# bonevbs/HierarchicalSolvers.jl

Hardware: AMD Instinct MI355X
Metric: factorize+solve time, synthetic 3D problem, exact (swlevel=0) nested-dissection elimination (lower is better)
Workload: dtype f64; 1 GPU; poisson3d_128; n=2097152, nnz=14581760, tree_nodes=1023, tree_depth=10, nrhs=1, compression=none (swlevel=0), partition=subtree-per-rank x1

## Files before the change

### hierarchicalsolvers.jl_amd/_lib.py

```python
from __future__ import annotations

import ctypes as C
import os
import subprocess

_HERE = os.path.dirname(os.path.abspath(__file__))
LIB_PATH = os.path.join(_HERE, "libhs_solver.so")
CSRC = os.path.join(_HERE, "csrc")

i64 = C.c_int64
p_i64 = C.POINTER(C.c_int64)
p_f64 = C.POINTER(C.c_double)


class hs_options(C.Structure):
    _fields_ = [
        ("swlevel", i64), ("swsize", i64), ("atol", C.c_double), ("rtol", C.c_double), ("c_tol", C.c_double),
        ("leafsize", i64), ("kest", i64), ("stepsize", i64), ("verbose", C.c_uint8),
        ("keep_schur", C.c_uint8), ("profile", C.c_uint8), ("split", C.c_uint8), ("hss_d", C.c_uint8), ("hss_dexp", C.c_uint8), ("mf", C.c_uint8), ("dist_top", C.c_uint8), ("seed", i64), ("symmetric", C.c_uint8),
    ]


class hs_tree(C.Structure):
    _fields_ = [
        ("nnodes", i64), ("left", p_i64), ("right", p_i64),
        ("int_ptr", p_i64), ("int_idx", p_i64), ("bnd_ptr", p_i64), ("bnd_idx", p_i64),
        ("iloc_ptr", p_i64), ("iloc_idx", p_i64), ("bloc_ptr", p_i64), ("bloc_idx", p_i64),
    ]


class hs_stats(C.Structure):
    _fields_ = [
        ("n", i64), ("nnodes", i64), ("nlevels", i64), ("max_ni", i64), ("max_nb", i64),
        ("flops_factor", C.c_double), ("bytes_factors", C.c_double), ("bytes_solve", C.c_double),
        ("t_symbolic", C.c_double), ("t_upload", C.c_double), ("t_assemble", C.c_double), ("t_panel", C.c_double),
        ("t_trsm", C.c_double), ("t_gemm", C.c_double), ("t_total", C.c_double), ("t_solve", C.c_double),
        ("gemm_flops", C.c_double), ("gemm_launches", i64),
        ("t_mfma_kernel", C.c_double), ("mfma_kernel_launches", i64), ("gemm_bytes", C.c_double),
    ]


class hs_sparse_dev(C.Structure):
    _fields_ = [("n", i64), ("colptr", C.c_void_p), ("rowval", C.c_void_p), ("nzval", C.c_void_p),
                ("rowptr", C.c_void_p), ("colind", C.c_void_p), ("nzval_r", C.c_void_p)]


class hs_block_arg(C.Structure):
    _fields_ = [("dense", C.c_void_p), ("ld", i64), ("colptr", p_i64), ("rowval", p_i64), ("nzval", C.c_void_p)]


class hs_hss_blockop(C.Structure):
    _fields_ = [("n1", i64), ("n2", i64), ("H1", C.c_void_p), ("H2", C.c_void_p), ("gid", p_i64), ("A", C.POINTER(hs_sparse_dev)), ("lpos", C.c_void_p)]


class hs_hss_options(C.Structure):
    _fields_ = [("leafsize", i64), ("first_split", i64), ("atol", C.c_double), ("rtol", C.c_double), ("kest", i64), ("pad", i64), ("seed", i64),
                ("level_scale", C.c_double)]


HS_TRANSFER_FN = C.CFUNCTYPE(C.c_int, C.c_void_p, i64, p_i64, C.POINTER(C.c_void_p), p_i64, i64, p_i64, C.POINTER(C.c_void_p), p_i64)

HS_OK = 0
HS_ERR_ARGUMENT, HS_ERR_DIMENSION, HS_ERR_TREE, HS_ERR_SINGULAR = -1, -2, -3, -4
HS_ERR_HSS_LEAF, HS_ERR_DEVICE, HS_ERR_NOMEM, HS_ERR_UNSUPPORTED = -5, -6, -7, -8
HS_BLK_LU, HS_BLK_LBI, HS_BLK_UIB, HS_BLK_S, HS_BLK_DLU = 0, 1, 2, 3, 4

EXPORTS = [
    "hs_options_default", "hs_factor_d", "hs_factor_z", "hs_ldiv_d", "hs_ldiv_z", "hs_ldiv_dev_d", "hs_ldiv_dev_z",
    "hs_ldiv_t_d", "hs_ldiv_t_z", "hs_ldiv_dev_t_d", "hs_ldiv_dev_t_z",
    "hs_ldiv_block_d", "hs_ldiv_block_z", "hs_ldiv_block_dev_d", "hs_ldiv_block_dev_z", "hs_ldiv_block_info", "hsk_multi_prob_d", "hsk_multi_prob_z",
    "hs_ldiv_block_t_d", "hs_ldiv_block_t_z", "hs_ldiv_block_dev_t_d", "hs_ldiv_block_dev_t_z", "hsk_multi_prob_t_d", "hsk_multi_prob_t_z",
    "hs_ldiv_ulv_d", "hs_ldiv_ulv_z", "hs_ldiv_ulv_dev_d", "hs_ldiv_ulv_dev_z",
    "hs_mul_d", "hs_mul_z", "hs_mul_dev_d", "hs_mul_dev_z", "hs_mul_info", "hs_factor_error_d", "hs_factor_error_z",
    "hsk_multi_tri_d", "hsk_multi_tri_z", "hsk_multi_tri_t_d", "hsk_multi_tri_t_z",
    "hs_ldiv_sparse_d", "hs_ldiv_sparse_z", "hs_ldiv_sparse_dev_d", "hs_ldiv_sparse_dev_z", "hs_ldiv_sparse_plan", "hs_ldiv_sparse_info",
    "hs_opnorm", "hs_normestinv", "hs_condest", "hs_ldiv_refine_d", "hs_ldiv_refine_z", "hs_ldiv_refine_dev_d", "hs_ldiv_refine_dev_z",
    "hs_ldiv_refine_block_d", "hs_ldiv_refine_block_z", "hs_ldiv_refine_block_dev_d", "hs_ldiv_refine_block_dev_z", "hs_ldiv_refine_block_info",
    "hs_logabsdet", "hs_selinv", "hs_selinv_info", "hs_selinv_lr", "hs_selinv_lr_info", "hs_sym_info",
    "hs_interface_size", "hs_interface_indices", "hs_interface_matrix_d", "hs_interface_matrix_z", "hs_interface_info", "hsk_lu_product_d", "hsk_lu_product_z",
    "hs_interface_condense_d", "hs_interface_condense_z", "hs_interface_condense_dev_d", "hs_interface_condense_dev_z",
    "hs_interface_solve_d", "hs_interface_solve_z", "hs_interface_solve_dev_d", "hs_interface_solve_dev_z",
    "hs_interface_expand_d", "hs_interface_expand_z", "hs_interface_expand_dev_d", "hs_interface_expand_dev_z",
    "hs_sens_d", "hs_sens_z", "hs_sens_dev_d", "hs_sens_dev_z", "hs_misfit_d", "hs_misfit_z", "hs_misfit_dev_d", "hs_misfit_dev_z", "hs_sens_info", "hsk_sddmm_d", "hsk_sddmm_z",
    "hs_tangent_d", "hs_tangent_z", "hs_tangent_dev_d", "hs_tangent_dev_z", "hs_gn_hessvec_d", "hs_gn_hessvec_z", "hs_gn_hessvec_dev_d", "hs_gn_hessvec_dev_z",
    "hs_gn_diag_d", "hs_gn_diag_z", "hs_gn_diag_dev_d", "hs_gn_diag_dev_z", "hs_gn_info", "hsk_gn_rhs_d", "hsk_gn_rhs_z", "hsk_gn_rowsq_d", "hsk_gn_rowsq_z",
    "hs_mod_create_d", "hs_mod_create_z", "hs_mod_create_dev_d", "hs_mod_create_dev_z", "hs_mod_create_sparse_d", "hs_mod_create_sparse_z", "hs_mod_ldiv_d", "hs_mod_ldiv_z",
    "hs_mod_ldiv_dev_d", "hs_mod_ldiv_dev_z", "hs_mod_info", "hs_mod_free", "hs_gmres_block_mod_d", "hs_gmres_block_mod_z",
    "hs_eigs_d", "hs_eigs_z", "hs_eigs_info", "hs_eigs_gen_d", "hs_eigs_gen_z", "hs_eigs_gen_info", "hsk_eigs_coldot_d", "hsk_eigs_coldot_z", "hsk_eigs_rotate_d", "hsk_eigs_rotate_z", "hsk_eigs_chol_inv_d", "hsk_eigs_chol_inv_z", "hsk_small_eig_z", "hsk_eigs_phase_timing", "hsk_eigs_phases", "hsk_eigs_gen_mprod_seconds",
    "hs_f32_create", "hs_f32_ldiv_d", "hs_f32_ldiv_z", "hs_f32_ldiv_dev_d", "hs_f32_ldiv_dev_z", "hs_f32_info", "hs_f32_free", "hs_gmres_block_f32_d", "hs_gmres_block_f32_z",
    "hsk_multi_prob_f32_d", "hsk_multi_prob_f32_z", "hsk_multi_prob_t_f32_d", "hsk_multi_prob_t_f32_z", "hsk_round_factors_f32",
    "hsk_mod_inner_d", "hsk_mod_inner_z", "hsk_mod_apply_d", "hsk_mod_apply_z", "hsk_mod_gather_d", "hsk_mod_gather_z", "hsk_mod_cap_d", "hsk_mod_cap_z",
    "hs_maxrank", "hs_is_complex", "hs_size", "hs_free", "hs_last_error", "hs_last_error_info", "hs_get_stats",
    "hs_node_info", "hs_node_ranks", "hs_node_export", "hs_node_export_piv", "hs_device_info",
    "hs_analyze", "hs_plan", "hs_numeric_begin", "hs_numeric_levels", "hs_numeric_end", "hs_solve_fwd_levels", "hs_solve_bwd_levels",
    "hs_nlevels", "hs_cut_level", "hs_node_owner", "hs_num_exchanges", "hs_exchange_info", "hs_set_schur_buffer",
    "hs_pack_bnd", "hs_unpack_bnd", "hs_extract_owned", "hs_gmres_d", "hs_gmres_z", "hs_gmres_block_d", "hs_gmres_block_z", "hs_gmres_block_info", "hsk_spmm_d", "hsk_spmm_z",
    "hs_gmres_t_d", "hs_gmres_t_z", "hs_gmres_block_t_d", "hs_gmres_block_t_z", "hsk_spmm_op_d", "hsk_spmm_op_z",
    "hs_exchange_kind", "hs_schur_pack_size", "hs_schur_pack", "hs_schur_unpack", "hs_flow_info", "hs_hss_pack_size", "hs_hss_pack", "hs_hss_unpack", "hs_hss_qr_order",
    "hs_comm_unique_id", "hs_comm_create_rccl", "hs_comm_create_host", "hs_comm_free", "hs_comm_kind", "hs_comm_selftest", "hs_comm_bandwidth", "hs_set_comm",
    "hs_symbolic_from_elimtree", "hs_symbolic_from_graph", "hs_symbolic_size", "hs_symbolic_perm", "hs_symbolic_tree", "hs_symbolic_free",
    "hs_hss_options_default", "hs_hss_compress_d", "hs_hss_compress_z", "hs_hss_compress_ex_d", "hs_hss_compress_ex_z", "hs_hss_compress_lru_d", "hs_hss_compress_lru_z", "hs_hss_compress_lru_multi_d", "hs_hss_compress_lru_multi_z", "hs_hss_set_stream", "hs_hss_rank", "hs_hss_size", "hs_hss_samples", "hs_hss_num_nodes",
    "hs_hss_node_info", "hs_hss_node_data", "hs_hss_getindex", "hs_hss_basis", "hs_hss_expand", "hs_hss_mul", "hs_hss_mul_t", "hs_hss_child", "hs_hss_factor", "hs_hss_ldiv", "hs_hss_ldiv_t", "hsk_ulv_t_group_d", "hsk_ulv_t_group_z", "hs_hss_time", "hs_hss_trim", "hs_hss_free", "hs_node_schur_hss",
    "hs_hss_offdiag", "hs_hss_bytes", "hs_hss_prune_leaves", "hs_hss_compatible", "hs_hss_depth", "hs_hss_compress_blockop_d", "hs_hss_compress_blockop_z", "hs_hss_blockop_apply",
    "hsk_gemm_d", "hsk_gemm_z", "hsk_lowrank_d", "hsk_lowrank_z", "hsk_front_factor_d", "hsk_front_factor_z", "hsk_front_batch_d", "hsk_front_batch_z", "hsk_sweep_level_d", "hsk_sweep_level_z", "hsk_flow_tall_rule", "hsk_sweep_path", "hsk_mfma_f64_peak", "hsk_mfma_f64_peak_random", "hsk_flow_pingpong_us", "hsk_bisect_perm",
    "hs_probs_stats_mode", "hs_probs_stats", "hs_trim", "hs_stream_order",
    "hsk_leaf_envelope", "hsk_envelope_enable", "hsk_branch_envelope", "hsk_branch_envelope_enable", "hsk_front_batch_env_d", "hsk_op_flops_mode", "hsk_op_flops",
    "hsk_env_order_enable", "hsk_env_tile_order",
    "hsk_gemm_op_d", "hsk_gemm_lds_enable", "hsk_gemm_lds_launches",
    "hsk_gemm_lds_edge_launches", "hsk_gemm_reg_launches", "hsk_gemm_lds_route", "hsk_gemm_schur_d",
    "hsk_trsm_inv_d", "hsk_trsm_strip_enable", "hsk_trsm_strip_launches", "hsk_trsm_half_launches", "hsk_lookahead_runs", "hsk_front_batch_sym_d", "hsk_front_batch_sym_z",
    "hsk_qr_params", "hsk_qr_chol_d", "hsk_qr_chol_z", "hsk_qr_select", "hsk_qr_refine_d", "hsk_qr_refine_z",
]

_lib = None


def build(force=False, verbose=False):
    if force:
        subprocess.run(["make", "-C", CSRC, "clean"], check=True, capture_output=not verbose)
    r = subprocess.run(["make", "-C", CSRC, "-j4"], capture_output=True, text=True)
    if r.returncode != 0:
        raise RuntimeError("building libhs_solver.so failed:\n" + r.stdout[-4000:] + r.stderr[-4000:])
    return LIB_PATH


def lib():
    global _lib
    if _lib is not None:
        return _lib
    if not os.path.exists(LIB_PATH):
        raise RuntimeError(
            f"{LIB_PATH} not found: the HIP extension is not built (run __graft_entry__.build() or `make -C {CSRC}`); "
            "there is no CPU fallback"
        )
    try:
        import torch
    except Exception:
        pass
    L = C.CDLL(LIB_PATH)
    vp = C.c_void_p
    L.hs_options_default.argtypes = [C.POINTER(hs_options)]
    L.hs_options_default.restype = None
    for f in (L.hs_factor_d, L.hs_factor_z):
        f.argtypes = [i64, p_i64, p_i64, p_f64, C.POINTER(hs_tree), C.POINTER(hs_options), C.POINTER(vp)]
        f.restype = C.c_int
    for f in (L.hs_ldiv_d, L.hs_ldiv_z):
        f.argtypes = [vp, p_f64, i64, p_f64, i64, i64, i64]
        f.restype = C.c_int
    for f in (L.hs_ldiv_dev_d, L.hs_ldiv_dev_z):
        f.argtypes = [vp, vp, i64, vp, i64, i64, i64, vp]
        f.restype = C.c_int
    for host, dev in (("hs_ldiv_t", "hs_ldiv_dev_t"), ("hs_ldiv_block", "hs_ldiv_block_dev"), ("hs_ldiv_block_t", "hs_ldiv_block_dev_t"), ("hs_ldiv_ulv", "hs_ldiv_ulv_dev"),
                      ("hs_mul", "hs_mul_dev")):
        for sfx in ("_d", "_z"):
            f = getattr(L, host + sfx)
            f.argtypes = [vp, C.c_int, p_f64, i64, p_f64, i64, i64, i64]
            f.restype = C.c_int
            f = getattr(L, dev + sfx)
            f.argtypes = [vp, C.c_int, vp, i64, vp, i64, i64, i64, vp]
            f.restype = C.c_int
    L.hs_ldiv_block_info.argtypes = [vp, p_f64]
    L.hs_ldiv_block_info.restype = C.c_int
    L.hs_mul_info.argtypes = [vp, p_f64]
    L.hs_mul_info.restype = C.c_int
    for f in (L.hs_factor_error_d, L.hs_factor_error_z):
        f.argtypes = [vp, C.c_int, vp, i64, i64, i64, C.c_int, p_f64]
        f.restype = C.c_int
    for f in (L.hsk_multi_tri_d, L.hsk_multi_tri_z):
        f.argtypes = [i64, i64, i64, p_f64, i64, p_f64, i64, p_f64, i64, C.c_int, C.c_int, C.POINTER(C.c_int32)]
        f.restype = C.c_int
    for f in (L.hsk_multi_tri_t_d, L.hsk_multi_tri_t_z):
        f.argtypes = [i64, i64, i64, p_f64, i64, p_f64, i64, p_f64, i64, C.c_int, C.c_int, C.c_int, C.POINTER(C.c_int32)]
        f.restype = C.c_int
    for f in (L.hs_ldiv_sparse_d, L.hs_ldiv_sparse_z):
        f.argtypes = [vp, C.c_int, i64, i64, p_i64, p_i64, p_f64, p_i64, i64, p_f64, i64]
        f.restype = C.c_int
    for f in (L.hs_ldiv_sparse_dev_d, L.hs_ldiv_sparse_dev_z):
        f.argtypes = [vp, C.c_int, i64, i64, p_i64, p_i64, vp, p_i64, i64, vp, i64, vp]
        f.restype = C.c_int
    L.hs_ldiv_sparse_plan.argtypes = [vp, C.c_int, i64, i64, p_i64, p_i64, p_i64, i64, p_i64, p_i64, C.POINTER(C.c_uint8)]
    L.hs_ldiv_sparse_plan.restype = C.c_int
    L.hs_ldiv_sparse_info.argtypes = [vp, p_f64]
    L.hs_ldiv_sparse_info.restype = C.c_int
    for f in (L.hsk_multi_prob_d, L.hsk_multi_prob_z):
        f.argtypes = [i64, i64, i64, p_f64, i64, p_f64, i64, p_f64, i64, C.c_int, C.c_int, C.POINTER(C.c_int32)]
        f.restype = C.c_int
    for f in (L.hsk_multi_prob_t_d, L.hsk_multi_prob_t_z):
        f.argtypes = [i64, i64, i64, p_f64, i64, p_f64, i64, p_f64, i64, C.c_int, C.c_int, C.c_int, C.POINTER(C.c_int32)]
        f.restype = C.c_int
    L.hs_opnorm.argtypes = [vp, C.c_int, p_f64]
# ... 352 lines not shown
        f.restype = C.c_int
    for f in (L.hs_hss_compress_lru_d, L.hs_hss_compress_lru_z):
        f.argtypes = [i64, vp, i64, vp, i64, vp, i64, vp, i64, i64, i64, C.c_int, p_i64, C.POINTER(hs_hss_options), vp, C.POINTER(vp)]
        f.restype = C.c_int
    for f in (L.hs_hss_compress_lru_multi_d, L.hs_hss_compress_lru_multi_z):
        f.argtypes = [i64, p_i64, C.POINTER(vp), p_i64, C.POINTER(vp), p_i64, C.POINTER(vp), p_i64, C.POINTER(vp), p_i64, p_i64, p_i64, C.POINTER(p_i64),
                      C.POINTER(C.POINTER(hs_hss_options)), vp, C.POINTER(vp)]
        f.restype = C.c_int
    for f in (L.hs_hss_rank, L.hs_hss_size, L.hs_hss_samples, L.hs_hss_num_nodes, L.hs_hss_bytes):
        f.argtypes = [vp]
        f.restype = i64
    L.hs_node_schur_hss.argtypes = [vp, i64, C.POINTER(hs_hss_options), C.POINTER(vp)]
    L.hs_node_schur_hss.restype = C.c_int
    L.hs_hss_set_stream.argtypes = [vp, vp]
    L.hs_hss_set_stream.restype = C.c_int
    L.hs_hss_node_info.argtypes = [vp, i64, p_i64]
    L.hs_hss_node_info.restype = C.c_int
    L.hs_hss_node_data.argtypes = [vp, i64, p_i64, vp, vp, vp, vp]
    L.hs_hss_node_data.restype = C.c_int
    L.hs_hss_getindex.argtypes = [vp, p_i64, i64, p_i64, i64, vp, i64, C.c_int]
    L.hs_hss_getindex.restype = C.c_int
    L.hs_hss_trim.argtypes = []
    L.hs_hss_trim.restype = i64
    L.hs_hss_basis.argtypes = [vp, i64, vp, i64, C.c_int]
    L.hs_hss_basis.restype = C.c_int
    L.hs_hss_expand.argtypes = [vp, vp, i64, C.c_int]
    L.hs_hss_expand.restype = C.c_int
    L.hs_hss_mul.argtypes = [vp, vp, i64, vp, i64, i64, C.c_int]
    L.hs_hss_mul.restype = C.c_int
    L.hs_hss_mul_t.argtypes = [vp, vp, i64, vp, i64, i64, C.c_int]
    L.hs_hss_mul_t.restype = C.c_int
    L.hs_hss_child.argtypes = [vp, C.c_int, C.POINTER(vp)]
    L.hs_hss_child.restype = C.c_int
    L.hs_hss_prune_leaves.argtypes = [vp, C.POINTER(vp)]
    L.hs_hss_prune_leaves.restype = C.c_int
    L.hs_hss_compatible.argtypes = [vp, vp]
    L.hs_hss_compatible.restype = C.c_int
    L.hs_hss_depth.argtypes = [vp]
    L.hs_hss_depth.restype = i64
    L.hs_hss_offdiag.argtypes = [vp, C.c_int, vp, i64, vp, i64, C.c_int]
    L.hs_hss_offdiag.restype = C.c_int
    for f in (L.hs_hss_compress_blockop_d, L.hs_hss_compress_blockop_z):
        f.argtypes = [C.POINTER(hs_hss_blockop), vp, i64, vp, i64, vp, i64, i64, i64, p_i64, C.POINTER(hs_hss_options), vp, C.POINTER(vp)]
        f.restype = C.c_int
    L.hs_hss_blockop_apply.argtypes = [C.POINTER(hs_hss_blockop), C.c_int, vp, i64, vp, i64, i64, C.c_int, vp]
    L.hs_hss_blockop_apply.restype = C.c_int
    L.hs_hss_factor.argtypes = [vp]
    L.hs_hss_factor.restype = C.c_int
    L.hs_hss_ldiv.argtypes = [vp, vp, i64, i64, C.c_int]
    L.hs_hss_ldiv.restype = C.c_int
    L.hs_hss_ldiv_t.argtypes = [vp, C.c_int, vp, i64, i64, C.c_int]
    L.hs_hss_ldiv_t.restype = C.c_int
    for f in (L.hsk_ulv_t_group_d, L.hsk_ulv_t_group_z):
        f.argtypes = [i64, p_i64, p_f64, i64, p_f64, i64, p_f64, i64, C.c_int]
        f.restype = C.c_int
    L.hs_hss_time.argtypes = [vp, C.c_int]
    L.hs_hss_time.restype = C.c_double
    L.hs_hss_free.argtypes = [vp]
    L.hs_hss_free.restype = None
    L.hsk_bisect_perm.argtypes = [i64, p_i64, p_i64, i64, p_i64, p_i64]
    L.hsk_bisect_perm.restype = C.c_int
    L.hs_stream_order.argtypes = [vp, vp, C.c_int]
    L.hs_stream_order.restype = C.c_int
    L.hs_trim.argtypes = []
    L.hs_trim.restype = i64
    L.hs_probs_stats_mode.argtypes = [C.c_int]
    L.hs_probs_stats_mode.restype = C.c_int
    L.hs_probs_stats.argtypes = [p_f64]
    L.hs_probs_stats.restype = C.c_int
    L.hsk_leaf_envelope.argtypes = [i64, p_i64, p_i64, C.POINTER(C.c_int32), i64, i64, C.POINTER(C.c_int32), C.POINTER(C.c_int32)]
    L.hsk_leaf_envelope.restype = C.c_int
    L.hsk_envelope_enable.argtypes = [C.c_int]
    L.hsk_envelope_enable.restype = C.c_int
    L.hsk_branch_envelope.argtypes = [i64, p_i64, p_i64, C.POINTER(C.c_int32), i64, i64, i64, i64, C.POINTER(C.c_int32), C.POINTER(C.c_int32)]
    L.hsk_branch_envelope.restype = C.c_int
    L.hsk_front_batch_env_d.argtypes = [i64, p_i64, p_i64, C.c_int, p_f64, C.POINTER(C.c_int32), p_f64, p_f64, p_f64, p_i64, p_i64, p_i64]
    L.hsk_front_batch_env_d.restype = C.c_int
    L.hsk_branch_envelope_enable.argtypes = [C.c_int]
    L.hsk_branch_envelope_enable.restype = C.c_int
    L.hsk_env_order_enable.argtypes = [C.c_int]
    L.hsk_env_order_enable.restype = C.c_int
    L.hsk_env_tile_order.argtypes = [C.c_int, C.c_int, C.c_int, C.POINTER(C.c_int32), C.POINTER(C.c_int32)]
    L.hsk_env_tile_order.restype = C.c_int
    L.hsk_op_flops_mode.argtypes = [C.c_int]
    L.hsk_op_flops_mode.restype = C.c_int
    L.hsk_op_flops.argtypes = [p_f64]
    L.hsk_op_flops.restype = C.c_int
    L.hsk_flow_pingpong_us.argtypes = [C.c_int, C.c_int]
    L.hsk_flow_pingpong_us.restype = C.c_double
    L.hsk_mfma_f64_peak.argtypes = [C.c_int, C.c_int]
    L.hsk_mfma_f64_peak.restype = C.c_double
    L.hsk_mfma_f64_peak_random.argtypes = [C.c_int, C.c_int]
    L.hsk_mfma_f64_peak_random.restype = C.c_double
    _lib = L
    return L


class DimensionMismatch(ValueError):
    """Julia ``DimensionMismatch`` (blockmatrix.jl:13-16,116-117; nesteddissection.jl:107)."""


class SingularException(ArithmeticError):
    """``LinearAlgebra.SingularException`` -- what ``\\`` raises in the reference on an exactly singular block."""


class DeviceError(RuntimeError):
    """No usable gfx950 device / HIP runtime failure.  There is no CPU fallback."""


class UnsupportedError(NotImplementedError):
    pass


class NoConvergence(ArithmeticError):

    def __init__(self, msg, partial=None):
        super().__init__(msg)
        self.partial = partial


def check(status):
    if status == HS_OK:
        return
    msg = lib().hs_last_error().decode("utf-8", "replace")
    info = lib().hs_last_error_info()
    exc = {
        HS_ERR_ARGUMENT: ValueError,
        HS_ERR_DIMENSION: DimensionMismatch,
        HS_ERR_TREE: RuntimeError,
        HS_ERR_SINGULAR: SingularException,
        HS_ERR_HSS_LEAF: RuntimeError,
        HS_ERR_DEVICE: DeviceError,
        HS_ERR_NOMEM: MemoryError,
        HS_ERR_UNSUPPORTED: UnsupportedError,
    }.get(status, RuntimeError)
    e = exc(msg)
    e.info = info
    e.status = status
    raise e
```

### hierarchicalsolvers.jl_amd/csrc/hs_api.hip

```cpp
#include <chrono>
#include <mutex>
#include <algorithm>
#include <cmath>
#include <cstdarg>
#include <cstdio>
#include <cstring>
#include <cstdlib>
#include <string>
#include <utility>
#include <vector>

#include "../../include/hs_solver.h"
#include "../../include/hs_hss.h"
#include "hs_common.h"
#include "hs_host.h"
#include "hs_sweep.h"
#include "hs_condest.h"
#include "hs_selinv.h"
#include "hs_interface.h"
#include "hs_solve_multi.h"

static thread_local std::string g_err;
static thread_local long long g_err_info = 0;

// ... 105 lines not shown
      x12, x21;
  bool mfb = false;
  void *hss2 = nullptr, *hss_keep = nullptr;
  void *bW12 = nullptr, *bZ12 = nullptr, *bC21 = nullptr, *bZ21 = nullptr;
  int bk12 = 0, bk21 = 0, bldw = 0, bldz12 = 0, bldc21 = 0, bldz21 = 0;
  bool hss_interior() const { return hssd || (mf && !mfd); }
};

struct LevelH {
  std::vector<int> nodes;
  std::vector<int> mine;
  int maxni = 0, maxnb = 0, maxm = 0, maxnbc = 0;
  size_t lf_begin = 0, lf_end = 0;
  size_t cfs_end = 0;
  size_t sb_begin = 0, sb_end = 0;
  size_t desc_off = 0;
  size_t sc_off = 0, sc_cnt = 0;
  std::vector<int> h_ni, h_nb;
  std::vector<const int*> h_env;
  std::vector<const int*> h_env_leaf;
  int ndense = 0;
  int nplain = 0;
  int nmf = 0;
  int dmaxni = 0, dmaxnb = 0, dmaxm = 0;
  bool aligned16 = true;
  bool sym_ok = true;
};

struct Exchange {
  int node, level, src, dst, nb;
  long long nelems;
  int hss = 0;
};

#include "hs_envelope.h"
#include "hs_sched.h"
#include "hs_split.h"
#include "hs_comm.h"

struct hs_handle {
  size_t fac_bytes = 0, inv_bytes = 0, sb_bytes = 0;
  void* d_cfs = nullptr;
  size_t cfs_bytes = 0, cfs_elems = 0;
  bool is_complex = false;
  int64_t n = 0, nnz = 0;
  int nnodes = 0;
  int nreal = 0;
  int nuser = 0;
  std::vector<int> last_of_user, first_of_user, u_ni, u_nb, u_level;
  int rank = 0, nranks = 1, cut_level = 1;
  hs_options opts;
  std::vector<NodeH> nodes;
  std::vector<LevelH> levels;
  std::vector<int> fidx_host;
  std::vector<Exchange> exchanges;
  void* d_fac = nullptr;
  void* d_inv = nullptr;
  void* d_sb = nullptr;
  int* d_int = nullptr;
  int* d_tmpi = nullptr;
  int* d_info = nullptr;
  int* d_growth = nullptr;
  unsigned long long* d_symflag = nullptr;
  int64_t sym_fronts = 0, sym_plain = 0;
  bool optimistic = true;
  int* d_own = nullptr;
  int* d_pos = nullptr;
  int* d_owned = nullptr;
  int64_t n_owned = 0;
  int64_t* d_rowptr = nullptr;
  int32_t* d_colind = nullptr;
  int64_t* d_tperm = nullptr;
  void* d_nzr = nullptr;
  int* d_lpos = nullptr;
  bool mf_on = false;
  double static_factor_bytes = 0.0;
  int64_t* d_colptr = nullptr;
  int32_t* d_rowval = nullptr;
  void* d_nz = nullptr;
  void* d_nodes = nullptr;
  void* d_sc = nullptr;
  void* d_solve = nullptr;
  int* d_env = nullptr;
  std::vector<int> env_host;
  std::vector<const int*> env_dev[2];
  int env_dev_state = 1;
  void* d_w1 = nullptr;
  void* d_w2 = nullptr;
  int* d_flow = nullptr;
  void* d_e1 = nullptr;
  void* d_e2 = nullptr;
  size_t flow_bytes = 0;
  int* h_flow_err = nullptr;
  int flow_seq = 0;
  void* d_part = nullptr;
  void* d_b = nullptr;
  size_t fac_elems = 0, inv_elems = 0, sb_elems = 0, int_elems = 0;
  bool sb_kept = false;
  bool numeric_open = false, factored = false;
  hipStream_t stream = nullptr;
  hipStream_t stream2 = nullptr;
  hipStream_t stream_la = nullptr;
  hipStream_t stream2m = nullptr;
  hipEvent_t ev0 = nullptr, ev1 = nullptr;
  hs_comm* comm = nullptr;
  hipStream_t stream_comm = nullptr;
  int* d_gflags = nullptr;
  void* d_stage_u = nullptr;
  void *d_stage_s = nullptr, *d_stage_r = nullptr;
  void *d_xs = nullptr, *d_xr = nullptr, *d_xall = nullptr;
  int* d_owned_all = nullptr;
  std::vector<int64_t> owned_off;
  hipEvent_t ev_ca = nullptr, ev_cb = nullptr;
  Profiler prof;
  void* d_cdesc = nullptr;
  size_t cdesc_cap = 0;
  void* d_lr_t = nullptr;
  void* d_lr_part = nullptr;
  size_t lr_t_elems = 0, lr_part_elems = 0;
  int64_t maxrank = 0;
  std::vector<std::pair<int, hipEvent_t>> level_events;
  double flops = 0.0;
  hs_stats stats;
  void* cx = nullptr;
  void (*cx_free)(void*) = nullptr;
  void* sx = nullptr;
  void (*sx_free)(void*) = nullptr;
  void* mx = nullptr;
  void (*mx_free)(void*) = nullptr;
  void* ix = nullptr;
  void (*ix_free)(void*) = nullptr;
  std::vector<int> sp_owner;
  double sp_info[8] = {0, 0, 0, 0, 0, 0, 0, 0};
  double sens_info[8] = {0, 0, 0, 0, 0, 0, 0, 0};
  double gn_info[8] = {0, 0, 0, 0, 0, 0, 0, 0};
};

static inline int rup(int x, int a) { return (x + a - 1) / a * a; }
static inline size_t rups(size_t x, size_t a) { return (x + a - 1) / a * a; }

namespace {
struct ArenaCache {
  std::mutex mu;
  struct Blk { void* p; size_t bytes; };
  std::vector<Blk> v;
};
ArenaCache& arena_cache() {
  static ArenaCache* c = new ArenaCache();
  return *c;
}
constexpr size_t HS_ARENA_MIN = (size_t)256 << 20;
constexpr size_t HS_ARENA_SLOTS = 4;
bool arena_cache_on() {
  static const bool on = !(getenv("HS_ARENA_CACHE") && getenv("HS_ARENA_CACHE")[0] == '0');
  return on;
}
}
extern "C" int64_t hs_arena_trim(void) {
  int64_t freed = 0;
  ArenaCache& c = arena_cache();
  std::lock_guard<std::mutex> lk(c.mu);
  for (auto& b : c.v) {
    (void)hipFree(b.p);
    freed += (int64_t)b.bytes;
  }
  c.v.clear();
  return freed;
}
extern "C" int64_t hs_trim(void) { return hs_arena_trim() + hs_hss_trim(); }
static void* arena_take(size_t bytes) {
  if (!arena_cache_on() || bytes < HS_ARENA_MIN) return nullptr;
  ArenaCache& c = arena_cache();
  std::lock_guard<std::mutex> lk(c.mu);
  size_t best = c.v.size();
  for (size_t i = 0; i < c.v.size(); ++i)
    if (c.v[i].bytes >= bytes && c.v[i].bytes <= bytes + bytes / 8 && (best == c.v.size() || c.v[i].bytes < c.v[best].bytes)) best = i;
  if (best == c.v.size()) return nullptr;
  void* p = c.v[best].p;
  c.v.erase(c.v.begin() + (long)best);
  return p;
}
static void arena_give(void* p, size_t bytes) {
  if (!p) return;
  if (!arena_cache_on() || bytes < HS_ARENA_MIN) {
    (void)hipFree(p);
    return;
  }
  ArenaCache& c = arena_cache();
  std::lock_guard<std::mutex> lk(c.mu);
  c.v.push_back({p, bytes});
  while (c.v.size() > HS_ARENA_SLOTS) {
    (void)hipFree(c.v.front().p);
    c.v.erase(c.v.begin());
  }
}

static void free_lowrank_any(hs_handle* h);
static void free_hss_any(hs_handle* h);
static void free_mfd_buffers(hs_handle* h);
static void free_handle(hs_handle* h) {
  if (!h) return;
  if (h->stream) (void)hipStreamSynchronize(h->stream);
  if (h->cx && h->cx_free) h->cx_free(h->cx);
  if (h->sx && h->sx_free) h->sx_free(h->sx);
  if (h->mx && h->mx_free) h->mx_free(h->mx);
  if (h->ix && h->ix_free) h->ix_free(h->ix);
  for (auto& x : h->nodes)
    if (x.S_hss) {
      hs_hss_free((hs_hss*)x.S_hss);
      x.S_hss = nullptr;
    }
  free_mfd_buffers(h);
  free_hss_any(h);
  free_lowrank_any(h);
  arena_give(h->d_fac, h->fac_bytes);
  arena_give(h->d_inv, h->inv_bytes);
  arena_give(h->d_sb, h->sb_bytes);
  arena_give(h->d_cfs, h->cfs_bytes);
  void* ptrs[] = {h->d_int, h->d_tmpi, h->d_colptr, h->d_rowval, h->d_nz,
                  h->d_nodes, h->d_sc,  h->d_solve, h->d_w1,  h->d_w2,   h->d_part,   h->d_b,   h->d_owned,
                  h->d_rowptr, h->d_colind, h->d_tperm, h->d_nzr, h->d_lpos, h->d_env, h->d_symflag};
  for (void* p : ptrs)
    if (p) (void)hipFree(p);
  if (h->ev0) (void)hipEventDestroy(h->ev0);
  if (h->ev1) (void)hipEventDestroy(h->ev1);
  if (h->d_gflags) (void)hipFree(h->d_gflags);
  if (h->d_flow) (void)hipFree(h->d_flow);
  if (h->d_e1) (void)hipFree(h->d_e1);
  if (h->d_e2) (void)hipFree(h->d_e2);
  if (h->h_flow_err) (void)hipHostFree(h->h_flow_err);
  for (void* q : {h->d_xs, h->d_xr, h->d_xall, (void*)h->d_owned_all})
    if (q) (void)hipFree(q);
  if (h->ev_ca) (void)hipEventDestroy(h->ev_ca);
  if (h->ev_cb) (void)hipEventDestroy(h->ev_cb);
  if (h->d_stage_u) (void)hipFree(h->d_stage_u);
  if (h->d_stage_s) (void)hipFree(h->d_stage_s);
  if (h->d_stage_r) (void)hipFree(h->d_stage_r);
  if (h->stream_comm) (void)hipStreamDestroy(h->stream_comm);
  if (h->stream2) (void)hipStreamDestroy(h->stream2);
  if (h->stream_la) (void)hipStreamDestroy(h->stream_la);
  if (h->stream2m) (void)hipStreamDestroy(h->stream2m);
  if (h->stream) (void)hipStreamDestroy(h->stream);
  delete h;
}

extern "C" void hs_free(hs_handle* h) { free_handle(h); }

static void build_plan(hs_handle* h, int64_t n, const hs_tree* tr, const SplitTree* st = nullptr) {
  if (!tr || tr->nnodes <= 0) HS_FAIL(HS_ERR_ARGUMENT, 0, "ArgumentError: empty tree");
  const int nn = (int)tr->nnodes;
  h->nreal = nn;
  std::vector<NodeH>& N = h->nodes;
  N.assign(nn, NodeH());
  auto len = [](const int64_t* ptr, int i) { return (int)(ptr[i + 1] - ptr[i]); };
  for (int i = 0; i < nn; ++i) {
    NodeH& x = N[i];
    x.left = (int)tr->left[i];
    x.right = (int)tr->right[i];
    x.kind = st ? st->kind[i] : 0;
    x.user = st ? st->user[i] : i;
    if ((x.left < 0) != (x.right < 0) && x.kind != 2)
      HS_FAIL(HS_ERR_TREE, i, "Expected nested dissection to be a binary tree. Found a node with only one child.");
    x.leaf = x.left < 0;
    if (!x.leaf) {
      if (x.left >= i || x.right >= i || x.left == x.right)
        HS_FAIL(HS_ERR_ARGUMENT, i, "ArgumentError: tree is not in post-order (children must precede node %d)", i);
      if (N[x.left].parent >= 0 || (x.right >= 0 && N[x.right].parent >= 0)) HS_FAIL(HS_ERR_ARGUMENT, i, "ArgumentError: node has two parents");
      N[x.left].parent = i;
      if (x.right >= 0) N[x.right].parent = i;
    }
    x.ni = len(tr->int_ptr, i);
    x.nb = len(tr->bnd_ptr, i);
    x.m = x.ni + x.nb;
  }
  for (int i = 0; i < nn - 1; ++i)
    if (N[i].parent < 0) HS_FAIL(HS_ERR_ARGUMENT, i, "ArgumentError: found either less than or more than one root.");
  N[nn - 1].level = 1;
  int maxlevel = 1;
  for (int i = nn - 2; i >= 0; --i) {
    N[i].level = N[N[i].parent].level + 1;
    maxlevel = std::max(maxlevel, N[i].level);
  }
  h->fidx_host.clear();
  std::vector<int>& F = h->fidx_host;
  for (int i = 0; i < nn; ++i) {
    NodeH& x = N[i];
    x.off_fidx = F.size();
    for (int64_t e = tr->int_ptr[i]; e < tr->int_ptr[i + 1]; ++e) {
      int64_t g = tr->int_idx[e];
      if (g < 1 || g > n) HS_FAIL(HS_ERR_DIMENSION, i, "BoundsError: int index %lld of node %d outside 1:%lld", (long long)g, i, (long long)n);
      F.push_back((int)(g - 1));
    }
    for (int64_t e = tr->bnd_ptr[i]; e < tr->bnd_ptr[i + 1]; ++e) {
      int64_t g = tr->bnd_idx[e];
      if (g < 1 || g > n) HS_FAIL(HS_ERR_DIMENSION, i, "BoundsError: bnd index %lld of node %d outside 1:%lld", (long long)g, i, (long long)n);
      F.push_back((int)(g - 1));
    }
  }
  for (int i = 0; i < nn; ++i) {
    NodeH& x = N[i];
    if (x.leaf) {
      x.ni1 = x.ni;
      x.nb1 = x.nb;
      x.oni = x.ni; x.oni1 = x.ni1; x.onb1 = x.nb1;
// ... 525 lines not shown
      }
      HS_HIP(hipMemcpy(h->d_colptr, cp.data(), (n + 1) * sizeof(int64_t), hipMemcpyHostToDevice));
      HS_HIP(hipMemcpy(h->d_rowval, rv.data(), nnz * sizeof(int32_t), hipMemcpyHostToDevice));
    }
    {
      std::vector<int> hint(ints, 0);
      std::copy(h->fidx_host.begin(), h->fidx_host.end(), hint.begin());
      for (int i = 0; i < h->nnodes; ++i) {
        NodeH& x = N[i];
        if (x.parent < 0 || !(x.mine || x.ghost)) continue;
        int* cm = hint.data() + x.off_cmap;
        for (int e = 0; e < x.nb; ++e) cm[e] = -1;
        const NodeH& p = N[x.parent];
        if (p.level == 0) {
          for (int e = 0; e < x.nb; ++e) cm[e] = e;
          continue;
        }
        bool is_left = (p.left == i);
        int offi = is_left ? 0 : p.oni1, offb = is_left ? 0 : p.onb1;
        const int* np = (split.active && p.kind == 1 && !split.newpos[x.parent].empty()) ? split.newpos[x.parent].data() : nullptr;
        int q = 0;
        for (int64_t e = tree->iloc_ptr[i]; e < tree->iloc_ptr[i + 1]; ++e, ++q) cm[tree->iloc_idx[e] - 1] = np ? np[offi + q] : offi + q;
        q = 0;
        for (int64_t e = tree->bloc_ptr[i]; e < tree->bloc_ptr[i + 1]; ++e, ++q) cm[tree->bloc_idx[e] - 1] = p.oni + offb + q;
      }
      for (int i = 0; i < h->nnodes; ++i) {
        NodeH& x = N[i];
        if (x.off_spos < 0) continue;
        const std::vector<int>& np = split.newpos[i];
        int* sp = hint.data() + x.off_spos;
        for (int e = 0; e < x.oni; ++e) sp[np[e]] = e;
      }
      HS_HIP(hipMemcpy(dint, hint.data(), ints * sizeof(int), hipMemcpyHostToDevice));
      if (h->mf_on) mf_sperm(h, hint);
    }
    if (h->mf_on) {
      mf_couplings(h, n, colptr, rowval);
      mf_build_csr(h, n, colptr, rowval);
    }
    lapa("pattern, index lists, cmaps (host + upload)");
    if (nranks > 1) {
      std::vector<int> owned;
      for (int i = 0; i < h->nnodes; ++i)
        if (N[i].owner == h->rank) owned.insert(owned.end(), h->fidx_host.begin() + N[i].off_fidx, h->fidx_host.begin() + N[i].off_fidx + N[i].ni);
      h->n_owned = (int64_t)owned.size();
      dmalloc((void**)&h->d_owned, owned.size() * sizeof(int), "owned index list");
      if (!owned.empty()) HS_HIP(hipMemcpy(h->d_owned, owned.data(), owned.size() * sizeof(int), hipMemcpyHostToDevice));
    }

    if (colptr && rowval) {
      std::vector<int> where((size_t)n, -1);
      for (LevelH& L : h->levels) {
        L.h_env.clear();
        L.h_env_leaf.clear();
        for (int k = 0; k < L.ndense; ++k) {
          NodeH& x = N[L.mine[k]];
          if (x.kind != 0 || x.dist || x.compressed || x.hssd || x.mf || x.ni <= 0) continue;
          const int nblk = hs_env_nblocks(x.ni, x.nb);
          x.off_env = (long long)h->env_host.size();
          h->env_host.resize(h->env_host.size() + 2 * (size_t)nblk);
          int* fl = h->env_host.data() + x.off_env;
          const int* fidx = h->fidx_host.data() + x.off_fidx;
          if (x.leaf)
            hs_leaf_envelope(colptr, rowval, fidx, x.ni, x.nb, where.data(), fl, fl + nblk);
          else
            hs_branch_envelope(colptr, rowval, fidx, x.ni, x.nb, x.ni1, x.nb1, where.data(), fl, fl + nblk);
        }
      }
      if (!h->env_host.empty()) {
        dmalloc((void**)&h->d_env, h->env_host.size() * sizeof(int), "front envelopes");
        HS_HIP(hipMemcpy(h->d_env, h->env_host.data(), h->env_host.size() * sizeof(int), hipMemcpyHostToDevice));
        for (LevelH& L : h->levels) {
          bool any = false, any_leaf = false;
          for (int k = 0; k < L.ndense; ++k) {
            any = any || N[L.mine[k]].off_env >= 0;
            any_leaf = any_leaf || (N[L.mine[k]].off_env >= 0 && N[L.mine[k]].leaf);
          }
          for (int k = 0; k < L.ndense; ++k) {
            const NodeH& x = N[L.mine[k]];
            if (any) L.h_env.push_back(x.off_env >= 0 ? h->env_host.data() + x.off_env : nullptr);
            if (any_leaf) L.h_env_leaf.push_back(x.off_env >= 0 && x.leaf ? h->env_host.data() + x.off_env : nullptr);
          }
        }
      }
    }

    {
      std::vector<NodeDesc<T>> hn;
      std::vector<ScatterDesc<T>> hsc;
      std::vector<SolveNode<T>> sn;
      for (int lv = (int)h->levels.size() - 1; lv >= 0; --lv) {
        LevelH& L = h->levels[lv];
        L.sc_off = hsc.size();
        for (int id : L.mine) {
          NodeH& x = N[id];
          NodeDesc<T> d;
          memset(&d, 0, sizeof d);
          d.LF = (x.cfront ? (T*)h->d_cfs : dfac) + x.off_LF;
          d.UR = (x.cfront ? (T*)h->d_cfs : dfac) + x.off_UR;
          d.SB = dsb + x.off_SB;
          int nblk = (x.ni + HS_PB - 1) / HS_PB;
          d.invL = dinv + x.off_inv;
          d.invU = dinv + x.off_inv + (size_t)nblk * HS_PB * HS_PB;
          d.inv256L = dinv + x.off_inv256;
          d.inv256U = d.inv256L + (size_t)((x.ni + 255) / 256) * 256 * 256;
          d.ipiv = dint + x.off_ipiv;
          d.rperm = dint + x.off_rperm;
          d.cand0 = h->d_tmpi + x.off_cand;
          d.cand1 = d.cand0 + x.ncand;
          d.pivlist = d.cand1 + x.ncand;
          d.info = h->d_info + id;
          d.growth = h->d_growth + id;
          d.fidx = dint + x.off_fidx;
          d.ni = x.ni; d.nb = x.nb; d.m = x.m;
          d.ldl = x.ldl; d.ldu = x.ldu; d.lds = x.lds;
          d.ni1 = x.ni1; d.nb1 = x.nb1;
          d.s_ni = x.oni; d.s_ni1 = x.oni1; d.s_nb1 = x.onb1;
          d.spos = x.off_spos >= 0 ? dint + x.off_spos : nullptr;
          d.isleaf = x.leaf ? 1 : 0;
          d.node = id;
          d.env = x.off_env >= 0 ? h->d_env + x.off_env : nullptr;
          d.finalize();
          hn.push_back(d);
          h->env_dev[1].push_back(d.env);
          h->env_dev[0].push_back(x.leaf ? d.env : nullptr);
          if (x.batch_pos < L.ndense && ((((uintptr_t)d.LF | (uintptr_t)d.UR | (uintptr_t)d.SB) & 15) || ((d.ldl | d.ldu | d.lds) & 1)))
            L.aligned16 = false;
          SolveNode<T> q;
          memset(&q, 0, sizeof q);
          q.LF = d.LF; q.UR = d.UR; q.invL = d.invL; q.invU = d.invU;
          q.inv256L = dinv + x.off_inv256;
          q.inv256U = q.inv256L + (size_t)((x.ni + 255) / 256) * 256 * 256;
          q.rperm = d.rperm; q.fidx = d.fidx;
          q.ni = x.ni; q.nb = x.nb; q.m = x.m; q.ldl = x.ldl; q.ldu = x.ldu;
          q.compressed = x.compressed ? 1 : 0;
          q.mrows = x.compressed ? x.ni : x.m;
          if (x.hssd || x.mf) q.ni = q.nb = q.m = q.mrows = 0;
          q.woff = x.woff;
          q.poff = poff;
          poff += (long long)((x.nb + 511) / 512) * x.ni;
          sn.push_back(q);
          h->flops += front_flops(x.ni, x.nb);
          for (int side = 0; side < 2; ++side) {
            int c = side == 0 ? x.left : x.right;
            if (x.leaf || c < 0) continue;
            const NodeH& ch = N[c];
            if (ch.nb == 0 || x.mf) continue;
            ScatterDesc<T> sc;
            sc.S = dsb + ch.off_SB;
            sc.cmap = dint + ch.off_cmap;
            sc.nbc = ch.nb;
            sc.lds = ch.lds;
            sc.parent = x.batch_pos;
            hsc.push_back(sc);
            L.maxnbc = std::max(L.maxnbc, ch.nb);
          }
        }
        L.sc_cnt = hsc.size() - L.sc_off;
      }
      dmalloc(&h->d_nodes, hn.size() * sizeof(NodeDesc<T>), "front descriptors");
      dmalloc(&h->d_sc, hsc.size() * sizeof(ScatterDesc<T>), "scatter descriptors");
      dmalloc(&h->d_solve, sn.size() * sizeof(SolveNode<T>), "solve descriptors");
      if (!hn.empty()) HS_HIP(hipMemcpy(h->d_nodes, hn.data(), hn.size() * sizeof(NodeDesc<T>), hipMemcpyHostToDevice));
      if (h->env_dev[0] == h->env_dev[1]) h->env_dev[0].clear(), h->env_dev[1].clear();
      h->env_dev_state = 1;
      if (!hsc.empty()) HS_HIP(hipMemcpy(h->d_sc, hsc.data(), hsc.size() * sizeof(ScatterDesc<T>), hipMemcpyHostToDevice));
// ... 90 lines not shown
  T* dsb = (T*)h->d_sb;
  const NodeDesc<T>* dn_all = (const NodeDesc<T>*)h->d_nodes;
  const ScatterDesc<T>* dsc_all = (const ScatterDesc<T>*)h->d_sc;
  const bool branch_env = hs_branch_envelope_enabled();
  if (!h->env_dev[0].empty() && h->env_dev_state != (branch_env ? 1 : 0)) {
    HS_HIP(hipStreamSynchronize(s));
    const std::vector<const int*>& v = h->env_dev[branch_env ? 1 : 0];
    HS_HIP(hipMemcpy2D((char*)h->d_nodes + offsetof(NodeDesc<T>, env), sizeof(NodeDesc<T>), v.data(), sizeof(const int*), sizeof(const int*), v.size(),
                       hipMemcpyHostToDevice));
    h->env_dev_state = branch_env ? 1 : 0;
  }
  for (int lv = lv_from; lv >= lv_to; --lv) {
    LevelH& L = h->levels[lv];
    if (L.mine.empty()) continue;
    const NodeDesc<T>* dn = dn_all + L.desc_off;
    const int nb_ = (int)L.mine.size() - L.nmf;
    static const bool progress = getenv("HS_PROGRESS") != nullptr;
    if (progress) fprintf(stderr, "[hs] enqueue level %d (%d fronts)\n", lv, nb_);
    static const bool opt_env = !(getenv("HS_OPTIMISTIC") && getenv("HS_OPTIMISTIC")[0] == '0');
    bool try_opt = opt_env && h->optimistic && (L.ndense > 0 || L.nplain > 0);
    const NodeH* dx = (L.mine.size() == 1 && h->nodes[L.mine[0]].dist) ? &h->nodes[L.mine[0]] : nullptr;
    DistFront<T> DF;
    if (dx) {
      if (!h->comm) HS_FAIL(HS_ERR_ARGUMENT, 0, "ArgumentError: hs_options.dist_top needs a communicator (hs_set_comm) before hs_numeric_levels");
      hipStream_t sc = h->stream_comm;
      static const int dist_nb = Sched<T>::env_int("HS_DIST_NB", 512);
      if (dist_nb < 256 || (dist_nb & (dist_nb - 1))) HS_FAIL(HS_ERR_ARGUMENT, dist_nb, "ArgumentError: HS_DIST_NB = %d must be a power of two >= 256", dist_nb);
      const size_t nblk32 = (dx->ni + HS_PB - 1) / HS_PB;
      T* dinv = (T*)h->d_inv;
      static const int dist_period = std::max(1, Sched<T>::env_int("HS_DIST_PERIOD", 2));
      DF = DistFront<T>{h->comm, dx->glo, dx->gcnt, h->rank, dist_nb, dist_period, sc, dx->ni, dx->nb, dx->m, dx->ldl, dx->ldu, dx->lds,
                        dfac + dx->off_LF, dfac + dx->off_UR, dsb + dx->off_SB, dinv + dx->off_inv, dinv + dx->off_inv + nblk32 * HS_PB * HS_PB,
                        dinv + dx->off_inv256, dinv + dx->off_inv256 + (size_t)((dx->ni + 255) / 256) * 65536, h->d_int + dx->off_ipiv,
                        (T*)h->d_stage_s, (T*)h->d_stage_r, (T*)h->d_stage_u};
      const NodeH& cl = h->nodes[dx->left];
      const NodeH& cr = h->nodes[dx->right];
      const NodeH& cm = cl.mine ? cl : cr;
      const NodeH& co = cl.mine ? cr : cl;
      const int partner = cl.mine ? h->rank + cm.gcnt : h->rank - cm.gcnt;
      hipEvent_t ej;
      HS_HIP(hipEventCreateWithFlags(&ej, hipEventDisableTiming));
      HS_HIP(hipEventRecord(ej, s));
      HS_HIP(hipStreamWaitEvent(sc, ej, 0));
      std::vector<HsPiece> sends, recvs;
      if (cm.nb > 0) sends.push_back({partner, cm.ext_sb ? (T*)cm.ext_sb : dsb + cm.off_SB, (size_t)cm.lds * cm.nb * sizeof(T)});
      if (co.nb > 0) recvs.push_back({partner, co.ext_sb ? (T*)co.ext_sb : dsb + co.off_SB, (size_t)co.lds * co.nb * sizeof(T)});
      h->comm->transfer(sends, recvs, sc);
      HS_HIP(hipEventRecord(ej, sc));
      HS_HIP(hipStreamWaitEvent(s, ej, 0));
      HS_HIP(hipStreamSynchronize(sc));
      (void)hipEventDestroy(ej);
      try_opt = dist_group_or(h->comm, h->d_gflags, dx->glo, dx->gcnt, h->rank, try_opt ? 0 : 1, sc) == 0 && L.ndense > 0;
    }
    int sym_counted = 0;
    for (int attempt = 0; attempt < 2; ++attempt) {
    h->prof.tag = lv;
    hipEvent_t ea = h->prof.begin(s);
    if (L.lf_end > L.lf_begin) HS_HIP(hipMemsetAsync(dfac + L.lf_begin, 0, (L.lf_end - L.lf_begin) * sizeof(T), s));
    if (L.cfs_end > 0) HS_HIP(hipMemsetAsync(h->d_cfs, 0, L.cfs_end * sizeof(T), s));
    if (h->nranks == 1) {
      if (L.sb_end > L.sb_begin) HS_HIP(hipMemsetAsync(dsb + L.sb_begin, 0, (L.sb_end - L.sb_begin) * sizeof(T), s));
    } else {
      for (int id : L.mine) {
        const NodeH& x = h->nodes[id];
        if (x.nb == 0) continue;
        T* sb = x.ext_sb ? (T*)x.ext_sb : dsb + x.off_SB;
        HS_HIP(hipMemsetAsync(sb, 0, (size_t)x.lds * x.nb * sizeof(T), s));
      }
    }
    launch_init_fronts<T>(dn, nb_, L.maxni, s);
    launch_mark<T>(dn, nb_, L.maxm, h->d_own, h->d_pos, s);
    launch_gather<T>(dn, nb_, L.maxm, h->d_colptr, h->d_rowval, (const T*)h->d_nz, h->d_own, h->d_pos, s);
    launch_scatter<T>(dn, dsc_all + L.sc_off, (int)L.sc_cnt, L.maxnbc, s);
    h->prof.end(ea, HS_CAT_ASSEMBLE, s);
    if (L.ndense > 0) {
      Sched<T> sch{dn, L.ndense, L.dmaxni, L.dmaxnb, L.dmaxm, s, &h->prof, L.h_ni.data(), L.h_nb.data(), h->stream2, 0, h->stream_la, h->stream2m};
      sch.sn = (const SolveNode<T>*)h->d_solve + L.desc_off;
      sch.optimistic = try_opt && attempt == 0;
      sch.aligned16 = L.aligned16 && h->nranks == 1;
      const std::vector<const int*>& henv = branch_env ? L.h_env : L.h_env_leaf;
      if (sch.optimistic && !dx && !henv.empty() && hs_envelope_enabled()) {
        sch.env = true;
        sch.h_env = henv.data();
      }
      sch.sym = h->opts.symmetric && sch.optimistic && !dx && L.sym_ok;
      if (attempt == 1) h->sym_fronts -= sym_counted, h->sym_plain -= L.ndense - sym_counted;
      sym_counted = sch.sym ? L.ndense : 0;
      h->sym_fronts += sym_counted;
      h->sym_plain += L.ndense - sym_counted;
      if (dx)
        factor_front_dist<T>(sch, DF);
      else
        sch.factor_fronts();
    }
    if (L.nplain > 0)
      factor_compressed_level<T>(h, L.mine.data() + L.ndense, L.nplain, dn + L.ndense, (const SolveNode<T>*)h->d_solve + L.desc_off + L.ndense, 1, try_opt && attempt == 0);
      if (!(try_opt && attempt == 0)) break;
      std::vector<int> gr(h->nnodes);
      HS_HIP(hipMemcpyAsync(gr.data(), h->d_growth, sizeof(int) * h->nnodes, hipMemcpyDeviceToHost, s));
      HS_HIP(hipStreamSynchronize(s));
      static const bool force_redo = getenv("HS_OPTIMISTIC_FORCE_REDO") != nullptr;
      bool redo = force_redo;
      for (int k = 0; k < L.ndense + L.nplain; ++k) redo = redo || gr[L.mine[k]] != 0;
      if (dx) redo = dist_group_or(h->comm, h->d_gflags, dx->glo, dx->gcnt, h->rank, redo ? 1 : 0, h->stream_comm) != 0;
      if (!redo) break;
      h->optimistic = false;
      if (h->opts.verbose) fprintf(stderr, "[hs] level %d: a pivot outside the diagonal block was needed; redoing the level with tournament pivoting\n", lv);
    }
    h->sym_plain += (int64_t)L.mine.size() - L.ndense;
    if (L.nplain > 0) factor_compressed_level<T>(h, L.mine.data() + L.ndense, L.nplain, dn + L.ndense, (const SolveNode<T>*)h->d_solve + L.desc_off + L.ndense, 2);
    if (nb_ > L.ndense + L.nplain) factor_hss_fronts<T>(h, L.mine.data() + L.ndense + L.nplain, nb_ - L.ndense - L.nplain, dn + L.ndense + L.nplain);
    {
      std::vector<int> todo;
      for (int k = 0; k < L.ndense; ++k)
        if (h->nodes[L.mine[k]].s_hss) todo.push_back(L.mine[k]);
      if (!todo.empty()) {
        std::vector<MfSchurArgs<T>> args;
        for (int id : todo) {
          const NodeH& x = h->nodes[id];
          args.push_back(MfSchurArgs<T>{id, x.ext_sb ? (const T*)x.ext_sb : dsb + x.off_SB, x.lds, nullptr, 0, nullptr, 0, nullptr, 0, 0, 0});
        }
        mf_compress_schur_dense_batch<T>(h, args, s);
      }
    }
    if (L.nmf > 0) factor_mf_fronts<T>(h, L.mine.data() + nb_, L.nmf);
    static const bool lvl_env = getenv("HS_VERBOSE_LEVELS") != nullptr;
    if (h->opts.profile || lvl_env) {
      hipEvent_t e = nullptr;
      (void)hipEventCreate(&e);
      (void)hipEventRecord(e, s);
      h->level_events.push_back({lv, e});
    }
  }
}

static void numeric_end(hs_handle* h) {
  if (!h->numeric_open) HS_FAIL(HS_ERR_ARGUMENT, 0, "ArgumentError: hs_numeric_end before hs_numeric_begin");
  hipStream_t s = h->stream;
  HS_HIP(hipEventRecord(h->ev1, s));
  HS_HIP(hipStreamSynchronize(s));
  h->numeric_open = false;
  float ms = 0.f;
  HS_HIP(hipEventElapsedTime(&ms, h->ev0, h->ev1));
  h->stats.t_total = ms * 1e-3;
  Profiler& prof = h->prof;
  prof.collect();
  if (!h->level_events.empty()) {
    const char* ev = getenv("HS_VERBOSE_LEVELS");
    hipEvent_t prev = h->ev0;
    for (auto& le : h->level_events) {
      float lms = 0.f;
      (void)hipEventElapsedTime(&lms, prev, le.second);
      if (ev && ev[0] == '1') {
        const LevelH& L = h->levels[le.first];
        double fl = 0.0;
        for (int id : L.mine) fl += front_flops(h->nodes[id].ni, h->nodes[id].nb);
        if (h->is_complex) fl *= 4.0;
        fprintf(stderr, "[hs] level %2d: %4zu fronts, max (ni,nb)=(%d,%d)  %9.3f ms  %8.2f TFLOP/s (minimal count)\n", le.first, L.mine.size(),
                L.maxni, L.maxnb, lms, lms > 0 ? fl / (lms * 1e-3) / 1e12 : 0.0);
        if (prof.on && le.first >= 0 && le.first < 64) {
          const double* m = prof.ms_tag[le.first];
          fprintf(stderr, "[hs]          per-launch events: gemm %.1f  panel %.1f  laswp %.1f  trsm %.1f  assemble %.1f ms\n", m[HS_CAT_GEMM], m[HS_CAT_PANEL],
                  m[HS_CAT_LASWP], m[HS_CAT_TRSM], m[HS_CAT_ASSEMBLE]);
        }
      }
      if (prev != h->ev0) (void)hipEventDestroy(prev);
// ... 1162 lines not shown
```

### hierarchicalsolvers.jl_amd/csrc/hs_common.h

```cpp
#pragma once
#include <hip/hip_runtime.h>
#include <stdint.h>

#define HS_PB 32
#define HS_CHUNK 256
#define HS_BIG (1 << 30)
#define HS_GROWTH_MAX 4.0

struct cplx {
  double re, im;
};

__host__ __device__ inline cplx operator+(cplx a, cplx b) { return {a.re + b.re, a.im + b.im}; }
__host__ __device__ inline cplx operator-(cplx a, cplx b) { return {a.re - b.re, a.im - b.im}; }
__host__ __device__ inline cplx operator-(cplx a) { return {-a.re, -a.im}; }
__host__ __device__ inline cplx operator*(cplx a, cplx b) { return {a.re * b.re - a.im * b.im, a.re * b.im + a.im * b.re}; }
__host__ __device__ inline cplx operator/(cplx a, cplx b) {
  if (fabs(b.re) >= fabs(b.im)) {
    double r = b.im / b.re, d = b.re + b.im * r;
    return {(a.re + a.im * r) / d, (a.im - a.re * r) / d};
  } else {
    double r = b.re / b.im, d = b.re * r + b.im;
    return {(a.re * r + a.im) / d, (a.im * r - a.re) / d};
  }
// ... 17 lines not shown
template <>
__device__ __forceinline__ void gst<cplx>(cplx* p, cplx v) {
  hs_d2u w = {v.re, v.im};
  *(hs_d2u HS_AS_GLOBAL*)p = w;
}
__device__ __forceinline__ hs_d2u gld2(const double* p) { return *(const hs_d2u HS_AS_GLOBAL*)p; }
__device__ __forceinline__ hs_d2u gld2(const cplx* p) { return *(const hs_d2u HS_AS_GLOBAL*)p; }
__device__ __forceinline__ void gst2(cplx* p, hs_d2u v) { *(hs_d2u HS_AS_GLOBAL*)p = v; }

template <class T>
struct Scal;
template <>
struct Scal<double> {
  static __host__ __device__ inline double zero() { return 0.0; }
  static __host__ __device__ inline double one() { return 1.0; }
  static __host__ __device__ inline double abs1(double a) { return fabs(a); }
  static __host__ __device__ inline double fma(double a, double b, double c) { return ::fma(a, b, c); }
  static __host__ __device__ inline double fnma(double a, double b, double c) { return ::fma(-a, b, c); }
};
template <>
struct Scal<cplx> {
  static __host__ __device__ inline cplx zero() { return {0.0, 0.0}; }
  static __host__ __device__ inline cplx one() { return {1.0, 0.0}; }
  static __host__ __device__ inline double abs1(cplx a) { return fabs(a.re) + fabs(a.im); }
  static __host__ __device__ inline cplx fma(cplx a, cplx b, cplx c) {
    return {::fma(a.re, b.re, ::fma(-a.im, b.im, c.re)), ::fma(a.re, b.im, ::fma(a.im, b.re, c.im))};
  }
  static __host__ __device__ inline cplx fnma(cplx a, cplx b, cplx c) {
    return {::fma(-a.re, b.re, ::fma(a.im, b.im, c.re)), ::fma(-a.re, b.im, ::fma(-a.im, b.re, c.im))};
  }
};

template <class T>
struct NodeDesc {
  T* LF;
  T* UR;
  T* SB;
  T* invL;
  T* invU;
  T* inv256L;
  T* inv256U;
  int* ipiv;
  int* rperm;
  int* cand0;
  int* cand1;
  int* pivlist;
  int* info;
  int* growth;
  const int* fidx;
  int ni, nb, m;
  int ldl, ldu, lds;
  int ni1, nb1;
  const int* spos;
  int s_ni, s_ni1, s_nb1;
  int pivrows;
  int isleaf;
  int node;
  const int* env;
  T* mp[3];
  int mld[3], mrows[3], mcols[3];
  __host__ void finalize() {
    if (pivrows <= 0) pivrows = ni;
    if (s_ni <= 0) { s_ni = ni; s_ni1 = ni1; s_nb1 = nb1; }
    mp[0] = LF; mp[1] = UR; mp[2] = SB;
    mld[0] = ldl; mld[1] = ldu; mld[2] = lds;
    mrows[0] = m; mrows[1] = ni; mrows[2] = nb;
    mcols[0] = ni; mcols[1] = nb; mcols[2] = nb;
  }
};

enum { HS_MAT_LF = 0, HS_MAT_UR = 1, HS_MAT_SB = 2 };

struct GemmOp {
  int cmat, bmat;
  int r0, r1;
  int c0, c1;
  int k0, k1;
  int ainv;
  int cap;
  int prio;
  int env;
  int count;
  int order;
};

#define HS_ENV_NONE HS_BIG
__host__ __device__ inline int hs_env_block(int p, int ni) { return p < ni ? p >> 5 : ((ni + 31) >> 5) + ((p - ni) >> 5); }
__host__ __device__ inline int hs_env_min(const int* first, int ni, int lo, int hi) {
  int v = HS_ENV_NONE;
  for (int b = hs_env_block(lo, ni), b1 = hs_env_block(hi - 1, ni); b <= b1; ++b) v = first[b] < v ? first[b] : v;
  return v;
}
struct EnvClip {
  const int* fL;
  const int* fU;
  int row0, col0, kbase, ni;
};
__host__ __device__ inline int hs_env_kstart(const EnvClip& e, int m_lo, int m_hi, int n_lo, int n_hi) {
  int k = e.kbase;
  if (e.fL) { const int v = hs_env_min(e.fL, e.ni, e.row0 + m_lo, e.row0 + m_hi); k = v > k ? v : k; }
  if (e.fU) { const int v = hs_env_min(e.fU, e.ni, e.col0 + n_lo, e.col0 + n_hi); k = v > k ? v : k; }
  return k;
}

template <class T>
struct GemmProb {
  const T* A;
  const T* B;
  T* C;
  int M, N, K;
  int lda, ldb, ldc;
  int* flag = nullptr;
  int flag_rows = 0;
};

template <class T>
__device__ inline void mat_of(const NodeDesc<T>* pn, int which, T*& p, int& ld, int& rows, int& cols) {
  p = pn->mp[which];
  ld = pn->mld[which];
  rows = pn->mrows[which];
  cols = pn->mcols[which];
}

enum { HS_GEMM_ROUTE_REG = 0, HS_GEMM_ROUTE_LDS = 1, HS_GEMM_ROUTE_EDGE = 2 };
template <class T>
void launch_gemm_op(const NodeDesc<T>* dnodes, int nbatch, int maxM, int maxN, const GemmOp& op, hipStream_t s, int route = HS_GEMM_ROUTE_REG,
                    bool shifted = false, long long live_tiles = -1);
inline int hs_gemm_lds_route(int cmat, int r0, int k0, int k1, int ni) {
  const int K = (k1 < ni ? k1 : ni) - k0, arow = r0 + (cmat == HS_MAT_SB ? ni : 0);
  if (K <= 0 || (k0 & 1)) return HS_GEMM_ROUTE_REG;
  return ((K & 15) == 0 && !(arow & 1)) ? HS_GEMM_ROUTE_LDS : HS_GEMM_ROUTE_EDGE;
}
inline int hs_gemm_lds_route_join(int a, int b) {
  if (a == HS_GEMM_ROUTE_REG || b == HS_GEMM_ROUTE_REG) return HS_GEMM_ROUTE_REG;
  return (a == HS_GEMM_ROUTE_EDGE || b == HS_GEMM_ROUTE_EDGE) ? HS_GEMM_ROUTE_EDGE : HS_GEMM_ROUTE_LDS;
}
bool hs_trsm_strip_enabled();
void hs_trsm_half_note();
void hs_lookahead_note();
void launch_trsm_strip(const NodeDesc<double>* dnodes, int nbatch, int maxN, const GemmOp& op, hipStream_t s);
bool hs_envelope_enabled();
bool hs_branch_envelope_enabled();
template <class T>
void launch_gemm_probs(const GemmProb<T>* dprobs, int nprob, int maxM, int maxN, int accumulate_minus, hipStream_t s);

template <class T>
void launch_tournament_round(const NodeDesc<T>* dnodes, int nbatch, int pb, int round, int maxchunks, hipStream_t s);
template <class T>
void launch_tournament_stage(const NodeDesc<T>* dnodes, int nbatch, int pb, int stage, int maxblocks, hipStream_t s);
int hs_tour_block_rows(bool is_complex);
void hs_create_lookahead_streams(hipStream_t* la, hipStream_t* side_masked, hipStream_t* side);
template <class T>
void launch_panel_pivot(const NodeDesc<T>* dnodes, int nbatch, int pb, int fuse, hipStream_t s);
template <class T>
void launch_panel_l21(const NodeDesc<T>* dnodes, int nbatch, int pb, int maxrows, int fuse, hipStream_t s, int rlim = HS_BIG);
template <class T>
bool launch_trsm_small(const NodeDesc<T>* dnodes, int nbatch, int mat, int r0, int rows, int c0, int c1, int maxcols, hipStream_t s);
template <class T>
bool launch_group256(const NodeDesc<T>* dnodes, int nbatch, int grp, hipStream_t s);
template <class T>
void launch_laswp(const NodeDesc<T>* dnodes, int nbatch, int mat, int c0, int c1, int k0, int k1, int maxcols, hipStream_t s);
#define HS_SYM_STRIP 256
template <class T>
void launch_sym_transpose(const NodeDesc<T>* dnodes, int nbatch, int mat, int r0, int r1, int c0, int c1, int lower, int maxrows, int maxcols, hipStream_t s);
template <class T>
void launch_sym_check(int64_t n, const int64_t* colptr, const int32_t* rowval, const T* nz, unsigned long long* first, hipStream_t s);

template <class T>
void launch_init_fronts(const NodeDesc<T>* dnodes, int nbatch, int maxni, hipStream_t s);
template <class T>
void launch_mark(const NodeDesc<T>* dnodes, int nbatch, int maxm, int* own, int* pos, hipStream_t s);
template <class T>
void launch_gather(const NodeDesc<T>* dnodes, int nbatch, int maxm, const int64_t* colptr, const int32_t* rowval,
                   const T* nzval, const int* own, const int* pos, hipStream_t s);
template <class T>
struct ScatterDesc {
  const T* S;
  const int* cmap;
  int nbc, lds;
  int parent;
};
template <class T>
void launch_scatter(const NodeDesc<T>* dnodes, const ScatterDesc<T>* dsc, int nsc, int maxnbc, hipStream_t s);

template <class T>
struct SolveNode {
  const T* LF;
  const T* UR;
  const T* invL;
  const T* invU;
  T* inv256L;
  T* inv256U;
  const int* rperm;
  const int* fidx;
  int ni, nb, m, ldl, ldu;
  int mrows;
  int compressed;
  long long woff;
  long long poff;
};
template <class T>
void launch_sweep_gather(const SolveNode<T>* dn, int nbatch, int maxni, const T* b, T* w, bool perm, hipStream_t s);
template <class T>
void launch_sweep_scatter(const SolveNode<T>* dn, int nbatch, int maxni, T* b, const T* x, bool perm, hipStream_t s);
template <class T>
void launch_fwd_step(const SolveNode<T>* dn, int nbatch, int blk, int maxm, T* w, T* y, T* b, hipStream_t s);
template <class T>
void launch_int_update(const SolveNode<T>* dn, int nbatch, int maxni, int maxnb, const T* b, T* part, const T* y, T* w, hipStream_t s);
template <class T>
void launch_bwd_step(const SolveNode<T>* dn, int nbatch, int blk, T* w, T* x, hipStream_t s);
// ... 56 lines not shown
```

### hierarchicalsolvers.jl_amd/csrc/hs_dist.h

```cpp
#pragma once

template <class T>
struct DistFront {
  hs_comm* comm;
  int glo, gcnt, rank;
  int NB;
  int period;
  hipStream_t sc;
  int ni, nb, m, ldl, ldu, lds;
  T *LF, *UR, *SB, *invL, *invU, *inv256L, *inv256U;
  int* ipiv;
  T *stage_s, *stage_r;
  T* stage_u;
  int owner(int j) const { return glo + (j / period) % gcnt; }
};

static inline size_t dist_stage_elems(int m, int ni, int NB, size_t esz) {
  return (size_t)m * NB + (size_t)2 * (NB / HS_PB) * HS_PB * HS_PB + (size_t)2 * (NB / 256) * 65536 + ((size_t)2 * ni * sizeof(int) + esz - 1) / esz + 64;
}

template <class T>
static size_t dist_panel_message(const DistFront<T>& D, int j, T* stage, int pack, hipStream_t s) {
  const int c0 = j * D.NB, w = std::min(D.NB, D.ni - c0), rows = D.m - c0;
  const int b32 = c0 / HS_PB, n32 = (w + HS_PB - 1) / HS_PB, b256 = c0 / 256, n256 = (w + 255) / 256;
// ... 10 lines not shown
  blk(D.invL + (size_t)b32 * HS_PB * HS_PB, (size_t)n32 * HS_PB * HS_PB);
  blk(D.invU + (size_t)b32 * HS_PB * HS_PB, (size_t)n32 * HS_PB * HS_PB);
  blk(D.inv256L + (size_t)b256 * 65536, (size_t)n256 * 65536);
  blk(D.inv256U + (size_t)b256 * 65536, (size_t)n256 * 65536);
  const size_t ibytes = (size_t)2 * D.ni * sizeof(int);
  if (pack == 1) HS_HIP(hipMemcpyAsync(q, D.ipiv, ibytes, hipMemcpyDeviceToDevice, s));
  if (pack == 0) HS_HIP(hipMemcpyAsync(D.ipiv, q, ibytes, hipMemcpyDeviceToDevice, s));
  return (size_t)((char*)q - (char*)stage) + ibytes;
}

template <class T>
static void dist_fanout(const DistFront<T>& D, int j, T* from, size_t bytes, hipStream_t s) {
  const int owner = D.owner(j);
  std::vector<HsPiece> sends, recvs;
  if (owner == D.rank) {
    for (int r = D.glo; r < D.glo + D.gcnt; ++r)
      if (r != D.rank) sends.push_back({r, from, bytes});
  } else {
    recvs.push_back({owner, D.stage_r, bytes});
  }
  D.comm->transfer(sends, recvs, s);
}

template <class T>
static void dist_bcast_panel(const DistFront<T>& D, int j, hipStream_t s) {
  const size_t bytes = dist_panel_message(D, j, (T*)nullptr, -1, s);
  dist_fanout(D, j, D.stage_s, bytes, s);
  if (D.owner(j) != D.rank) dist_panel_message(D, j, D.stage_r, 0, s);
}

template <class T>
static void dist_bcast_upper(const DistFront<T>& D, int j, hipStream_t s) {
  const int c0 = j * D.NB, w = std::min(D.NB, D.ni - c0);
  if (c0 == 0) return;
  const bool mine = D.owner(j) == D.rank;
  const size_t bytes = (size_t)c0 * w * sizeof(T);
  T* Up = D.LF + (size_t)c0 * D.ldl;
  if (mine) HS_HIP(hipMemcpy2DAsync(D.stage_u, (size_t)c0 * sizeof(T), Up, (size_t)D.ldl * sizeof(T), (size_t)c0 * sizeof(T), w, hipMemcpyDeviceToDevice, s));
  dist_fanout(D, j, D.stage_u, bytes, s);
  if (!mine) HS_HIP(hipMemcpy2DAsync(Up, (size_t)D.ldl * sizeof(T), D.stage_r, (size_t)c0 * sizeof(T), (size_t)c0 * sizeof(T), w, hipMemcpyDeviceToDevice, s));
}

static inline void dist_bnd_slice(int nb, int gcnt, int q, int& b0, int& b1) {
  int per = ((nb + gcnt - 1) / gcnt + 127) / 128 * 128;
  b0 = std::min(q * per, nb);
  b1 = std::min(b0 + per, nb);
}

template <class T>
static void dist_allgather_bnd(const DistFront<T>& D, hipStream_t s) {
  if (D.nb == 0) return;
  int mb0, mb1;
  dist_bnd_slice(D.nb, D.gcnt, D.rank - D.glo, mb0, mb1);
  for (int which = 0; which < 2; ++which) {
    T* base = which == 0 ? D.UR : D.SB;
    const size_t ld = which == 0 ? D.ldu : D.lds;
    std::vector<HsPiece> sends, recvs;
    for (int q = 0; q < D.gcnt; ++q) {
      const int r = D.glo + q;
      if (r == D.rank) continue;
      int b0, b1;
      dist_bnd_slice(D.nb, D.gcnt, q, b0, b1);
      if (mb1 > mb0) sends.push_back({r, base + (size_t)mb0 * ld, ld * (mb1 - mb0) * sizeof(T)});
      if (b1 > b0) recvs.push_back({r, base + (size_t)b0 * ld, ld * (b1 - b0) * sizeof(T)});
    }
    D.comm->transfer(sends, recvs, s);
  }
}

template <class T>
static void factor_front_dist(Sched<T>& base, const DistFront<T>& D) {
  const int NB = D.NB, ni = D.ni, g = D.gcnt, me = D.rank - D.glo;
  const int nblk = (ni + NB - 1) / NB;
  if (nblk <= 0) return;
  auto mine = [&](int j) { return D.owner(j) == D.rank; };
  int last_packed = -1;
  Sched<T> mn = base, side = base;
  mn.s2 = nullptr;
  mn.s_la = nullptr;
  side.s = base.s2 ? base.s2 : base.s;
  side.s2 = nullptr;
  side.s_la = nullptr;
  side.hiprio = base.s2 ? 1 : 0;
  hipStream_t s = mn.s, s2 = side.s, sc = D.sc;
  int b0, b1;
  dist_bnd_slice(D.nb, g, me, b0, b1);
  std::vector<hipEvent_t> ev_have(nblk), ev_fact(nblk);
  for (auto& e : ev_have) HS_HIP(hipEventCreateWithFlags(&e, hipEventDisableTiming));
  for (auto& e : ev_fact) HS_HIP(hipEventCreateWithFlags(&e, hipEventDisableTiming));
  hipEvent_t ev_main, ev_iter[3];
  HS_HIP(hipEventCreateWithFlags(&ev_main, hipEventDisableTiming));
  for (auto& e : ev_iter) HS_HIP(hipEventCreateWithFlags(&e, hipEventDisableTiming));
  HS_HIP(hipEventRecord(ev_main, s));
  HS_HIP(hipStreamWaitEvent(sc, ev_main, 0));
  if (s2 != s) HS_HIP(hipStreamWaitEvent(s2, ev_main, 0));
  if (mine(0)) {
    side.lu_rec(0, NB);
    dist_panel_message(D, 0, D.stage_s, 1, s2);
    last_packed = 0;
    HS_HIP(hipEventRecord(ev_fact[0], s2));
    HS_HIP(hipStreamWaitEvent(sc, ev_fact[0], 0));
  }
  dist_bcast_panel(D, 0, sc);
  HS_HIP(hipEventRecord(ev_have[0], sc));
  for (int j = 0; j < nblk; ++j) {
    const int c0 = j * NB, c1 = c0 + NB, c2 = c1 + NB;
    const bool has_next = j + 1 < nblk;
    if (j >= 3) HS_HIP(hipEventSynchronize(ev_iter[j % 3]));
    HS_HIP(hipStreamWaitEvent(s, mine(j) ? ev_fact[j] : ev_have[j], 0));
    const bool next_mine = has_next && mine(j + 1);
    if (next_mine) {
      mn.laswp(HS_MAT_LF, c1, c2, c0, c1);
      mn.trsm_rec(HS_MAT_LF, c0, c1, c1, c2);
      mn.gemm(HS_MAT_LF, HS_MAT_LF, c1, HS_BIG, c1, c2, c0, c1);
      HS_HIP(hipEventRecord(ev_main, s));
      HS_HIP(hipStreamWaitEvent(s2, ev_main, 0));
      side.lu_rec(c1, c2);
      if (last_packed >= 0) HS_HIP(hipStreamWaitEvent(s2, ev_have[last_packed], 0));
      dist_panel_message(D, j + 1, D.stage_s, 1, s2);
      last_packed = j + 1;
      HS_HIP(hipEventRecord(ev_fact[j + 1], s2));
      HS_HIP(hipStreamWaitEvent(sc, ev_fact[j + 1], 0));
    }
    if (has_next) {
      dist_bcast_panel(D, j + 1, sc);
      HS_HIP(hipEventRecord(ev_have[j + 1], sc));
      dist_bcast_upper(D, j + 1, sc);
    }
    for (int k = j + (next_mine ? 2 : 1); k < nblk;) {
      if (!mine(k)) {
        ++k;
        continue;
      }
      int ke = k;
      while (ke < nblk && mine(ke)) ++ke;
      const int k0 = k * NB, k1 = ke * NB;
      mn.laswp(HS_MAT_LF, k0, k1, c0, c1);
      mn.trsm_rec(HS_MAT_LF, c0, c1, k0, k1);
      mn.gemm(HS_MAT_LF, HS_MAT_LF, c1, HS_BIG, k0, k1, c0, c1);
      k = ke;
    }
    if (b1 > b0) {
      mn.laswp(HS_MAT_UR, b0, b1, c0, c1);
      mn.trsm_rec(HS_MAT_UR, c0, c1, b0, b1);
      mn.gemm(HS_MAT_UR, HS_MAT_UR, c1, HS_BIG, b0, b1, c0, c1);
    }
    HS_HIP(hipEventRecord(ev_iter[j % 3], s));
  }
  HS_HIP(hipEventRecord(ev_main, sc));
  HS_HIP(hipStreamWaitEvent(s, ev_main, 0));
  for (int c0 = 0; c0 + NB < ni; c0 += NB) mn.laswp(HS_MAT_LF, c0, c0 + NB, c0 + NB, HS_BIG);
  if (b1 > b0) mn.gemm(HS_MAT_SB, HS_MAT_UR, 0, HS_BIG, b0, b1, 0, HS_BIG);
  if (D.nb > 0) {
    HS_HIP(hipEventRecord(ev_main, s));
    HS_HIP(hipStreamWaitEvent(sc, ev_main, 0));
    dist_allgather_bnd(D, sc);
    HS_HIP(hipEventRecord(ev_main, sc));
    HS_HIP(hipStreamWaitEvent(s, ev_main, 0));
  }
  HS_HIP(hipStreamSynchronize(s));
  for (auto& e : ev_have) (void)hipEventDestroy(e);
  for (auto& e : ev_fact) (void)hipEventDestroy(e);
  for (auto& e : ev_iter) (void)hipEventDestroy(e);
  (void)hipEventDestroy(ev_main);
}

// ... 18 lines not shown
```

### hierarchicalsolvers.jl_amd/csrc/hs_sched.h

```cpp
#pragma once
#include <algorithm>
#include <climits>
#include <cstdio>
#include <cstdlib>
#include <utility>
#include <vector>
#include "../../include/hs_solver.h"
#include "hs_common.h"

enum { HS_CAT_GEMM = 0, HS_CAT_PANEL = 1, HS_CAT_LASWP = 2, HS_CAT_TRSM = 3, HS_CAT_ASSEMBLE = 4, HS_NCAT = 5 };
struct Profiler {
  bool on = false;
  struct Rec {
    hipEvent_t e0, e1;
    int cat;
    double fl;
    int M, N, K, nbatch, tag;
    int form, side;
    double bytes;
  };
  int tag = 0;
  double ms_tag[64][HS_NCAT] = {};
  std::vector<Rec> recs;
  double flops[HS_NCAT] = {0, 0, 0, 0, 0};
  double gemm_bytes = 0.0;
  double ms[HS_NCAT] = {0, 0, 0, 0, 0};
  long long launches[HS_NCAT] = {0, 0, 0, 0, 0};
  hipEvent_t begin(hipStream_t s) {
    hipEvent_t e = nullptr;
    if (on) {
      (void)hipEventCreate(&e);
      (void)hipEventRecord(e, s);
    }
    return e;
  }
  void end(hipEvent_t e0, int cat, hipStream_t s, double fl = 0.0, int M = 0, int N = 0, int K = 0, int nbatch = 0, int form = 0, int side = 0,
           double bytes = 0.0) {
    launches[cat]++;
    flops[cat] += fl;
    if (!on) return;
    hipEvent_t e1;
    (void)hipEventCreate(&e1);
    (void)hipEventRecord(e1, s);
    recs.push_back({e0, e1, cat, fl, M, N, K, nbatch, tag, form, side, bytes});
  }
  void collect() {
    const char* logf = getenv("HS_GEMM_LOG");
    FILE* lf = (logf && on) ? fopen(logf, "a") : nullptr;
    const char* logl = getenv("HS_LAUNCH_LOG");
    FILE* ll = (logl && on) ? fopen(logl, "a") : nullptr;
    for (auto& r : recs) {
      float t = 0.f;
      if (hipEventElapsedTime(&t, r.e0, r.e1) == hipSuccess) {
        ms[r.cat] += t;
        if (r.tag >= 0 && r.tag < 64) ms_tag[r.tag][r.cat] += t;
      }
      if (lf && r.cat == HS_CAT_GEMM) fprintf(lf, "%d %d %d %d %.6g %.6f\n", r.M, r.N, r.K, r.nbatch, r.fl, t);
      if (ll) fprintf(ll, "%d %d %d %d %d %.6g %.6f\n", r.tag, r.cat, r.form, r.side, r.nbatch, r.bytes, t);
      (void)hipEventDestroy(r.e0);
      (void)hipEventDestroy(r.e1);
    }
    if (lf) fclose(lf);
    if (ll) fclose(ll);
    recs.clear();
  }
};

template <class T>
struct Sched {
  const NodeDesc<T>* dn;
  int nbatch, maxni, maxnb, maxm;
  hipStream_t s;
  Profiler* pf;
  const int* h_ni;
  const int* h_nb;
  hipStream_t s2 = nullptr;
  int maxpiv = 0;
  hipStream_t s_la = nullptr;
  hipStream_t s2m = nullptr;
  int hiprio = 0;
  const SolveNode<T>* sn = nullptr;
  bool wide = false;
  int rlim = HS_BIG;
  bool optimistic = false;
  bool env = false;
  const int* const* h_env = nullptr;
  bool sym = false;
  bool aligned16 = false;

  void dbg(const char* what, int a = 0, int b = 0, int c = 0, int d = 0) {
    static int on = -1;
    if (on < 0) {
      const char* e = getenv("HS_DEBUG_SYNC");
      on = (e && (e[0] == '1' || e[0] == '2')) ? 1 : 0;
    }
    if (!on) return;
    hipError_t e = hipStreamSynchronize(s);
    if (e == hipSuccess) e = hipGetLastError();
    if (e != hipSuccess) fprintf(stderr, "[hs debug] %s(%d,%d,%d,%d) nbatch=%d maxni=%d maxnb=%d maxm=%d -> %s\n", what, a, b, c, d, nbatch, maxni, maxnb, maxm, hipGetErrorString(e));
  }

  static int env_int(const char* name, int dflt) {
    const char* e = getenv(name);
    return e ? atoi(e) : dflt;
  }
  int rows_of(int mat) const { return mat == HS_MAT_LF ? maxm : (mat == HS_MAT_UR ? maxni : maxnb); }
  int cols_of(int mat) const { return mat == HS_MAT_LF ? maxni : maxnb; }

  std::vector<std::pair<int, int>> kcol;
  std::vector<long long> kpre;
  void gemm(int cmat, int bmat, int r0, int r1, int c0, int c1, int k0, int k1, int cap = 0) {
    GemmOp op{cmat, bmat, r0, r1, c0, c1, k0, k1, 0, cap, hiprio, env ? 1 : 0};
    int M = std::min(r1, rows_of(cmat)) - r0, N = std::min(c1, cols_of(cmat)) - c0, K = std::min(k1, maxni) - k0;
    if (M <= 0 || N <= 0 || K <= 0) return;
    double fl = 0.0;
    bool clipped = false;
    long long live = 0;
    int route = (sizeof(T) == 8 && aligned16 && h_ni) ? HS_GEMM_ROUTE_LDS : HS_GEMM_ROUTE_REG;
    bool shifted = false;
    if (h_ni) {
      for (int i = 0; i < nbatch; ++i) {
        int ni = h_ni[i], nb = h_nb[i], m = ni + nb;
        int rows = cmat == HS_MAT_LF ? m : (cmat == HS_MAT_UR ? ni : nb), cols = cmat == HS_MAT_LF ? ni : nb;
        double Mi = std::min(r1, rows) - r0, Ni = std::min(c1, cols) - c0, Ki = std::min(k1, ni) - k0;
        if (Mi > 0 && Ni > 0 && Ki > 0) {
          route = hs_gemm_lds_route_join(route, hs_gemm_lds_route(cmat, r0, k0, k1, ni));
          shifted = shifted || ((r0 + (cmat == HS_MAT_SB ? ni : 0)) & 1);
          if (env && h_env && h_env[i]) {
            const int BMh = 128, BNh = sizeof(T) == 16 ? 64 : 128;
            const int M_ = (int)Mi, N_ = (int)Ni, kend = k0 + (int)Ki;
            const int* fL = h_env[i];
            const int* fU = fL + hs_env_block(m - 1, ni) + 1;
            const int row0 = r0 + (cmat == HS_MAT_SB ? ni : 0), col0 = c0 + (cmat == HS_MAT_LF ? 0 : ni);
            const int tn_ = (N_ + BNh - 1) / BNh;
            kcol.clear();
            long long ncols = 0;
            int kc_min = HS_ENV_NONE;
            for (int tn = 0; tn < tn_; ++tn) {
              const int kc = hs_env_min(fU, ni, col0 + tn * BNh, col0 + std::min(N_, (tn + 1) * BNh));
              if (kc >= kend) continue;
              kcol.push_back({kc, std::min(BNh, N_ - tn * BNh)});
              kc_min = std::min(kc_min, kc);
            }
            std::sort(kcol.begin(), kcol.end());
            kpre.assign(2 * (kcol.size() + 1), 0);
            for (size_t j = 0; j < kcol.size(); ++j) {
              kpre[2 * (j + 1)] = kpre[2 * j] + kcol[j].second;
              kpre[2 * (j + 1) + 1] = kpre[2 * j + 1] + (long long)kcol[j].second * kcol[j].first;
            }
            ncols = kpre[2 * kcol.size()];
            const long long ncolsk = kpre[2 * kcol.size() + 1];
            long long macs = 0, nrows = 0, rd = 0;
            int kr_min = HS_ENV_NONE;
            for (int m0 = 0; m0 < M_ && ncols > 0; m0 += BMh) {
              const int mt = std::min(BMh, M_ - m0);
              const int kr = std::max(k0, hs_env_min(fL, ni, row0 + m0, row0 + m0 + mt));
              if (kr >= kend) continue;
              const size_t j = std::upper_bound(kcol.begin(), kcol.end(), std::make_pair(kr, INT_MAX)) - kcol.begin();
              macs += mt * (kpre[2 * j] * (kend - kr) + (ncols - kpre[2 * j]) * kend - (ncolsk - kpre[2 * j + 1]));
              nrows += mt;
              rd += (long long)mt * (kend - std::max(kr, kc_min));
              kr_min = std::min(kr_min, kr);
            }
            fl += 2.0 * (double)macs;
            clipped = clipped || macs != (long long)M_ * N_ * (kend - k0);
            live += (long long)((nrows + BMh - 1) / BMh) * (long long)kcol.size();
            if (nrows > 0)
              for (const auto& c : kcol) rd += (long long)c.second * (kend - std::max(c.first, kr_min));
            pf->gemm_bytes += (2.0 * (double)nrows * (double)ncols + (double)rd) * sizeof(T);
            continue;
          }
          fl += 2.0 * Mi * Ni * Ki;
          pf->gemm_bytes += (Mi * Ki + Ki * Ni + 2.0 * Mi * Ni) * sizeof(T);
          live += (long long)(((int)Mi + 127) / 128) * (((int)Ni + (sizeof(T) == 16 ? 63 : 127)) / (sizeof(T) == 16 ? 64 : 128));
        }
      }
      if (sizeof(T) == 16) fl *= 4.0;
    }
    if (env && h_ni && !clipped) op.env = 0;
    hipEvent_t e0 = pf->begin(s);
    launch_gemm_op<T>(dn, nbatch, M, N, op, s, route, shifted, op.env ? live : -1);
    pf->end(e0, HS_CAT_GEMM, s, fl, M, N, K, nbatch, 0, hiprio);
    dbg("gemm", cmat, r0, c0, k0);
  }
  void panel(int pb, int fuse = 0) {
    int c0 = pb * HS_PB;
    if (c0 >= maxni) return;
    static const int big = env_int("HS_TOUR_BIG", 0);
    hipEvent_t e0 = pf->begin(s);
    if (optimistic) {
      fuse |= 4;
    } else if (big) {
      const int BR = hs_tour_block_rows(sizeof(T) == 16);
      int cnt = (maxpiv > 0 ? maxpiv : maxni) - c0, nblk = (cnt + BR - 1) / BR;
      for (int stage = 0;; ++stage) {
        launch_tournament_stage<T>(dn, nbatch, pb, stage, nblk, s);
        dbg("tournament", pb, stage, nblk);
        if (nblk == 1) break;
        cnt = nblk * HS_PB;
        nblk = (cnt + BR - 1) / BR;
      }
    } else {
      int cnt = (maxpiv > 0 ? maxpiv : maxni) - c0, nch = (cnt + HS_CHUNK - 1) / HS_CHUNK;
      for (int round = 0;; ++round) {
        launch_tournament_round<T>(dn, nbatch, pb, round, nch, s);
        dbg("tournament", pb, round, nch);
        if (nch == 1) break;
        cnt = nch * HS_PB;
        nch = (cnt + HS_CHUNK - 1) / HS_CHUNK;
      }
    }
    launch_panel_pivot<T>(dn, nbatch, pb, fuse, s);
    dbg("panel_pivot", pb);
    launch_panel_l21<T>(dn, nbatch, pb, std::min(maxm, rlim) - c0, fuse, s, rlim);
    dbg("panel_l21", pb);
    pf->end(e0, HS_CAT_PANEL, s, 0.0, 0, 0, 0, nbatch, 0, hiprio);
  }
  void laswp(int mat, int c0, int c1, int k0, int k1) {
    int nc = std::min(c1, cols_of(mat)) - c0;
    if (nc <= 0 || k0 >= maxni) return;
    hipEvent_t e0 = pf->begin(s);
    launch_laswp<T>(dn, nbatch, mat, c0, c1, k0, k1, nc, s);
    pf->end(e0, HS_CAT_LASWP, s, 0.0, 0, 0, 0, nbatch, 0, hiprio);
    dbg("laswp", mat, c0, k0, k1);
  }
  bool sym_on() const { return sym && optimistic && rlim == HS_BIG; }
  static int sym_strip(int extent, long long tiles_m, int bn) {
    const int lo = HS_SYM_STRIP * std::max(1, (extent + 16 * HS_SYM_STRIP - 1) / (16 * HS_SYM_STRIP));
    const int hi = std::max(lo, extent / 4 / HS_SYM_STRIP * HS_SYM_STRIP);
    const long long units = (1024LL * bn + HS_SYM_STRIP * std::max(1LL, tiles_m) - 1) / (HS_SYM_STRIP * std::max(1LL, tiles_m));
    return (int)std::min<long long>(hi, std::max<long long>(lo, HS_SYM_STRIP * units));
  }
  bool gemm_lower(int cmat, int bmat, int c0, int c1, int k0, int k1, int cap = 0) {
    c1 = std::min(c1, cols_of(cmat));
    if (c1 <= c0) return false;
    long long tiles_m = 0;
    for (int i = 0; i < nbatch; ++i) {
      const int rows = !h_ni ? rows_of(cmat) : (cmat == HS_MAT_LF ? h_ni[i] + h_nb[i] : h_nb[i]);
      tiles_m += std::max(0, rows - c0 + 127) / 128;
    }
    const int W = sym_strip(c1 - c0, tiles_m, sizeof(T) == 16 ? 64 : 128);
    for (int j0 = c0; j0 < c1; j0 += W) gemm(cmat, bmat, j0, HS_BIG, j0, std::min(c1, j0 + W), k0, k1, cap);
    return c1 - c0 > W;
  }
  void transpose(int mat, int r0, int r1, int c0, int c1, bool lower) {
    const int lim = mat == HS_MAT_LF ? maxni : maxnb;
    const int nr = std::min(r1, lim) - r0, nc = std::min(c1, lim) - c0;
    if (nr <= 0 || nc <= 0) return;
    hipEvent_t e0 = pf->begin(s);
    launch_sym_transpose<T>(dn, nbatch, mat, r0, r1, c0, c1, lower ? 1 : 0, nr, nc, s);
    pf->end(e0, HS_CAT_LASWP, s, 0.0, 0, 0, 0, nbatch, 0, hiprio);
    dbg("sym_transpose", mat, r0, c0, lower);
  }
  double trsm_bytes(int mat, bool below, int blk0, int blkw, int f0, int f1, int rd_hi, int wr_lo, int wr_hi) const {
    if (!pf->on || !h_ni) return 0.0;
    double b = 0.0;
    for (int i = 0; i < nbatch; ++i) {
      const int ni = h_ni[i], nb = h_nb[i];
      const int w = std::min(blkw, ni - blk0);
      const int ext = std::min(f1, below ? ni + nb : (mat == HS_MAT_LF ? ni : nb)) - f0;
      if (w <= 0 || ext <= 0) continue;
      b += (double)ext * (std::min(rd_hi, w) + std::max(0, std::min(wr_hi, w) - wr_lo)) * sizeof(T);
    }
    return b;
// ... 87 lines not shown
    if (c1 - c0 == 256 && diag_first()) {
      hipEvent_t eg = pf->begin(s);
      if (launch_group256<T>(dn, nbatch, c0 / 256, s)) {
        pf->end(eg, HS_CAT_PANEL, s, 0.0, 0, 0, 0, nbatch, 0, hiprio);
        dbg("group256", c0);
      } else {
        if (eg) (void)hipEventDestroy(eg);
        rlim = c0 + 256;
        lu_rec_inner(c0, c1);
        rlim = HS_BIG;
      }
      launch_inv256<T>(sn, nbatch, maxni, s, c0 / 256);
      const int r0 = c0 + 256;
      if (r0 < maxm) {
        if (sizeof(T) == 8) {
          for (int code : {7, 8}) {
            GemmOp op{HS_MAT_LF, HS_MAT_LF, r0, HS_BIG, c0, c1, c0, c1, code, 0, hiprio, env ? 1 : 0};
            hipEvent_t e0 = pf->begin(s);
            launch_gemm_op<T>(dn, nbatch, maxm - r0, 128, op, s);
            pf->end(e0, HS_CAT_TRSM, s, 0.0, 0, 0, 0, nbatch, code, hiprio,
                    code == 7 ? trsm_bytes(HS_MAT_LF, true, c0, 256, r0, HS_BIG, 256, 128, 256) : trsm_bytes(HS_MAT_LF, true, c0, 256, r0, HS_BIG, 128, 0, 128));
            dbg("l_below", c0, r0, code);
          }
        } else {
          const int wl = std::min(256, maxni - c0);
          for (int q = (wl - 1) / 64; q >= 0; --q) {
            GemmOp op{HS_MAT_LF, HS_MAT_LF, r0, HS_BIG, c0, c1, c0, c1, 16 + q, 0, hiprio, env ? 1 : 0};
            hipEvent_t e0 = pf->begin(s);
            launch_gemm_op<T>(dn, nbatch, maxm - r0, 64, op, s);
            pf->end(e0, HS_CAT_TRSM, s);
            dbg("l_below", c0, r0, 16 + q);
          }
        }
      }
      return;
    }
    lu_rec_inner(c0, c1);
    if (sn && c1 - c0 == 256) launch_inv256<T>(sn, nbatch, maxni, s, c0 / 256);
  }
  void lu_rec_inner(int c0, int c1) {
    if (c1 - c0 == HS_PB) {
      panel(c0 / HS_PB);
      return;
    }
    static const int pair = env_int("HS_PANEL_PAIR", 1);
    if (pair && c1 - c0 == 2 * HS_PB) {
      panel(c0 / HS_PB, 1);
      if (c0 + HS_PB < maxni) panel(c0 / HS_PB + 1, 2);
      return;
    }
    int mid = (c0 + c1) / 2;
    lu_rec(c0, mid);
    if (mid < maxni) {
      laswp(HS_MAT_LF, mid, c1, c0, mid);
      trsm_rec(HS_MAT_LF, c0, mid, mid, c1);
      if (sym_on() && c1 - mid >= 256) {
        if (gemm_lower(HS_MAT_LF, HS_MAT_LF, mid, c1, c0, mid)) transpose(HS_MAT_LF, mid, c1, mid, c1, true);
      } else {
        gemm(HS_MAT_LF, HS_MAT_LF, mid, rlim, mid, c1, c0, mid);
      }
      lu_rec(mid, c1);
      laswp(HS_MAT_LF, c0, mid, mid, c1);
    }
  }
  void factor_fronts_lookahead(int NB) {
    Sched<T> mn = *this;
    Sched<T> side = *this;
    hipStream_t s_la = (nbatch == 1 && s2m) ? this->s_la : nullptr;
    hipStream_t s2 = s_la ? s2m : this->s2;
    hipEvent_t ev_main, ev_side;
    (void)hipEventCreateWithFlags(&ev_main, hipEventDisableTiming);
    (void)hipEventCreateWithFlags(&ev_side, hipEventDisableTiming);
    if (s_la) {
      mn.s = s_la;
      (void)hipEventRecord(ev_main, s);
      (void)hipStreamWaitEvent(s_la, ev_main, 0);
    }
    mn.s2 = nullptr;
    mn.s_la = nullptr;
    side.s = s2;
    side.s2 = nullptr;
    side.s_la = nullptr;
    side.hiprio = 1;
    if (s_la) {
      (void)hipStreamWaitEvent(s2, ev_main, 0);
      side.lu_rec(0, NB);
      (void)hipEventRecord(ev_side, s2);
      (void)hipStreamWaitEvent(mn.s, ev_side, 0);
    } else {
      mn.lu_rec(0, NB);
    }
    static const int cap_total = env_int("HS_LA_GEMM_CAP", 448);
    static const int cap_opt = env_int("HS_LA_CAP_OPT", 0);
    const int gcap = (cap_total > 0 && nbatch == 1 && (!optimistic || cap_opt)) ? cap_total : 0;
    hipEvent_t ev_iter[3];
    for (auto& e : ev_iter) (void)hipEventCreateWithFlags(&e, hipEventDisableTiming);
    int iter = 0;
    for (int c0 = 0; c0 < maxni; c0 += NB, ++iter) {
      const int c1 = c0 + NB, c2 = c1 + NB;
      const bool has_next = c1 < maxni;
      if (iter >= 3) (void)hipEventSynchronize(ev_iter[iter % 3]);
      if (has_next) {
        mn.laswp(HS_MAT_LF, c1, c2, c0, c1);
        mn.trsm_rec(HS_MAT_LF, c0, c1, c1, c2);
        mn.gemm(HS_MAT_LF, HS_MAT_LF, c1, HS_BIG, c1, c2, c0, c1);
        if (mn.sym_on()) {
          mn.transpose(HS_MAT_LF, c1, c2, c1, c2, true);
          mn.transpose(HS_MAT_LF, c2, HS_BIG, c1, c2, false);
        }
        (void)hipEventRecord(ev_main, mn.s);
        (void)hipStreamWaitEvent(s2, ev_main, 0);
        side.lu_rec(c1, c2);
        (void)hipEventRecord(ev_side, s2);
        mn.laswp(HS_MAT_LF, c2, HS_BIG, c0, c1);
        mn.trsm_rec(HS_MAT_LF, c0, c1, c2, HS_BIG);
        if (mn.sym_on())
          mn.gemm_lower(HS_MAT_LF, HS_MAT_LF, c2, HS_BIG, c0, c1, has_next ? gcap : 0);
        else
          mn.gemm(HS_MAT_LF, HS_MAT_LF, c1, HS_BIG, c2, HS_BIG, c0, c1, has_next ? gcap : 0);
      }
      if (maxnb > 0) {
        mn.laswp(HS_MAT_UR, 0, HS_BIG, c0, c1);
        mn.trsm_rec(HS_MAT_UR, c0, c1, 0, HS_BIG);
        mn.gemm(HS_MAT_UR, HS_MAT_UR, c1, HS_BIG, 0, HS_BIG, c0, c1, has_next ? gcap : 0);
      }
      if (has_next) (void)hipStreamWaitEvent(mn.s, ev_side, 0);
      (void)hipEventRecord(ev_iter[iter % 3], mn.s);
    }
    for (auto& e : ev_iter) (void)hipEventDestroy(e);
    for (int c0 = 0; c0 + NB < maxni; c0 += NB) mn.laswp(HS_MAT_LF, c0, c0 + NB, c0 + NB, HS_BIG);
    if (s_la) {
      (void)hipEventRecord(ev_main, s_la);
      (void)hipStreamWaitEvent(s, ev_main, 0);
    }
    if (maxnb > 0) schur_update();
    (void)hipEventDestroy(ev_main);
    (void)hipEventDestroy(ev_side);
  }
  void factor_fronts() {
    if (maxni <= 0) return;
    static const int la_min = env_int("HS_LA_MIN", sizeof(T) == 16 ? 1200 : 1536), la_nb = env_int("HS_LA_NB", sizeof(T) == 16 ? 512 : 1024);
    const bool la_inv_ok = !sn || la_nb >= 256;
    if (s2 && la_nb >= HS_PB && (la_nb & (la_nb - 1)) == 0 && maxni >= la_min && maxni > la_nb && la_inv_ok) {
      hs_lookahead_note();
      factor_fronts_lookahead(la_nb);
      return;
    }
    int P2 = HS_PB;
    while (P2 < maxni) P2 *= 2;
    lu_rec(0, P2);
    if (sn && P2 < 256) launch_inv256<T>(sn, nbatch, maxni, s, 0);
    if (maxnb > 0) {
      laswp(HS_MAT_UR, 0, HS_BIG, 0, P2);
      trsm_rec(HS_MAT_UR, 0, P2, 0, HS_BIG);
      schur_update();
    }
  }
  void schur_update() {
    if (sym_on()) {
      gemm_lower(HS_MAT_SB, HS_MAT_UR, 0, HS_BIG, 0, HS_BIG);
      transpose(HS_MAT_SB, 0, HS_BIG, 0, HS_BIG, true);
    } else {
      gemm(HS_MAT_SB, HS_MAT_UR, 0, HS_BIG, 0, HS_BIG, 0, HS_BIG);
    }
  }
};
// ... 2 lines not shown
```

### hierarchicalsolvers.jl_amd/csrc/hs_testhooks.hip

```cpp
#include <algorithm>
#include <atomic>
#include <cstring>
#include <chrono>
#include <vector>

#include "../../include/hs_kernels.h"
#include "hs_host.h"
#include "hs_sched.h"
#include "hs_envelope.h"
#include "hs_lowrank.h"
#include "hs_solve_multi.h"
#include "hs_sweep.h"

namespace {
void need_device() {
  int cnt = 0;
  if (hipGetDeviceCount(&cnt) != hipSuccess || cnt <= 0) HS_FAIL(HS_ERR_DEVICE, 0, "no HIP device available");
}
size_t rup32(size_t e) { return (e + 31) / 32 * 32; }
template <class T>
T* put_block(HsDevBuf& buf, const T* src, int64_t ld, int64_t rows, int64_t cols) {
  const int64_t r = std::max<int64_t>(rows, 1);
  T* d = buf.get<T>((size_t)(r * std::max<int64_t>(cols, 1)));
  if (src && rows > 0 && cols > 0) HS_HIP(hipMemcpy2D(d, r * sizeof(T), src, ld * sizeof(T), rows * sizeof(T), cols, hipMemcpyHostToDevice));
// ... 111 lines not shown
  time_repeats(repeat, ms_out, [&] { sch.gemm(HS_MAT_UR, HS_MAT_UR, r0, HS_BIG, 0, HS_BIG, k0, k1); });
  prof.collect();
}
extern "C" int hsk_gemm_op_d(int64_t count, const int64_t* M, const int64_t* N, int64_t K, int64_t koff, int64_t roff, const double* A,
                             const double* B, double* C, int64_t* routed, int repeat, double* ms_out) {
  HS_GUARD(gemm_op_hook(count, M, N, K, koff, roff, A, B, C, routed, repeat, ms_out));
}

static void gemm_schur_hook(int64_t count, const int64_t* ni_, const int64_t* nb_, const double* A, const double* B, double* C, int env,
                            int64_t* routed_lds, int64_t* routed_edge, int repeat, double* ms_out) {
  typedef double T;
  const bool data = A && B && C;
  if (count <= 0 || count > 65535 || !ni_ || !nb_ || (!data && (A || B || C)) || (env && !data))
    HS_FAIL(HS_ERR_ARGUMENT, count, "hsk_gemm_schur_d: count in [1, 65535], ni and nb non-null, A, B, C all given or all null (env needs them) required");
  for (int64_t f = 0; f < count; ++f)
    if (ni_[f] <= 0 || nb_[f] <= 0 || ni_[f] + nb_[f] > (1 << 20))
      HS_FAIL(HS_ERR_ARGUMENT, f, "hsk_gemm_schur_d: front %lld has ni = %lld, nb = %lld", (long long)f, (long long)ni_[f], (long long)nb_[f]);
  need_device();
  auto even = [](int v) { return (v + 1) / 2 * 2; };
  std::vector<NodeDesc<T>> hn(count);
  std::vector<int> h_ni(count), h_nb(count);
  std::vector<size_t> olf(count), our(count), osb(count), oenv(count);
  size_t nT = 0, nE = 0;
  int maxni = 0, maxnb = 0, maxm = 0;
  for (int64_t f = 0; f < count; ++f) {
    const int ni = (int)ni_[f], nb = (int)nb_[f];
    h_ni[f] = ni; h_nb[f] = nb;
    maxni = std::max(maxni, ni); maxnb = std::max(maxnb, nb); maxm = std::max(maxm, ni + nb);
    olf[f] = nT; nT += rup32((size_t)even(ni + nb) * ni);
    our[f] = nT; nT += rup32((size_t)even(ni) * nb);
    osb[f] = nT; nT += rup32((size_t)even(nb) * nb);
    oenv[f] = nE; nE += 2 * (size_t)hs_env_nblocks(ni, nb);
  }
  HsDevBuf buf("hsk_gemm_schur_d");
  T* dbuf = buf.get<T>(nT);
  NodeDesc<T>* dn = buf.get<NodeDesc<T>>((size_t)count);
  HS_HIP(hipMemsetD32(dbuf, 0x3F800000, 2 * nT));
  std::vector<int> henv(env ? nE : 0);
  std::vector<const int*> h_envp(count, nullptr);
  int* denv = env ? buf.get<int>(nE) : nullptr;
  bool aligned = true;
  const T *Af = A, *Bf = B;
  T* Cf = C;
  for (int64_t f = 0; f < count; ++f) {
    NodeDesc<T>& d = hn[f];
    memset(&d, 0, sizeof d);
    d.ni = h_ni[f]; d.nb = h_nb[f]; d.m = d.ni + d.nb;
    d.ldl = even(d.m); d.ldu = even(d.ni); d.lds = even(d.nb);
    d.LF = dbuf + olf[f]; d.UR = dbuf + our[f]; d.SB = dbuf + osb[f];
    d.ni1 = d.ni; d.nb1 = d.nb; d.node = (int)f;
    const int ni = d.ni, nb = d.nb;
    if (env) {
      const int nI = (ni + 31) / 32, nblk = hs_env_nblocks(ni, nb);
      int* fL = henv.data() + oenv[f];
      int* fU = fL + nblk;
      for (int b = 0; b < nblk; ++b) fL[b] = fU[b] = b < nI ? 32 * b : HS_ENV_NONE;
      for (int k = 0; k < ni; ++k)
        for (int r = 0; r < nb; ++r)
          if (Af[(size_t)r + (size_t)k * nb] != 0.0) { int& v = fL[nI + r / 32]; v = std::min(v, k & ~31); }
      for (int c = 0; c < nb; ++c)
        for (int k = 0; k < ni; ++k)
          if (Bf[(size_t)k + (size_t)c * ni] != 0.0) { int& v = fU[nI + c / 32]; v = std::min(v, k & ~31); break; }
      d.env = denv + oenv[f];
      h_envp[f] = fL;
    }
    d.finalize();
    aligned = aligned && !((((uintptr_t)d.LF | (uintptr_t)d.UR | (uintptr_t)d.SB) & 15) || ((d.ldl | d.ldu | d.lds) & 1));
    if (data) {
      HS_HIP(hipMemcpy2D(d.LF + ni, sizeof(T) * d.ldl, Af, sizeof(T) * nb, sizeof(T) * nb, ni, hipMemcpyHostToDevice));
      HS_HIP(hipMemcpy2D(d.UR, sizeof(T) * d.ldu, Bf, sizeof(T) * ni, sizeof(T) * ni, nb, hipMemcpyHostToDevice));
      HS_HIP(hipMemcpy2D(d.SB, sizeof(T) * d.lds, Cf, sizeof(T) * nb, sizeof(T) * nb, nb, hipMemcpyHostToDevice));
      Af += (size_t)nb * ni; Bf += (size_t)ni * nb; Cf += (size_t)nb * nb;
    }
  }
  if (env) HS_HIP(hipMemcpy(denv, henv.data(), sizeof(int) * nE, hipMemcpyHostToDevice));
  HS_HIP(hipMemcpy(dn, hn.data(), sizeof(NodeDesc<T>) * count, hipMemcpyHostToDevice));
  Profiler prof;
  Sched<T> sch{dn, (int)count, maxni, maxnb, maxm, (hipStream_t) nullptr, &prof, h_ni.data(), h_nb.data()};
  sch.aligned16 = aligned;
  if (env) {
    sch.optimistic = true;
    sch.env = true;
    sch.h_env = h_envp.data();
  }
  const long long lds0 = hsk_gemm_lds_launches(0), edge0 = hsk_gemm_lds_edge_launches(0);
  sch.gemm(HS_MAT_SB, HS_MAT_UR, 0, HS_BIG, 0, HS_BIG, 0, HS_BIG);
  HS_HIP(hipDeviceSynchronize());
  if (routed_lds) *routed_lds = (int64_t)(hsk_gemm_lds_launches(0) - lds0);
  if (routed_edge) *routed_edge = (int64_t)(hsk_gemm_lds_edge_launches(0) - edge0);
  if (data) {
    Cf = C;
    for (int64_t f = 0; f < count; ++f) {
      const NodeDesc<T>& d = hn[f];
      bring_block(Cf, d.nb, d.SB, d.lds, d.nb, d.nb);
      Cf += (size_t)d.nb * d.nb;
    }
  }
  time_repeats(repeat, ms_out, [&] { sch.gemm(HS_MAT_SB, HS_MAT_UR, 0, HS_BIG, 0, HS_BIG, 0, HS_BIG); });
  prof.collect();
}
extern "C" int hsk_gemm_schur_d(int64_t count, const int64_t* ni, const int64_t* nb, const double* A, const double* B, double* C, int env,
                                int64_t* routed_lds, int64_t* routed_edge, int repeat, double* ms_out) {
  HS_GUARD(gemm_schur_hook(count, ni, nb, A, B, C, env, routed_lds, routed_edge, repeat, ms_out));
}

static void trsm_inv_hook(int64_t count, const int64_t* ni_, const int64_t* nb_, int64_t r0, int64_t c0, int64_t c1, int64_t ldpad, int64_t shift,
                          const double* inv, double* X, int env, int64_t* strips) {
  typedef double T;
  if (count <= 0 || count > 65535 || !ni_ || !nb_ || !inv || !X || r0 < 0 || (r0 & 255) || c0 < 0 || c1 <= c0 || ldpad < 0 || shift < 0 || shift > 1)
    HS_FAIL(HS_ERR_ARGUMENT, count, "hsk_trsm_inv_d: count in [1, 65535], r0 a multiple of 256, 0 <= c0 < c1, ldpad >= 0, shift 0 or 1 and non-null arrays required");
  for (int64_t f = 0; f < count; ++f)
    if (ni_[f] <= 0 || nb_[f] <= 0 || ni_[f] + nb_[f] > (1 << 20))
      HS_FAIL(HS_ERR_ARGUMENT, f, "hsk_trsm_inv_d: front %lld has ni = %lld, nb = %lld", (long long)f, (long long)ni_[f], (long long)nb_[f]);
  need_device();
  std::vector<NodeDesc<T>> hn(count);
  std::vector<SolveNode<T>> hs(count);
  std::vector<int> h_ni(count), h_nb(count);
  std::vector<size_t> our(count), oenv(count);
  size_t nT = 0, nE = 0;
  int maxni = 0, maxnb = 0, maxm = 0;
  const size_t nblk = (size_t)(r0 / 256) + 1;
  for (int64_t f = 0; f < count; ++f) {
    const int ni = (int)ni_[f], nb = (int)nb_[f];
    h_ni[f] = ni; h_nb[f] = nb;
    maxni = std::max(maxni, ni); maxnb = std::max(maxnb, nb); maxm = std::max(maxm, ni + nb);
    our[f] = nT + (size_t)shift; nT += rup32((size_t)(ni + ldpad) * nb + 2);
    oenv[f] = nE; nE += 2 * (size_t)hs_env_nblocks(ni, nb);
  }
  HsDevBuf buf("hsk_trsm_inv_d");
  T* dbuf = buf.get<T>(nT);
  T* dinv = buf.get<T>((size_t)count * nblk * 65536);
  NodeDesc<T>* dn = buf.get<NodeDesc<T>>((size_t)count);
  SolveNode<T>* dsn = buf.get<SolveNode<T>>((size_t)count);
  HS_HIP(hipMemsetD32(dbuf, 0x3F800000, 2 * nT));
  HS_HIP(hipMemsetD32(dinv, 0x3F800000, 2 * (size_t)count * nblk * 65536));
  std::vector<int> henv(env ? nE : 0);
  std::vector<const int*> h_envp(count, nullptr);
  int* denv = env ? buf.get<int>(nE) : nullptr;
  const T* Xf = X;
  for (int64_t f = 0; f < count; ++f) {
    NodeDesc<T>& d = hn[f];
    memset(&d, 0, sizeof d);
    memset(&hs[f], 0, sizeof hs[f]);
    const int ni = h_ni[f], nb = h_nb[f];
    d.ni = ni; d.nb = nb; d.m = ni + nb;
    d.ldl = d.m; d.ldu = ni + (int)ldpad; d.lds = nb;
    d.UR = dbuf + our[f];
    d.inv256L = dinv + (size_t)f * nblk * 65536;
    d.ni1 = ni; d.nb1 = nb; d.node = (int)f;
    if (env) {
      const int nI = (ni + 31) / 32, nb_all = hs_env_nblocks(ni, nb);
      int* fL = henv.data() + oenv[f];
      int* fU = fL + nb_all;
      for (int b = 0; b < nb_all; ++b) fL[b] = fU[b] = b < nI ? 32 * b : HS_ENV_NONE;
      for (int c = 0; c < nb; ++c)
        for (int k = 0; k < ni; ++k)
          if (Xf[(size_t)k + (size_t)c * ni] != 0.0) { int& v = fU[nI + c / 32]; v = std::min(v, k & ~31); break; }
      d.env = denv + oenv[f];
      h_envp[f] = fL;
    }
    d.finalize();
    d.mrows[HS_MAT_LF] = d.mcols[HS_MAT_LF] = d.mrows[HS_MAT_SB] = d.mcols[HS_MAT_SB] = 0;
    HS_HIP(hipMemcpy2D(d.UR, sizeof(T) * d.ldu, Xf, sizeof(T) * ni, sizeof(T) * ni, nb, hipMemcpyHostToDevice));
    HS_HIP(hipMemcpy(d.inv256L + (nblk - 1) * 65536, inv + (size_t)f * 65536, sizeof(T) * 65536, hipMemcpyHostToDevice));
    Xf += (size_t)ni * nb;
  }
// ... 107 lines not shown
    d.ipiv = dint + x.ip;
    d.rperm = d.ipiv + x.ni;
    d.info = d.rperm + x.ni;
    d.growth = d.info + 1;
    d.cand0 = dint + x.cand;
    d.cand1 = d.cand0 + x.ncand;
    d.pivlist = d.cand1 + x.ncand;
    d.ni = x.ni; d.nb = x.nb; d.m = x.m;
    d.ldl = x.ldl; d.ldu = x.ldu; d.lds = x.lds;
    d.ni1 = x.ni; d.nb1 = x.nb; d.isleaf = 1; d.node = (int)k;
    d.pivrows = x.ni;
    d.finalize();
    SolveNode<T>& q = hs[k];
    memset(&q, 0, sizeof q);
    q.LF = d.LF; q.UR = d.UR; q.invL = d.invL; q.invU = d.invU;
    q.inv256L = d.inv256L; q.inv256U = d.inv256U;
    q.rperm = d.rperm;
    q.ni = x.ni; q.nb = x.nb; q.m = x.m; q.ldl = x.ldl; q.ldu = x.ldu;
    q.mrows = x.m;
    const int m = x.m;
    if (x.ni > 0) HS_HIP(hipMemcpy2D(d.LF, sizeof(T) * x.ldl, Fk, sizeof(T) * m, sizeof(T) * m, x.ni, hipMemcpyHostToDevice));
    if (x.ni > 0 && x.nb > 0) HS_HIP(hipMemcpy2D(d.UR, sizeof(T) * x.ldu, Fk + (size_t)m * x.ni, sizeof(T) * m, sizeof(T) * x.ni, x.nb, hipMemcpyHostToDevice));
    if (x.nb > 0) HS_HIP(hipMemcpy2D(d.SB, sizeof(T) * x.lds, Fk + (size_t)m * x.ni + x.ni, sizeof(T) * m, sizeof(T) * x.nb, x.nb, hipMemcpyHostToDevice));
    Fk += (size_t)m * m;
  }
  HS_HIP(hipMemcpy(dn, hn.data(), sizeof(NodeDesc<T>) * count, hipMemcpyHostToDevice));
}

template <class T>
void FrontBatch<T>::set_env(const int32_t* env) {
  size_t nE = 0;
  for (int64_t k = 0; k < count; ++k) nE += 2 * (size_t)hs_env_nblocks(o[k].ni, o[k].nb);
  env_host.assign(env, env + nE);
  int* denv = buf.get<int>(nE);
  HS_HIP(hipMemcpy(denv, env_host.data(), sizeof(int) * nE, hipMemcpyHostToDevice));
  h_env.resize(count);
  size_t off = 0;
  for (int64_t k = 0; k < count; ++k) {
    hn[k].env = denv + off;
    h_env[k] = env_host.data() + off;
    off += 2 * (size_t)hs_env_nblocks(o[k].ni, o[k].nb);
  }
  HS_HIP(hipMemcpy(dn, hn.data(), sizeof(NodeDesc<T>) * count, hipMemcpyHostToDevice));
}

template <class T>
int FrontBatch<T>::aligned16_status() const {
  for (int64_t k = 0; k < count; ++k) {
    const NodeDesc<T>& d = hn[k];
    if ((((uintptr_t)d.LF | (uintptr_t)d.UR | (uintptr_t)d.SB) & 15) || ((d.ldl | d.ldu | d.lds) & 1)) {
      hs_set_error(HS_ERR_UNSUPPORTED, k, "front batch: LF / UR / SB of front %lld are not 16-byte aligned with even leading dimensions", (long long)k);
      return HS_ERR_UNSUPPORTED;
    }
  }
  return HS_OK;
}

template <class T>
void FrontBatch<T>::factor(int mode, double* ms_out, bool sym) {
  const bool aligned = (mode & 4) != 0;
  mode &= 3;
  if (aligned) HS_CHECK(aligned16_status());
  Profiler prof;
  struct Streams {
    hipStream_t main = nullptr, side = nullptr, la = nullptr, sidem = nullptr;
    ~Streams() {
      for (hipStream_t s : {main, side, la, sidem})
        if (s) (void)hipStreamDestroy(s);
    }
  } st;
  HsEvents<2> ev;
  HS_HIP(hipStreamCreate(&st.main));
  hs_create_lookahead_streams(&st.la, &st.sidem, &st.side);
  HS_HIP(hipEventRecord(ev[0], st.main));
  launch_init_fronts<T>(dn, (int)count, maxni, st.main);
  Sched<T> sch{dn, (int)count, maxni, maxnb, maxm, st.main, &prof, h_ni.data(), h_nb.data(), st.side, 0, st.la, st.sidem};
  if (mode >= 2) sch.sn = dsn;
  sch.optimistic = (mode == 1 || mode == 2);
  sch.aligned16 = aligned;
  sch.sym = sym && sch.optimistic;
  if (sch.optimistic && !h_env.empty()) {
    sch.env = true;
    sch.h_env = h_env.data();
  }
  const auto h0 = std::chrono::steady_clock::now();
  sch.factor_fronts();
  HS_HIP(hipEventRecord(ev[1], st.main));
  if (getenv("HS_HOOK_VERBOSE"))
    fprintf(stderr, "[hook] host enqueue time %.2f ms\n", std::chrono::duration<double, std::milli>(std::chrono::steady_clock::now() - h0).count());
  HS_HIP(hipEventSynchronize(ev[1]));
  float ms = 0.f;
  HS_HIP(hipEventElapsedTime(&ms, ev[0], ev[1]));
  if (ms_out) *ms_out = ms;
  HS_HIP(hipDeviceSynchronize());
}

template <class T>
void FrontBatch<T>::copy_out(T* outLF, T* outUR, T* outSB, int64_t* out_rperm, int64_t* info, int64_t* growth, T* outInvL, T* outInvU, T* outInv256L,
                             T* outInv256U) {
  std::vector<int> ip;
  size_t pLF = 0, pUR = 0, pSB = 0, pR = 0, pInv = 0, pInv256 = 0;
  for (int64_t k = 0; k < count; ++k) {
    const Off& x = o[k];
    const NodeDesc<T>& d = hn[k];
    const int ni = x.ni, nb = x.nb, m = x.m;
    if (ni > 0 && outLF) bring_block(outLF + pLF, m, d.LF, x.ldl, m, ni);
    if (ni > 0 && nb > 0 && outUR) bring_block(outUR + pUR, ni, d.UR, x.ldu, ni, nb);
    if (nb > 0 && outSB) bring_block(outSB + pSB, nb, d.SB, x.lds, nb, nb);
    ip.resize((size_t)ni + 2);
    HS_HIP(hipMemcpy(ip.data(), d.rperm, sizeof(int) * ((size_t)ni + 2), hipMemcpyDeviceToHost));
    if (out_rperm)
      for (int i = 0; i < ni; ++i) out_rperm[pR + i] = ip[i];
    if (info) info[k] = ip[ni];
    if (growth) growth[k] = ip[ni + 1];
    const size_t n32 = (size_t)x.nblk * HS_PB * HS_PB, n256 = (size_t)x.nb256 * 65536;
    if (outInvL && n32) HS_HIP(hipMemcpy(outInvL + pInv, d.invL, sizeof(T) * n32, hipMemcpyDeviceToHost));
    if (outInvU && n32) HS_HIP(hipMemcpy(outInvU + pInv, d.invU, sizeof(T) * n32, hipMemcpyDeviceToHost));
    if (outInv256L && n256) HS_HIP(hipMemcpy(outInv256L + pInv256, d.inv256L, sizeof(T) * n256, hipMemcpyDeviceToHost));
    if (outInv256U && n256) HS_HIP(hipMemcpy(outInv256U + pInv256, d.inv256U, sizeof(T) * n256, hipMemcpyDeviceToHost));
    pLF += (size_t)m * ni; pUR += (size_t)ni * nb; pSB += (size_t)nb * nb; pR += ni; pInv += n32; pInv256 += n256;
  }
}

template <class T>
static void front_batch_hook(int64_t count, const int64_t* ni_, const int64_t* nb_, int mode, const T* F, T* outLF, T* outUR, T* outSB,
                             int64_t* out_rperm, int64_t* info, int64_t* growth, T* outInvL, T* outInvU, T* outInv256L, T* outInv256U,
                             double* ms_out, const int32_t* env = nullptr, bool sym = false) {
  FrontBatch<T>::check(sym ? "hsk_front_batch_sym" : "hsk_front_batch", count, ni_, nb_, F, mode, 0, 7);
  if (sym && mode != 1 && mode != 2 && mode != (2 | 4))
    HS_FAIL(HS_ERR_ARGUMENT, mode, "hsk_front_batch_sym: the symmetric schedule runs under optimistic pivoting only (modes 1, 2 and 2 | 4)");
  if (env && (mode & 3) != 1 && (mode & 3) != 2) HS_FAIL(HS_ERR_ARGUMENT, mode, "hsk_front_batch_env: block envelopes hold under optimistic pivoting only (modes 1, 2)");
  if ((outInvL || outInvU || outInv256L || outInv256U) && (mode & 3) < 2)
    HS_FAIL(HS_ERR_ARGUMENT, mode, "hsk_front_batch: the stored inverses are returned by modes 2 and 3 only");
  FrontBatch<T> fb;
  fb.setup(count, ni_, nb_, F);
  if (env) fb.set_env(env);
  fb.upload_solve();
  fb.factor(mode, ms_out, sym);
  fb.copy_out(outLF, outUR, outSB, out_rperm, info, growth, outInvL, outInvU, outInv256L, outInv256U);
}

template <class T>
static void sweep_level_hook(int64_t count, const int64_t* ni_, const int64_t* nb_, int mode, const T* F, const int64_t* flags, int64_t n,
                             const int64_t* fidx, const T* b, int path, int trans, int tall, T* outLF, T* outUR, int64_t* out_rperm, int64_t* info,
                             int64_t* growth, T* outInvL, T* outInvU, T* outInv256L, T* outInv256U, T* out_y, T* out_bfwd, T* out_x, T* out_bbwd,
                             int* tall_used) {
  const char* name = "hsk_sweep_level";
  FrontBatch<T>::check(name, count, ni_, nb_, F, mode, 2);
  if (!fidx || !b || n <= 0 || n > 0x7fffffff || path < 0 || path > 2 || trans < 0 || trans > 2 || tall < -1 || tall > 1)
    HS_FAIL(HS_ERR_ARGUMENT, 0, "%s: fidx and b non-null, n in [1, 2^31), path in 0..2, trans in 0..2 and tall in -1..1 required", name);
  if (path == 2 && trans != 0) HS_FAIL(HS_ERR_ARGUMENT, trans, "%s: the 32-column sweeps (path 2) exist for trans = 0 only", name);
  if (trans == 2 && sizeof(T) == 8) HS_FAIL(HS_ERR_ARGUMENT, trans, "%s: trans = 2 (adjoint) is for ComplexF64; Float64 has trans = 1", name);
  size_t nidx = 0;
  for (int64_t k = 0; k < count; ++k) nidx += (size_t)(ni_[k] + nb_[k]);
  std::vector<int> hidx(nidx + 1, 0);
  {
    std::vector<char> seen((size_t)n, 0);
    for (size_t p = 0; p < nidx; ++p) {
      if (fidx[p] < 0 || fidx[p] >= n || seen[(size_t)fidx[p]])
        HS_FAIL(HS_ERR_ARGUMENT, (int64_t)p, "%s: fidx[%lld] = %lld is outside 0:%lld or occurs twice (the fronts of a level are disjoint)", name,
                (long long)p, (long long)fidx[p], (long long)n - 1);
      seen[(size_t)fidx[p]] = 1;
      hidx[p] = (int)fidx[p];
    }
  }
  FrontBatch<T> fb;
// ... 825 lines not shown
```

### hierarchicalsolvers.jl_amd/csrc/kernels_gemm.hip

```cpp
#include <atomic>
#include <mutex>
#include <vector>
#include <algorithm>
#include <initializer_list>
#include <cstdio>
#include <cstdlib>
#include <cstring>
#include "hs_common.h"

typedef double double4_t __attribute__((ext_vector_type(4)));
typedef hs_d2u double2_u;

template <class T>
struct TileCfg;
template <>
struct TileCfg<double> {
  static constexpr int BM = 128, BN = 128;
  static constexpr int BK = 16;
  static constexpr int LDA = 144;
  static constexpr int LDB = 18;
  static constexpr int A_IMG = BK * LDA;
  static constexpr int STAGE = A_IMG + BN * LDB;
  static constexpr int STAGE_LDS = A_IMG + BN * BK;
  static constexpr int smem_doubles = 2 * STAGE;
  static constexpr int smem_doubles_lds = 2 * STAGE_LDS;
};
template <>
struct TileCfg<cplx> {
  static constexpr int BM = 128, BN = 64;
  static constexpr int BK = 16;
  static constexpr int LDA = 144;
  static constexpr int LDB = 18;
  static constexpr int smem_doubles = 2 * BK * LDA + 2 * BN * LDB;
};

__host__ __device__ inline int xcd_remap(int bid, int nwg) {
  int q = nwg >> 3, r = nwg & 7, x = bid & 7, o = bid >> 3;
  int base = (x < r) ? x * (q + 1) : r * (q + 1) + (x - r) * q;
  return base + o;
}
__host__ __device__ inline int xcd_remap_shift(int bid, int nwg, int shift) {
  if (shift == 0) return xcd_remap(bid, nwg);
  const int x = (bid + shift) & 7;
  int base = 0;
#pragma unroll
  for (int xx = 0; xx < 8; ++xx) {
    const int first = (xx - shift) & 7;
    const int cnt = first < nwg ? (nwg - first + 7) >> 3 : 0;
    base += (xx < x) ? cnt : 0;
  }
  return base + ((bid - ((x - shift) & 7)) >> 3);
}

__host__ __device__ inline void tile_coords(int t, int tiles_m, int tiles_n, int& tm, int& tn) {
  const int GROUP_M = 8;
  int per_group = GROUP_M * tiles_n;
  int g = t / per_group;
  int first_m = g * GROUP_M;
  int gm = min(tiles_m - first_m, GROUP_M);
  int in_g = t - g * per_group;
  tm = first_m + in_g % gm;
  tn = in_g / gm;
}

__host__ __device__ inline int env_order_stride(int T) {
  if (T <= 8) return 1;
  const int s0 = (T * 40503 + 32768) >> 16;
  for (int d = 0;; ++d)
    for (int s = s0 - d; s <= s0 + d; s += (d ? 2 * d : 1)) {
      int a = s, b = T;
      while (b) { const int r = a % b; a = b; b = r; }
      if (a == 1) return s;
    }
}
__host__ __device__ inline void env_order_apply(int& tm, int& tn, int tiles_m, int tiles_n, int sm, int sn) {
  if (sm > 1) tm = tm * sm % tiles_m;
  if (sn > 1) tn = tn * sn % tiles_n;
}

template <class T, bool ENV>
__device__ inline bool resolve_op(const NodeDesc<T>* pn, const GemmOp& op, GemmProb<T>& p, EnvClip* ep) {
  EnvClip e_unused;
  EnvClip& e = ENV ? *ep : e_unused;
  T *cp, *bp;
  int ldc, ldb, crows, ccols, brows, bcols;
  mat_of(pn, op.cmat, cp, ldc, crows, ccols);
  mat_of(pn, op.bmat, bp, ldb, brows, bcols);
  const int ni = pn->ni, ldl = pn->ldl;
  T* const LF = pn->LF;
  const int* env = nullptr;
  const int* envU = nullptr;
  if constexpr (ENV) {
    env = op.env ? pn->env : nullptr;
    envU = env ? env + hs_env_block(pn->m - 1, ni) + 1 : nullptr;
    e.fL = e.fU = nullptr;
    e.ni = ni;
    e.row0 = op.r0 + (op.cmat == HS_MAT_SB ? ni : 0);
    e.col0 = op.c0 + (op.cmat == HS_MAT_LF ? 0 : ni);
    e.kbase = op.k0;
  }
  if (op.ainv >= 16) {
    const int q = op.ainv - 16;
    const int wl = min(256, ni - op.k0);
    const int M = min(op.r1, crows) - op.r0;
    const int N = min(64, wl - 64 * q);
    if (wl <= 0 || M <= 0 || N <= 0 || q > 3) return false;
    const T* V = pn->inv256U + (size_t)(op.k0 / 256) * 65536;
    T* X = LF + (size_t)op.r0 + (size_t)op.k0 * ldl;
    p.A = X; p.B = V + (size_t)(64 * q) * 256; p.C = X + (size_t)(64 * q) * ldl;
    p.M = M; p.N = N; p.K = min(wl, 64 * (q + 1));
    p.lda = ldl; p.ldb = 256; p.ldc = ldl;
    p.flag = pn->growth;
    p.flag_rows = pn->pivrows - op.r0;
    if constexpr (ENV) e.fL = env;
    return true;
  }
  if (op.ainv >= 7) {
    const int wl = min(256, ni - op.k0);
    const int M = min(op.r1, crows) - op.r0;
    if (wl <= 0 || M <= 0) return false;
    const T* V = pn->inv256U + (size_t)(op.k0 / 256) * 65536;
    T* X = LF + (size_t)op.r0 + (size_t)op.k0 * ldl;
    if (op.ainv == 7) {
      if (wl <= 128) return false;
      p.A = X; p.B = V + (size_t)128 * 256; p.C = X + (size_t)128 * ldl;
      p.M = M; p.N = wl - 128; p.K = wl;
    } else {
      p.A = X; p.B = V; p.C = X;
      p.M = M; p.N = min(128, wl); p.K = min(128, wl);
    }
    p.lda = ldl; p.ldb = 256; p.ldc = ldl;
    p.flag = pn->growth;
    p.flag_rows = pn->pivrows - op.r0;
    if constexpr (ENV) e.fL = env;
    return true;
  }
  if (op.ainv >= 3) {
    const int wl = min(256, ni - op.r0);
    const int N = min(op.c1, ccols) - op.c0;
    if (wl <= 0 || N <= 0) return false;
    const bool up = op.ainv >= 5;
    const T* inv = (up ? pn->inv256U : pn->inv256L) + (size_t)(op.r0 / 256) * 65536;
    const bool second_half_rows = (op.ainv == 3 || op.ainv == 6);
    const bool full_k = (op.ainv == 3 || op.ainv == 5);
    const int ro = second_half_rows ? 128 : 0;
    const int M = min(128, wl - ro);
    if (M <= 0) return false;
    const int ko = (op.ainv == 6) ? 128 : 0;
    const int K = full_k ? wl : (op.ainv == 4 ? min(128, wl) : wl - 128);
    if (K <= 0) return false;
    p.A = inv + ro + (size_t)ko * 256;
    p.B = cp + (size_t)(op.r0 + ko) + (size_t)op.c0 * ldc;
    p.C = cp + (size_t)(op.r0 + ro) + (size_t)op.c0 * ldc;
    p.M = M; p.N = N; p.K = K;
    p.lda = 256; p.ldb = ldc; p.ldc = ldc;
    if constexpr (ENV)
      if (!up) { e.fU = envU; e.kbase = op.r0; }
    return true;
  }
  if (op.ainv) {
// ... 518 lines not shown
            acci[i][j] = __builtin_amdgcn_mfma_f64_16x16x4f64(bfr[j][ks], afi[ks], acci[i][j], 0, 0, 0);
          }
          __builtin_amdgcn_sched_barrier(0);
        }
      }
    }
    __syncthreads();
    if (more) {
      store_tile();
      __syncthreads();
    }
  }
  cplx* __restrict__ C = p.C;
#pragma unroll
  for (int i = 0; i < 4; ++i) {
    const int mm = m0 + wm * 64 + i * 16 + l15;
    const bool rok = mm < M;
    double2_u cv[2][4];
#pragma unroll
    for (int j = 0; j < 2; ++j)
#pragma unroll
      for (int r = 0; r < 4; ++r) {
        const int nn = n0 + wn * 32 + j * 16 + l4 + 4 * r;
        double2_u o = {0.0, 0.0};
        if (minus && rok && nn < N) o = gld2(C + (size_t)mm + (size_t)nn * p.ldc);
        cv[j][r] = o;
      }
#pragma unroll
    for (int j = 0; j < 2; ++j)
#pragma unroll
      for (int r = 0; r < 4; ++r) {
        const int nn = n0 + wn * 32 + j * 16 + l4 + 4 * r;
        if (rok && nn < N) {
          double2_u v = {accr[i][j][r], acci[i][j][r]};
          if (minus) {
            v.x = cv[j][r].x - v.x;
            v.y = cv[j][r].y - v.y;
          }
          gst2(C + (size_t)mm + (size_t)nn * p.ldc, v);
          if (p.flag && mm < p.flag_rows && !(fabs(v.x) + fabs(v.y) <= HS_GROWTH_MAX)) *p.flag = 1;
        }
      }
  }
}

__device__ double g_op_flops;

enum class Tile {
  Reg,
  Lds,
  LdsEdge,
};
template <class T>
struct TileWalk {
  int tiles_m, tiles_n, ntiles, shift;
  __device__ __forceinline__ TileWalk(int M, int N) {
    tiles_m = (M + TileCfg<T>::BM - 1) / TileCfg<T>::BM, tiles_n = (N + TileCfg<T>::BN - 1) / TileCfg<T>::BN;
    ntiles = tiles_m * tiles_n;
    shift = (int)((gridDim.x * blockIdx.y) & 7u);
  }
  __device__ __forceinline__ void coords(int bid, int& tm, int& tn) const {
    int t = xcd_remap_shift(bid, ntiles, (gridDim.x & 7u) ? shift : 0);
    tile_coords(t, tiles_m, tiles_n, tm, tn);
  }
  __device__ __forceinline__ bool more(int bid) const { return bid + (int)gridDim.x < ntiles; }
};
template <class T, Tile TILE = Tile::Reg>
__device__ inline void gemm_dispatch(const GemmProb<T>& p, bool minus, double* smem, int mlo = 0) {
  const TileWalk<T> w(p.M, p.N);
  for (int bid = blockIdx.x; bid < w.ntiles; bid += gridDim.x) {
    int tm, tn;
    w.coords(bid, tm, tn);
    if constexpr (sizeof(T) == 16)
      gemm_tile_z(p, tm, tn, minus, smem);
    else if constexpr (TILE == Tile::Reg)
      gemm_tile_d(p, tm, tn, minus, smem);
    else
      gemm_tile_d_lds<TILE == Tile::LdsEdge>(p, tm, tn, minus, smem, mlo);
    if (w.more(bid)) __syncthreads();
  }
}

template <class T, Tile TILE = Tile::Reg>
__device__ inline void gemm_dispatch_env(GemmProb<T>& p, bool minus, double* smem, const EnvClip* e, int count, int order, int mlo = 0) {
  const TileWalk<T> w(p.M, p.N);
  const int sm = order ? env_order_stride(w.tiles_m) : 1, sn = order ? env_order_stride(w.tiles_n) : 1;
  bool ran = false;
  for (int bid = blockIdx.x; bid < w.ntiles; bid += gridDim.x) {
    int tm, tn;
    w.coords(bid, tm, tn);
    env_order_apply(tm, tn, w.tiles_m, w.tiles_n, sm, sn);
    int dk = 0;
    {
      const int m_lo = tm * TileCfg<T>::BM, n_lo = tn * TileCfg<T>::BN;
      const int m_hi = min(m_lo + TileCfg<T>::BM, p.M), n_hi = min(n_lo + TileCfg<T>::BN, p.N);
      if (e->fL || e->fU) {
        dk = hs_env_kstart(*e, m_lo, m_hi, n_lo, n_hi) - e->kbase;
        if (dk >= p.K) continue;
      }
      if (count && threadIdx.x == 0)
        atomicAdd(&g_op_flops, (sizeof(T) == 16 ? 8.0 : 2.0) * (double)(m_hi - m_lo) * (double)(n_hi - n_lo) * (double)(p.K - dk));
    }
    const size_t da = (size_t)dk * p.lda;
    p.A += da;
    p.B += dk;
    p.K -= dk;
    if (ran) __syncthreads();
    ran = true;
    if constexpr (sizeof(T) == 16)
      gemm_tile_z(p, tm, tn, minus, smem);
    else if constexpr (TILE == Tile::Reg)
      gemm_tile_d(p, tm, tn, minus, smem);
    else
      gemm_tile_d_lds<true>(p, tm, tn, minus, smem, mlo);
    p.A -= da;
    p.B -= dk;
    p.K += dk;
  }
}

template <class T, bool TRSM>
__device__ __forceinline__ bool op_prologue(const NodeDesc<T>* __restrict__ nodes, const GemmOp& op, GemmProb<T>& p) {
  if (TRSM || op.prio) __builtin_amdgcn_s_setprio(2);
  return resolve_op<T, false>(nodes + blockIdx.y, op, p, nullptr);
}
template <class T>
__global__ __launch_bounds__(256, 2) void gemm_op_kernel(const NodeDesc<T>* __restrict__ nodes, GemmOp op) {
  extern __shared__ __attribute__((aligned(16))) double smem[];
  GemmProb<T> p;
  if (!op_prologue<T, false>(nodes, op, p)) return;
  gemm_dispatch<T>(p, true, smem);
}
template <class T>
__global__ __launch_bounds__(256, 2) void gemm_op_lds_kernel(const NodeDesc<T>* __restrict__ nodes, GemmOp op) {
  static_assert(sizeof(T) == 8, "real double only");
  extern __shared__ __attribute__((aligned(16))) double smem[];
  GemmProb<T> p;
  if (!op_prologue<T, false>(nodes, op, p)) return;
  gemm_dispatch<T, Tile::Lds>(p, true, smem);
}
__device__ inline int edge_shift_rows(GemmProb<double>& p) {
  if (!((uintptr_t)p.A & 15)) return 0;
  p.A -= 1;
  p.C -= 1;
  p.M += 1;
  p.flag_rows += 1;
  return 1;
}
template <class T>
__global__ __launch_bounds__(256, 2) void gemm_op_lds_edge_kernel(const NodeDesc<T>* __restrict__ nodes, GemmOp op) {
  static_assert(sizeof(T) == 8, "real double only");
  extern __shared__ __attribute__((aligned(16))) double smem[];
  GemmProb<T> p;
  if (!op_prologue<T, false>(nodes, op, p)) return;
  const int mlo = edge_shift_rows(p);
  gemm_dispatch<T, Tile::LdsEdge>(p, true, smem, mlo);
}
template <class T>
__global__ __launch_bounds__(256, 2) void trsm_inv_kernel(const NodeDesc<T>* __restrict__ nodes, GemmOp op) {
  extern __shared__ __attribute__((aligned(16))) double smem[];
  GemmProb<T> p;
  if (!op_prologue<T, true>(nodes, op, p)) return;
  gemm_dispatch<T>(p, false, smem);
}
template <class T>
__global__ __launch_bounds__(256, 2) void gemm_op_env_kernel(const NodeDesc<T>* __restrict__ nodes, GemmOp op) {
  extern __shared__ __attribute__((aligned(16))) double smem[];
  GemmProb<T> p;
  EnvClip e;
  if (op.prio) __builtin_amdgcn_s_setprio(2);
  if (op.ainv) return;
  if (!resolve_op<T, true>(nodes + blockIdx.y, op, p, &e)) return;
  gemm_dispatch_env<T>(p, true, smem, &e, op.count, op.order);
}
template <class T>
__global__ __launch_bounds__(256, 2) void gemm_op_env_lds_kernel(const NodeDesc<T>* __restrict__ nodes, GemmOp op) {
  static_assert(sizeof(T) == 8, "real double only");
  extern __shared__ __attribute__((aligned(16))) double smem[];
  GemmProb<T> p;
  EnvClip e;
  if (op.prio) __builtin_amdgcn_s_setprio(2);
  if (op.ainv) return;
  if (!resolve_op<T, true>(nodes + blockIdx.y, op, p, &e)) return;
  const int mlo = edge_shift_rows(p);
  e.row0 -= mlo;
  gemm_dispatch_env<T, Tile::LdsEdge>(p, true, smem, &e, 0, op.order, mlo);
}
template <class T>
__global__ __launch_bounds__(256, 2) void trsm_inv_env_kernel(const NodeDesc<T>* __restrict__ nodes, GemmOp op) {
  extern __shared__ __attribute__((aligned(16))) double smem[];
  GemmProb<T> p;
  EnvClip e;
  __builtin_amdgcn_s_setprio(2);
  if (!op.ainv) return;
  if (!resolve_op<T, true>(nodes + blockIdx.y, op, p, &e)) return;
  gemm_dispatch_env<T>(p, false, smem, &e, 0, 0);
}

__device__ double g_probs_flops;
template <class T>
__global__ __launch_bounds__(256, 2) void gemm_probs_kernel(const GemmProb<T>* __restrict__ probs, int minus) {
  extern __shared__ __attribute__((aligned(16))) double smem[];
  GemmProb<T> p = probs[blockIdx.y];
  if (p.M <= 0 || p.N <= 0) return;
  if ((minus & 2) && blockIdx.x == 0 && threadIdx.x == 0) atomicAdd(&g_probs_flops, (sizeof(T) == 16 ? 8.0 : 2.0) * p.M * (double)p.N * p.K);
  gemm_dispatch<T>(p, (minus & 1) != 0, smem);
}
__global__ __launch_bounds__(256, 2) void gemm_probs_skinny_kernel(const GemmProb<double>* __restrict__ probs, int minus) {
  extern __shared__ __attribute__((aligned(16))) double smem[];
  GemmProb<double> p = probs[blockIdx.y];
  if (p.M <= 0 || p.N <= 0) return;
  if ((minus & 2) && blockIdx.x == 0 && threadIdx.x == 0) atomicAdd(&g_probs_flops, 2.0 * p.M * (double)p.N * p.K);
  minus &= 1;
  if (p.M <= 64 && p.N > 64) {
    const int tn_ = (p.N + 127) / 128;
    for (int bid = blockIdx.x; bid < tn_; bid += gridDim.x) {
      gemm_tile_s_d<64, 128>(p, 0, bid, minus != 0, smem);
      if (bid + (int)gridDim.x < tn_) __syncthreads();
    }
    return;
  }
  const int tm_ = (p.M + 63) / 64, tn_ = (p.N + 63) / 64, nt = tm_ * tn_;
  for (int bid = blockIdx.x; bid < nt; bid += gridDim.x) {
    gemm_tile_s_d<64, 64>(p, bid % tm_, bid / tm_, minus != 0, smem);
    if (bid + (int)gridDim.x < nt) __syncthreads();
  }
}

template <class T>
__global__ void resolve_dump_kernel(const NodeDesc<T>* __restrict__ nodes, GemmOp op, GemmProb<T>* out, int* ok) {
  GemmProb<T> p;
  memset(&p, 0, sizeof p);
  ok[blockIdx.x] = resolve_op<T, false>(nodes + blockIdx.x, op, p, nullptr) ? 1 : 0;
  out[blockIdx.x] = p;
}

namespace {
std::atomic<int> g_env_on{-1};
std::atomic<int> g_benv_on{-1};
std::atomic<int> g_env_order_on{-1};
std::atomic<int> g_op_count_on{0};
std::atomic<int> g_lds_on{-1};
std::atomic<long long> g_lds_launches{0};
std::atomic<long long> g_lds_edge_launches{0};
std::atomic<long long> g_reg_launches{0};
}
static bool gemm_lds_enabled() {
  int v = g_lds_on.load(std::memory_order_relaxed);
  if (v < 0) {
    const char* e = getenv("HS_GEMM_LDS");
    v = (e && e[0] == '0') ? 0 : 1;
    g_lds_on.store(v);
  }
  return v != 0;
}
extern "C" int hsk_gemm_lds_enable(int on) {
  const int prev = gemm_lds_enabled() ? 1 : 0;
  g_lds_on.store(on ? 1 : 0);
  return prev;
}
extern "C" long long hsk_gemm_lds_launches(int reset) {
  return reset ? g_lds_launches.exchange(0) : g_lds_launches.load();
}
extern "C" long long hsk_gemm_lds_edge_launches(int reset) {
  return reset ? g_lds_edge_launches.exchange(0) : g_lds_edge_launches.load();
}
extern "C" long long hsk_gemm_reg_launches(int reset) {
  return reset ? g_reg_launches.exchange(0) : g_reg_launches.load();
}
extern "C" int hsk_gemm_lds_route(int cmat, int r0, int k0, int k1, int ni) { return hs_gemm_lds_route(cmat, r0, k0, k1, ni); }
bool hs_envelope_enabled() {
  int v = g_env_on.load();
  if (v < 0) {
    const char* e = getenv("HS_LEAF_ENVELOPE");
    v = (e && e[0] == '0') ? 0 : 1;
    g_env_on.store(v);
  }
  return v != 0;
}
extern "C" int hsk_envelope_enable(int on) {
  const int prev = hs_envelope_enabled() ? 1 : 0;
  g_env_on.store(on ? 1 : 0);
  return prev;
}
bool hs_branch_envelope_enabled() {
  int v = g_benv_on.load();
  if (v < 0) {
    const char* e = getenv("HS_BRANCH_ENVELOPE");
    v = (e && e[0] == '0') ? 0 : 1;
    g_benv_on.store(v);
  }
  return v != 0;
}
extern "C" int hsk_branch_envelope_enable(int on) {
  const int prev = hs_branch_envelope_enabled() ? 1 : 0;
  g_benv_on.store(on ? 1 : 0);
  return prev;
}
static bool env_order_enabled() {
  int v = g_env_order_on.load(std::memory_order_relaxed);
  if (v < 0) {
    const char* e = getenv("HS_ENV_ORDER");
    v = (e && e[0] == '0') ? 0 : 1;
    g_env_order_on.store(v);
  }
  return v != 0;
}
extern "C" int hsk_env_order_enable(int on) {
  const int prev = env_order_enabled() ? 1 : 0;
  g_env_order_on.store(on ? 1 : 0);
  return prev;
}
extern "C" int hsk_env_tile_order(int tiles_m, int tiles_n, int order, int32_t* tm, int32_t* tn) {
  if (tiles_m <= 0 || tiles_n <= 0 || tiles_m > 32768 || tiles_n > 32768 || !tm || !tn || (long long)tiles_m * tiles_n > (1 << 24)) return -1;
  const int ntiles = tiles_m * tiles_n;
  const int sm = order ? env_order_stride(tiles_m) : 1, sn = order ? env_order_stride(tiles_n) : 1;
  for (int bid = 0; bid < ntiles; ++bid) {
    int m, n;
    tile_coords(xcd_remap_shift(bid, ntiles, 0), tiles_m, tiles_n, m, n);
    env_order_apply(m, n, tiles_m, tiles_n, sm, sn);
    tm[bid] = m;
    tn[bid] = n;
  }
  return 0;
}
extern "C" int hsk_op_flops_mode(int on) {
  (void)hipDeviceSynchronize();
  g_op_count_on.store(on ? 1 : 0);
  const double z = 0.0;
  return hipMemcpyToSymbol(HIP_SYMBOL(g_op_flops), &z, sizeof z) == hipSuccess ? 0 : -6;
}
extern "C" int hsk_op_flops(double* out) {
  if (!out) return -1;
  if (hipDeviceSynchronize() != hipSuccess) return -6;
  return hipMemcpyFromSymbol(out, HIP_SYMBOL(g_op_flops), sizeof *out) == hipSuccess ? 0 : -6;
}

template <class T>
static void dump_resolved_op(const NodeDesc<T>* dnodes, int nbatch, int maxM, int maxN, const GemmOp& op, hipStream_t s) {
  GemmProb<T>* dp;
  int* dok;
  (void)hipMalloc((void**)&dp, sizeof(GemmProb<T>) * nbatch);
  (void)hipMalloc((void**)&dok, sizeof(int) * nbatch);
  hipLaunchKernelGGL(resolve_dump_kernel<T>, dim3(nbatch), dim3(1), 0, s, dnodes, op, dp, dok);
  (void)hipStreamSynchronize(s);
  GemmProb<T> hp;
  int hok;
  NodeDesc<T> hn;
  for (int i = 0; i < nbatch && i < 4; ++i) {
    (void)hipMemcpy(&hp, dp + i, sizeof hp, hipMemcpyDeviceToHost);
    (void)hipMemcpy(&hok, dok + i, sizeof hok, hipMemcpyDeviceToHost);
    (void)hipMemcpy(&hn, dnodes + i, sizeof hn, hipMemcpyDeviceToHost);
    fprintf(stderr, "[hs debug] gemm op c%d b%d r[%d,%d) c[%d,%d) k[%d,%d) node%d: ok=%d A=%p B=%p C=%p M=%d N=%d K=%d ld=%d,%d,%d | LF=%p UR=%p SB=%p ni=%d nb=%d m=%d ld=%d,%d,%d maxM=%d maxN=%d\n",
            op.cmat, op.bmat, op.r0, op.r1, op.c0, op.c1, op.k0, op.k1, i, hok, (void*)hp.A, (void*)hp.B, (void*)hp.C, hp.M, hp.N, hp.K, hp.lda,
            hp.ldb, hp.ldc, (void*)hn.LF, (void*)hn.UR, (void*)hn.SB, hn.ni, hn.nb, hn.m, hn.ldl, hn.ldu, hn.lds, maxM, maxN);
  }
  (void)hipFree(dp);
  (void)hipFree(dok);
}

template <class K>
static void opt_in_lds(std::once_flag& once, std::initializer_list<K> kernels, int lds_bytes) {
  std::call_once(once, [&] {
    for (K k : kernels) (void)hipFuncSetAttribute((const void*)k, hipFuncAttributeMaxDynamicSharedMemorySize, lds_bytes);
  });
}

template <class T>
struct OpKernel {
  void (*fn)(const NodeDesc<T>*, GemmOp);
  int lds_bytes;
  std::atomic<long long>* launches;
};
template <class T>
static OpKernel<T> pick_op_kernel(const GemmOp& op, int route) {
  constexpr int lds_reg = TileCfg<T>::smem_doubles * 8;
  if constexpr (sizeof(T) == 8) {
    constexpr int lds_direct = TileCfg<T>::smem_doubles_lds * 8;
    if (route == HS_GEMM_ROUTE_LDS) return {gemm_op_lds_kernel<T>, lds_direct, &g_lds_launches};
    if (route != HS_GEMM_ROUTE_REG) return {op.env ? gemm_op_env_lds_kernel<T> : gemm_op_lds_edge_kernel<T>, lds_direct, &g_lds_edge_launches};
  }
  std::atomic<long long>* const reg = (sizeof(T) == 8 && !op.ainv && !op.count) ? &g_reg_launches : nullptr;
  if (op.env || op.count) return {op.ainv ? trsm_inv_env_kernel<T> : gemm_op_env_kernel<T>, lds_reg, reg};
  return {op.ainv ? trsm_inv_kernel<T> : gemm_op_kernel<T>, lds_reg, reg};
}

template <class T>
void launch_gemm_op(const NodeDesc<T>* dnodes, int nbatch, int maxM, int maxN, const GemmOp& op_in, hipStream_t s, int route, bool shifted,
                    long long live_tiles) {
  if (nbatch <= 0 || maxM <= 0 || maxN <= 0) return;
  GemmOp op = op_in;
  op.count = (!op.ainv && g_op_count_on.load(std::memory_order_relaxed)) ? 1 : 0;
  op.order = (op.env && !op.ainv && env_order_enabled()) ? 1 : 0;
  static const bool dump = getenv("HS_DEBUG_SYNC") && getenv("HS_DEBUG_SYNC")[0] == '2';
  if (dump) dump_resolved_op(dnodes, nbatch, maxM, maxN, op, s);
  if (sizeof(T) != 8 || op.ainv || op.count || !gemm_lds_enabled()) route = HS_GEMM_ROUTE_REG;
  if (op.env && route == HS_GEMM_ROUTE_LDS) route = HS_GEMM_ROUTE_EDGE;
  if (route == HS_GEMM_ROUTE_EDGE && shifted) maxM += 1;
  int tiles = ((maxM + TileCfg<T>::BM - 1) / TileCfg<T>::BM) * ((maxN + TileCfg<T>::BN - 1) / TileCfg<T>::BN);
  if (op.cap > 0 && tiles > op.cap) tiles = std::max(8, op.cap / 8 * 8);
  if (op.env && !(op.cap > 0)) {
    static const int walk_max = getenv("HS_ENV_WALK") ? atoi(getenv("HS_ENV_WALK")) : 4;
    int walk = walk_max;
    if (live_tiles >= 0) walk = (int)std::min<long long>(walk, (long long)tiles * nbatch / std::max(1LL, live_tiles));
    if (walk > 1 && tiles >= 32 && (long long)tiles * nbatch >= 4096) tiles = std::max(8, tiles / walk / 8 * 8);
  }
  static std::once_flag once_reg;
  opt_in_lds(once_reg, {gemm_op_kernel<T>, trsm_inv_kernel<T>, gemm_op_env_kernel<T>, trsm_inv_env_kernel<T>}, TileCfg<T>::smem_doubles * 8);
  if constexpr (sizeof(T) == 8) {
    if (route != HS_GEMM_ROUTE_REG) {
      static std::once_flag once_direct;
      opt_in_lds(once_direct, {gemm_op_lds_kernel<T>, gemm_op_lds_edge_kernel<T>, gemm_op_env_lds_kernel<T>}, TileCfg<T>::smem_doubles_lds * 8);
    }
  }
  const OpKernel<T> k = pick_op_kernel<T>(op, route);
  if (k.launches) k.launches->fetch_add(1, std::memory_order_relaxed);
  hipLaunchKernelGGL(k.fn, dim3(tiles, nbatch), dim3(256), k.lds_bytes, s, dnodes, op);
}

namespace {
struct ProbsAcc {
  std::mutex mu;
  int mode = 0;
  long long launches = 0;
  std::vector<std::pair<hipEvent_t, hipEvent_t>> ev;
};
ProbsAcc& probs_acc() {
  static ProbsAcc* a = new ProbsAcc();
  return *a;
}
}
extern "C" int hs_probs_stats_mode(int mode) {
  ProbsAcc& a = probs_acc();
  std::lock_guard<std::mutex> lk(a.mu);
  (void)hipDeviceSynchronize();
  for (auto& e : a.ev) { (void)hipEventDestroy(e.first); (void)hipEventDestroy(e.second); }
  a.ev.clear();
  a.launches = 0;
  a.mode = mode;
  const double z = 0.0;
  return hipMemcpyToSymbol(HIP_SYMBOL(g_probs_flops), &z, sizeof z) == hipSuccess ? 0 : -6;
}
extern "C" int hs_probs_stats(double* out3) {
  if (!out3) return -1;
  ProbsAcc& a = probs_acc();
  std::lock_guard<std::mutex> lk(a.mu);
  if (hipDeviceSynchronize() != hipSuccess) return -6;
  double fl = 0.0, ms = 0.0;
  if (hipMemcpyFromSymbol(&fl, HIP_SYMBOL(g_probs_flops), sizeof fl) != hipSuccess) return -6;
  for (auto& e : a.ev) {
    float t = 0.f;
    if (hipEventElapsedTime(&t, e.first, e.second) == hipSuccess) ms += t;
  }
  out3[0] = fl; out3[1] = (double)a.launches; out3[2] = ms * 1e-3;
  return 0;
}

template <class T>
void launch_gemm_probs(const GemmProb<T>* dprobs, int nprob, int maxM, int maxN, int minus, hipStream_t s) {
  if (nprob <= 0 || maxM <= 0 || maxN <= 0) return;
  minus = minus ? 1 : 0;
  hipEvent_t pe0 = nullptr, pe1 = nullptr;
  {
    ProbsAcc& a = probs_acc();
    if (a.mode) {
      std::lock_guard<std::mutex> lk(a.mu);
      a.launches++;
      minus |= 2;
      if (a.mode >= 2 && hipEventCreate(&pe0) == hipSuccess && hipEventCreate(&pe1) == hipSuccess) {
        (void)hipEventRecord(pe0, s);
        a.ev.push_back({pe0, pe1});
      } else {
        pe1 = nullptr;
      }
    }
  }
  struct Rec {
    hipEvent_t e; hipStream_t s;
    ~Rec() { if (e) (void)hipEventRecord(e, s); }
  } rec{pe1, s};
  int tiles = ((maxM + TileCfg<T>::BM - 1) / TileCfg<T>::BM) * ((maxN + TileCfg<T>::BN - 1) / TileCfg<T>::BN);
  constexpr int lds_bytes = TileCfg<T>::smem_doubles * 8;
  static std::once_flag once;
  opt_in_lds(once, {gemm_probs_kernel<T>}, lds_bytes);
  if constexpr (sizeof(T) == 8) {
    static const bool skinny = !(getenv("HS_GEMM_SKINNY") && getenv("HS_GEMM_SKINNY")[0] == '0');
    static const int small_tiles = getenv("HS_GEMM_SMALL_TILES") ? atoi(getenv("HS_GEMM_SMALL_TILES")) : 128;
    if (skinny && (maxM <= 64 || (long long)tiles * nprob <= small_tiles)) {
      if (maxM > 64) tiles = ((maxM + 63) / 64) * ((maxN + 63) / 64);
      static std::once_flag once_skinny;
      opt_in_lds(once_skinny, {gemm_probs_skinny_kernel}, lds_bytes);
      hipLaunchKernelGGL(gemm_probs_skinny_kernel, dim3(tiles, nprob), dim3(256), lds_bytes, s, (const GemmProb<double>*)dprobs, minus);
      return;
    }
  }
  hipLaunchKernelGGL(gemm_probs_kernel<T>, dim3(tiles, nprob), dim3(256), lds_bytes, s, dprobs, minus);
}

template void launch_gemm_op<double>(const NodeDesc<double>*, int, int, int, const GemmOp&, hipStream_t, int, bool, long long);
template void launch_gemm_op<cplx>(const NodeDesc<cplx>*, int, int, int, const GemmOp&, hipStream_t, int, bool, long long);
template void launch_gemm_probs<double>(const GemmProb<double>*, int, int, int, int, hipStream_t);
template void launch_gemm_probs<cplx>(const GemmProb<cplx>*, int, int, int, int, hipStream_t);
```

### include/hs_kernels.h

```cpp
#ifndef HS_KERNELS_H
#define HS_KERNELS_H
#include <stdint.h>
#include "hs_solver.h"
#ifdef __cplusplus
extern "C" {
#endif

int hsk_gemm_d(int64_t M, int64_t N, int64_t K, const double* A, int64_t lda, const double* B, int64_t ldb,
               double* C, int64_t ldc, int minus, int repeat, double* ms_out);
int hsk_gemm_z(int64_t M, int64_t N, int64_t K, const double* A, int64_t lda, const double* B, int64_t ldb,
               double* C, int64_t ldc, int minus, int repeat, double* ms_out);

int hsk_front_factor_d(int64_t count, int64_t ni, int64_t nb, const double* F, double* outLF, double* outUR,
                       double* outSB, int64_t* out_rperm, int64_t* info, double* ms_out);
int hsk_front_factor_z(int64_t count, int64_t ni, int64_t nb, const double* F, double* outLF, double* outUR,
                       double* outSB, int64_t* out_rperm, int64_t* info, double* ms_out);

long long hsk_lookahead_runs(int reset);
int hsk_front_batch_d(int64_t count, const int64_t* ni, const int64_t* nb, int mode, const double* F, double* outLF, double* outUR,
                      double* outSB, int64_t* out_rperm, int64_t* info, int64_t* growth, double* outInvL, double* outInvU,
                      double* outInv256L, double* outInv256U, double* ms_out);
int hsk_front_batch_z(int64_t count, const int64_t* ni, const int64_t* nb, int mode, const double* F, double* outLF, double* outUR,
                      double* outSB, int64_t* out_rperm, int64_t* info, int64_t* growth, double* outInvL, double* outInvU,
                      double* outInv256L, double* outInv256U, double* ms_out);
// ... 24 lines not shown

int hsk_qr_params(double* out4);
int hsk_qr_chol_d(int64_t njobs, const int32_t* b, const int32_t* first, const double* G, const double* thr, double* top, int32_t* p, double* L,
                  double* Linv, double* LinvP, double* d, int32_t* lperm, int32_t* nacc);
int hsk_qr_chol_z(int64_t njobs, const int32_t* b, const int32_t* first, const double* G, const double* thr, double* top, int32_t* p, double* L,
                  double* Linv, double* LinvP, double* d, int32_t* lperm, int32_t* nacc);
int hsk_qr_select(int64_t njobs, const int32_t* m, const int32_t* done, const int32_t* want, int32_t* p, const double* res2, double* outmax);
int hsk_qr_refine_d(int64_t njobs, const int32_t* m, const int32_t* q, const double* M, int32_t* p, const int32_t* rmax, const double* atol_scale,
                    const double* floor_abs, int norm_select, double atol, double rtol, double scale_floor, int32_t* r, double* top, double* d,
                    double* T, int32_t* blocks, int32_t* nblocks, int64_t* counters);
int hsk_qr_refine_z(int64_t njobs, const int32_t* m, const int32_t* q, const double* M, int32_t* p, const int32_t* rmax, const double* atol_scale,
                    const double* floor_abs, int norm_select, double atol, double rtol, double scale_floor, int32_t* r, double* top, double* d,
                    double* T, int32_t* blocks, int32_t* nblocks, int64_t* counters);

int hsk_multi_prob_d(int64_t M, int64_t K, int64_t kc, const double* A, int64_t lda, const double* X, int64_t ldx, double* C, int64_t ldc,
                     int minus, int trap, const int32_t* map);
int hsk_multi_prob_z(int64_t M, int64_t K, int64_t kc, const double* A, int64_t lda, const double* X, int64_t ldx, double* C, int64_t ldc,
                     int minus, int trap, const int32_t* map);

int hsk_multi_prob_t_d(int64_t M, int64_t K, int64_t kc, const double* A, int64_t lda, const double* X, int64_t ldx, double* C, int64_t ldc,
                       int minus, int trap, int conj, const int32_t* map);
int hsk_multi_prob_t_z(int64_t M, int64_t K, int64_t kc, const double* A, int64_t lda, const double* X, int64_t ldx, double* C, int64_t ldc,
                       int minus, int trap, int conj, const int32_t* map);

int hsk_multi_tri_d(int64_t M, int64_t K, int64_t kc, const double* A, int64_t lda, const double* X, int64_t ldx, double* C, int64_t ldc,
                    int plus, int tri, const int32_t* map);
int hsk_multi_tri_z(int64_t M, int64_t K, int64_t kc, const double* A, int64_t lda, const double* X, int64_t ldx, double* C, int64_t ldc,
                    int plus, int tri, const int32_t* map);
int hsk_multi_tri_t_d(int64_t M, int64_t K, int64_t kc, const double* A, int64_t lda, const double* X, int64_t ldx, double* C, int64_t ldc,
                      int plus, int tri, int conj, const int32_t* map);
int hsk_multi_tri_t_z(int64_t M, int64_t K, int64_t kc, const double* A, int64_t lda, const double* X, int64_t ldx, double* C, int64_t ldc,
                      int plus, int tri, int conj, const int32_t* map);

int hsk_multi_prob_f32_d(int64_t M, int64_t K, int64_t kc, const double* A, int64_t lda, const double* X, int64_t ldx, double* C, int64_t ldc,
                         int minus, int trap, const int32_t* map);
int hsk_multi_prob_f32_z(int64_t M, int64_t K, int64_t kc, const double* A, int64_t lda, const double* X, int64_t ldx, double* C, int64_t ldc,
                         int minus, int trap, const int32_t* map);
int hsk_multi_prob_t_f32_d(int64_t M, int64_t K, int64_t kc, const double* A, int64_t lda, const double* X, int64_t ldx, double* C, int64_t ldc,
                           int minus, int trap, int conj, const int32_t* map);
int hsk_multi_prob_t_f32_z(int64_t M, int64_t K, int64_t kc, const double* A, int64_t lda, const double* X, int64_t ldx, double* C, int64_t ldc,
                           int minus, int trap, int conj, const int32_t* map);
int hsk_round_factors_f32(hs_handle* F, int64_t* counts2);

int hsk_lu_product_d(int64_t nb, const double* LF, int64_t ldl, const int32_t* rperm, double* S, int64_t lds, double* flops_out);
int hsk_lu_product_z(int64_t nb, const double* LF, int64_t ldl, const int32_t* rperm, double* S, int64_t lds, double* flops_out);

int hsk_ulv_t_group_d(int64_t njobs, const int64_t* desc, const double* Abuf, int64_t na, const double* Xbuf, int64_t nx, double* Cbuf, int64_t nc, int conj);
int hsk_ulv_t_group_z(int64_t njobs, const int64_t* desc, const double* Abuf, int64_t na, const double* Xbuf, int64_t nx, double* Cbuf, int64_t nc, int conj);

int hsk_spmm_d(int64_t n, const int64_t* colptr, const int64_t* rowval, const double* nzval, const double* X, int64_t ldx, const double* B, int64_t ldb, double* Y,
               int64_t ldy, int64_t nrhs);
int hsk_spmm_z(int64_t n, const int64_t* colptr, const int64_t* rowval, const double* nzval, const double* X, int64_t ldx, const double* B, int64_t ldb, double* Y,
               int64_t ldy, int64_t nrhs);

int hsk_spmm_op_d(int trans, int64_t n, const int64_t* colptr, const int64_t* rowval, const double* nzval, const double* X, int64_t ldx, const double* B, int64_t ldb,
                  double* Y, int64_t ldy, int64_t nrhs);
int hsk_spmm_op_z(int trans, int64_t n, const int64_t* colptr, const int64_t* rowval, const double* nzval, const double* X, int64_t ldx, const double* B, int64_t ldb,
                  double* Y, int64_t ldy, int64_t nrhs);

int hsk_sddmm_d(int64_t n, const int64_t* colptr, const int64_t* rowval, int64_t kc, const double* L, int64_t ldl, const double* R, int64_t ldr, int swap, int conjl,
                int conjr, int diag, int form, double* G, double* seconds);
int hsk_sddmm_z(int64_t n, const int64_t* colptr, const int64_t* rowval, int64_t kc, const double* L, int64_t ldl, const double* R, int64_t ldr, int swap, int conjl,
                int conjr, int diag, int form, double* G, double* seconds);

int hsk_gn_rhs_d(int trans, int64_t n, const int64_t* colptr, const int64_t* rowval, const double* E, int pattern, const double* X, int64_t ldx, int64_t kc, double* P,
                 int64_t ldp);
int hsk_gn_rhs_z(int trans, int64_t n, const int64_t* colptr, const int64_t* rowval, const double* E, int pattern, const double* X, int64_t ldx, int64_t kc, double* P,
                 int64_t ldp);
int hsk_gn_rowsq_d(int64_t n, int64_t kc, const double* X, int64_t ldx, double* acc);
int hsk_gn_rowsq_z(int64_t n, int64_t kc, const double* X, int64_t ldx, double* acc);

int hsk_bisect_perm(int64_t n, const int64_t* colptr, const int64_t* rowval, int64_t ni, const int64_t* ids, int64_t* perm_out);

int hs_probs_stats_mode(int mode);
int hs_probs_stats(double* out3);

int hsk_leaf_envelope(int64_t n, const int64_t* colptr, const int64_t* rowval, const int32_t* fidx, int64_t ni, int64_t nb, int32_t* firstL, int32_t* firstU);
int hsk_branch_envelope(int64_t n, const int64_t* colptr, const int64_t* rowval, const int32_t* fidx, int64_t ni, int64_t nb, int64_t ni1, int64_t nb1,
                        int32_t* firstL, int32_t* firstU);
int hsk_envelope_enable(int on);
int hsk_branch_envelope_enable(int on);
int hsk_env_order_enable(int on);
int hsk_env_tile_order(int tiles_m, int tiles_n, int order, int32_t* tm, int32_t* tn);
int hsk_op_flops_mode(int on);
int hsk_op_flops(double* out);

int hsk_gemm_op_d(int64_t count, const int64_t* M, const int64_t* N, int64_t K, int64_t koff, int64_t roff, const double* A, const double* B,
                  double* C, int64_t* routed, int repeat, double* ms_out);
int hsk_gemm_lds_enable(int on);
long long hsk_gemm_lds_launches(int reset);
long long hsk_gemm_lds_edge_launches(int reset);
long long hsk_gemm_reg_launches(int reset);
int hsk_gemm_lds_route(int cmat, int r0, int k0, int k1, int ni);

int hsk_gemm_schur_d(int64_t count, const int64_t* ni, const int64_t* nb, const double* A, const double* B, double* C, int env,
                     int64_t* routed_lds, int64_t* routed_edge, int repeat, double* ms_out);

int hsk_trsm_inv_d(int64_t count, const int64_t* ni, const int64_t* nb, int64_t r0, int64_t c0, int64_t c1, int64_t ldpad, int64_t shift,
                   const double* inv, double* X, int env, int64_t* strips);
int hsk_trsm_strip_enable(int on);
long long hsk_trsm_strip_launches(int reset);
long long hsk_trsm_half_launches(int reset);

int hsk_mod_inner_d(int64_t n, int64_t k, int64_t m, const double* P, int64_t ldp, const double* Y, int64_t ldy, int conj, double* T, int64_t ldt);
int hsk_mod_inner_z(int64_t n, int64_t k, int64_t m, const double* P, int64_t ldp, const double* Y, int64_t ldy, int conj, double* T, int64_t ldt);
int hsk_mod_apply_d(int64_t n, int64_t k, int64_t m, double* Y, int64_t ldy, const double* Z, int64_t ldz, const double* T, int64_t ldt, int conj);
int hsk_mod_apply_z(int64_t n, int64_t k, int64_t m, double* Y, int64_t ldy, const double* Z, int64_t ldz, const double* T, int64_t ldt, int conj);
int hsk_mod_gather_d(int64_t n, int64_t k, int64_t m, const double* Y, int64_t ldy, const int64_t* J, double* T, int64_t ldt);
int hsk_mod_gather_z(int64_t n, int64_t k, int64_t m, const double* Y, int64_t ldy, const int64_t* J, double* T, int64_t ldt);
int hsk_mod_cap_d(int64_t k, int64_t m, const double* C, int64_t ldc, int op, double* T, int64_t ldt);
int hsk_mod_cap_z(int64_t k, int64_t m, const double* C, int64_t ldc, int op, double* T, int64_t ldt);

int hsk_eigs_rotate_d(int64_t n, int64_t K, int64_t N, const double* V, int64_t ldv, const double* Q, int64_t ldq, int inplace, double* Out, int64_t ldo);
int hsk_eigs_rotate_z(int64_t n, int64_t K, int64_t N, const double* V, int64_t ldv, const double* Q, int64_t ldq, int inplace, double* Out, int64_t ldo);
int hsk_eigs_chol_inv_d(int64_t p, const double* G, int64_t ldg, double* R, double* Rinv, int* info);
int hsk_eigs_chol_inv_z(int64_t p, const double* G, int64_t ldg, double* R, double* Rinv, int* info);
int hsk_small_eig_z(int64_t m, const double* H, int64_t ldh, double* w, double* Y, int64_t ldy);
int hsk_eigs_coldot_d(int64_t n, int64_t nc, const double* X, int64_t ldx, const double* Y, int64_t ldy, const int* pair, double* d);
int hsk_eigs_coldot_z(int64_t n, int64_t nc, const double* X, int64_t ldx, const double* Y, int64_t ldy, const int* pair, double* d);
int hsk_eigs_phase_timing(int on);
int hsk_eigs_phases(double* out4);
double hsk_eigs_gen_mprod_seconds(void);

double hsk_flow_pingpong_us(int peer, int iters);
double hsk_mfma_f64_peak(int waves_per_simd, int iters);
double hsk_mfma_f64_peak_random(int waves_per_simd, int iters);

#ifdef __cplusplus
}
#endif
#endif
```

Before: 2.133 s.

## Order envelope GEMM tiles by sorted envelope keys via device-built permutation tables

Adds a small pre-kernel that, for large envelope-clipped Schur GEMMs on the LDS-edge route, sorts row and column tiles by their envelope start, groups them into 8x8 units ordered by cost, and writes a per-front tile permutation table. The GEMM kernel then reads tile coordinates from this table in place of the strided ordering, so that tiles with similar work run together and the tile-to-XCD assignment is more balanced. This is the new default order setting. It costs one extra kernel launch per qualifying GEMM and device memory for the tables, and it only applies above a minimum tile count.

```diff
diff --git a/hierarchicalsolvers.jl_amd/_lib.py b/hierarchicalsolvers.jl_amd/_lib.py
--- a/hierarchicalsolvers.jl_amd/_lib.py
+++ b/hierarchicalsolvers.jl_amd/_lib.py
@@ -105,7 +105,7 @@
     "hsk_gemm_d", "hsk_gemm_z", "hsk_lowrank_d", "hsk_lowrank_z", "hsk_front_factor_d", "hsk_front_factor_z", "hsk_front_batch_d", "hsk_front_batch_z", "hsk_sweep_level_d", "hsk_sweep_level_z", "hsk_flow_tall_rule", "hsk_sweep_path", "hsk_mfma_f64_peak", "hsk_mfma_f64_peak_random", "hsk_flow_pingpong_us", "hsk_bisect_perm",
     "hs_probs_stats_mode", "hs_probs_stats", "hs_trim", "hs_stream_order",
     "hsk_leaf_envelope", "hsk_envelope_enable", "hsk_branch_envelope", "hsk_branch_envelope_enable", "hsk_front_batch_env_d", "hsk_op_flops_mode", "hsk_op_flops",
-    "hsk_env_order_enable", "hsk_env_tile_order",
+    "hsk_env_order_enable", "hsk_env_tile_order", "hsk_env_phase_order", "hsk_env_perm", "hsk_env_perm_slot_limit", "hsk_env_perm_min_tiles", "hsk_env_perm_launches",
     "hsk_gemm_op_d", "hsk_gemm_lds_enable", "hsk_gemm_lds_launches",
     "hsk_gemm_lds_edge_launches", "hsk_gemm_reg_launches", "hsk_gemm_lds_route", "hsk_gemm_schur_d",
     "hsk_trsm_inv_d", "hsk_trsm_strip_enable", "hsk_trsm_strip_launches", "hsk_trsm_half_launches", "hsk_lookahead_runs", "hsk_front_batch_sym_d", "hsk_front_batch_sym_z",
@@ -624,6 +624,16 @@
     L.hsk_env_order_enable.restype = C.c_int
     L.hsk_env_tile_order.argtypes = [C.c_int, C.c_int, C.c_int, C.POINTER(C.c_int32), C.POINTER(C.c_int32)]
     L.hsk_env_tile_order.restype = C.c_int
+    L.hsk_env_phase_order.argtypes = [C.c_int, C.c_int, C.POINTER(C.c_int32), C.POINTER(C.c_int32), C.c_int] + [C.POINTER(C.c_int32)] * 3
+    L.hsk_env_phase_order.restype = C.c_int
+    L.hsk_env_perm.argtypes = [C.c_int] * 3 + [C.POINTER(C.c_int32)] + [C.c_int] * 10 + [C.POINTER(C.c_uint16)]
+    L.hsk_env_perm.restype = C.c_int
+    L.hsk_env_perm_slot_limit.argtypes = [C.c_int]
+    L.hsk_env_perm_slot_limit.restype = C.c_int
+    L.hsk_env_perm_min_tiles.argtypes = [C.c_int]
+    L.hsk_env_perm_min_tiles.restype = C.c_int
+    L.hsk_env_perm_launches.argtypes = [C.c_int]
+    L.hsk_env_perm_launches.restype = C.c_longlong
     L.hsk_op_flops_mode.argtypes = [C.c_int]
     L.hsk_op_flops_mode.restype = C.c_int
     L.hsk_op_flops.argtypes = [p_f64]
diff --git a/hierarchicalsolvers.jl_amd/csrc/hs_api.hip b/hierarchicalsolvers.jl_amd/csrc/hs_api.hip
--- a/hierarchicalsolvers.jl_amd/csrc/hs_api.hip
+++ b/hierarchicalsolvers.jl_amd/csrc/hs_api.hip
@@ -211,6 +211,8 @@
   void* d_sc = nullptr;
   void* d_solve = nullptr;
   int* d_env = nullptr;
+  uint16_t* d_perm = nullptr;
+  size_t perm_cap = 0;
   std::vector<int> env_host;
   std::vector<const int*> env_dev[2];
   int env_dev_state = 1;
@@ -348,7 +350,7 @@
   arena_give(h->d_cfs, h->cfs_bytes);
   void* ptrs[] = {h->d_int, h->d_tmpi, h->d_colptr, h->d_rowval, h->d_nz,
                   h->d_nodes, h->d_sc,  h->d_solve, h->d_w1,  h->d_w2,   h->d_part,   h->d_b,   h->d_owned,
-                  h->d_rowptr, h->d_colind, h->d_tperm, h->d_nzr, h->d_lpos, h->d_env, h->d_symflag};
+                  h->d_rowptr, h->d_colind, h->d_tperm, h->d_nzr, h->d_lpos, h->d_env, h->d_symflag, h->d_perm};
   for (void* p : ptrs)
     if (p) (void)hipFree(p);
   if (h->ev0) (void)hipEventDestroy(h->ev0);
@@ -1040,6 +1042,13 @@
             if (any_leaf) L.h_env_leaf.push_back(x.off_env >= 0 && x.leaf ? h->env_host.data() + x.off_env : nullptr);
           }
         }
+        for (const LevelH& L : h->levels) {
+          int maxm = 0;
+          for (int k = 0; k < L.ndense; ++k) maxm = std::max(maxm, N[L.mine[k]].ni + N[L.mine[k]].nb);
+          if (sizeof(T) == 8 && L.ndense > 0 && hs_env_perm_wanted(maxm))
+            h->perm_cap = std::max(h->perm_cap, (size_t)L.ndense * hs_env_perm_stride(hs_env_perm_slot(maxm)));
+        }
+        if (h->perm_cap) dmalloc((void**)&h->d_perm, 2 * h->perm_cap * sizeof(uint16_t), "tile order tables");
       }
     }
 
@@ -1296,6 +1305,9 @@
       if (sch.optimistic && !dx && !henv.empty() && hs_envelope_enabled()) {
         sch.env = true;
         sch.h_env = henv.data();
+        sch.perm = h->d_perm;
+        sch.perm_side = h->d_perm ? h->d_perm + h->perm_cap : nullptr;
+        sch.perm_cap = h->perm_cap;
       }
       sch.sym = h->opts.symmetric && sch.optimistic && !dx && L.sym_ok;
       if (attempt == 1) h->sym_fronts -= sym_counted, h->sym_plain -= L.ndense - sym_counted;
diff --git a/hierarchicalsolvers.jl_amd/csrc/hs_common.h b/hierarchicalsolvers.jl_amd/csrc/hs_common.h
--- a/hierarchicalsolvers.jl_amd/csrc/hs_common.h
+++ b/hierarchicalsolvers.jl_amd/csrc/hs_common.h
@@ -123,7 +123,14 @@
   int env;
   int count;
   int order;
-};
+  int perm_slot;
+  uint16_t* perm;
+};
+#define HS_ENV_PERM_MAX 512
+#define HS_ENV_PERM_MIN_TILES 2048
+__host__ __device__ inline int hs_env_perm_stride(int slot) { return (2 + 2 * slot * slot + 2 * slot + (slot >> 3) * (slot >> 3) + 1) & ~1; }
+int hs_env_perm_slot(int maxm);
+bool hs_env_perm_wanted(int maxm);
 
 #define HS_ENV_NONE HS_BIG
 __host__ __device__ inline int hs_env_block(int p, int ni) { return p < ni ? p >> 5 : ((ni + 31) >> 5) + ((p - ni) >> 5); }
@@ -166,7 +173,8 @@
 enum { HS_GEMM_ROUTE_REG = 0, HS_GEMM_ROUTE_LDS = 1, HS_GEMM_ROUTE_EDGE = 2 };
 template <class T>
 void launch_gemm_op(const NodeDesc<T>* dnodes, int nbatch, int maxM, int maxN, const GemmOp& op, hipStream_t s, int route = HS_GEMM_ROUTE_REG,
-                    bool shifted = false, long long live_tiles = -1);
+                    bool shifted = false, long long live_tiles = -1,
+                    uint16_t* perm = nullptr, int perm_slot = 0);
 inline int hs_gemm_lds_route(int cmat, int r0, int k0, int k1, int ni) {
   const int K = (k1 < ni ? k1 : ni) - k0, arow = r0 + (cmat == HS_MAT_SB ? ni : 0);
   if (K <= 0 || (k0 & 1)) return HS_GEMM_ROUTE_REG;
diff --git a/hierarchicalsolvers.jl_amd/csrc/hs_dist.h b/hierarchicalsolvers.jl_amd/csrc/hs_dist.h
--- a/hierarchicalsolvers.jl_amd/csrc/hs_dist.h
+++ b/hierarchicalsolvers.jl_amd/csrc/hs_dist.h
@@ -116,6 +116,7 @@
   side.s2 = nullptr;
   side.s_la = nullptr;
   side.hiprio = base.s2 ? 1 : 0;
+  side.perm = base.s2 ? base.perm_side : base.perm;
   hipStream_t s = mn.s, s2 = side.s, sc = D.sc;
   int b0, b1;
   dist_bnd_slice(D.nb, g, me, b0, b1);
diff --git a/hierarchicalsolvers.jl_amd/csrc/hs_sched.h b/hierarchicalsolvers.jl_amd/csrc/hs_sched.h
--- a/hierarchicalsolvers.jl_amd/csrc/hs_sched.h
+++ b/hierarchicalsolvers.jl_amd/csrc/hs_sched.h
@@ -87,6 +87,10 @@
   const int* const* h_env = nullptr;
   bool sym = false;
   bool aligned16 = false;
+
+  uint16_t* perm = nullptr;
+  uint16_t* perm_side = nullptr;
+  size_t perm_cap = 0;
 
   void dbg(const char* what, int a = 0, int b = 0, int c = 0, int d = 0) {
     static int on = -1;
@@ -179,7 +183,9 @@
     }
     if (env && h_ni && !clipped) op.env = 0;
     hipEvent_t e0 = pf->begin(s);
-    launch_gemm_op<T>(dn, nbatch, M, N, op, s, route, shifted, op.env ? live : -1);
+    const int pslot = (sizeof(T) == 8 && op.env && perm) ? hs_env_perm_slot(maxm) : 0;
+    const bool pfits = pslot > 0 && (size_t)nbatch * hs_env_perm_stride(pslot) <= perm_cap;
+    launch_gemm_op<T>(dn, nbatch, M, N, op, s, route, shifted, op.env ? live : -1, pfits ? perm : nullptr, pfits ? pslot : 0);
     pf->end(e0, HS_CAT_GEMM, s, fl, M, N, K, nbatch, 0, hiprio);
     dbg("gemm", cmat, r0, c0, k0);
   }
@@ -433,6 +439,7 @@
     side.s2 = nullptr;
     side.s_la = nullptr;
     side.hiprio = 1;
+    side.perm = perm_side;
     if (s_la) {
       (void)hipStreamWaitEvent(s2, ev_main, 0);
       side.lu_rec(0, NB);
diff --git a/hierarchicalsolvers.jl_amd/csrc/hs_testhooks.hip b/hierarchicalsolvers.jl_amd/csrc/hs_testhooks.hip
--- a/hierarchicalsolvers.jl_amd/csrc/hs_testhooks.hip
+++ b/hierarchicalsolvers.jl_amd/csrc/hs_testhooks.hip
@@ -217,6 +217,8 @@
     sch.optimistic = true;
     sch.env = true;
     sch.h_env = h_envp.data();
+    sch.perm_cap = (size_t)count * hs_env_perm_stride(hs_env_perm_slot(maxm));
+    sch.perm = buf.get<uint16_t>(sch.perm_cap);
   }
   const long long lds0 = hsk_gemm_lds_launches(0), edge0 = hsk_gemm_lds_edge_launches(0);
   sch.gemm(HS_MAT_SB, HS_MAT_UR, 0, HS_BIG, 0, HS_BIG, 0, HS_BIG);
@@ -490,6 +492,11 @@
   if (sch.optimistic && !h_env.empty()) {
     sch.env = true;
     sch.h_env = h_env.data();
+    if (sizeof(T) == 8) {
+      sch.perm_cap = (size_t)count * hs_env_perm_stride(hs_env_perm_slot(maxm));
+      sch.perm = buf.template get<uint16_t>(2 * sch.perm_cap);
+      sch.perm_side = sch.perm + sch.perm_cap;
+    }
   }
   const auto h0 = std::chrono::steady_clock::now();
   sch.factor_fronts();
diff --git a/hierarchicalsolvers.jl_amd/csrc/kernels_gemm.hip b/hierarchicalsolvers.jl_amd/csrc/kernels_gemm.hip
--- a/hierarchicalsolvers.jl_amd/csrc/kernels_gemm.hip
+++ b/hierarchicalsolvers.jl_amd/csrc/kernels_gemm.hip
@@ -3,10 +3,12 @@
 #include <vector>
 #include <algorithm>
 #include <initializer_list>
+#include <climits>
 #include <cstdio>
 #include <cstdlib>
 #include <cstring>
 #include "hs_common.h"
+#include "hs_envelope.h"
 
 typedef double double4_t __attribute__((ext_vector_type(4)));
 typedef hs_d2u double2_u;
@@ -76,6 +78,54 @@
 __host__ __device__ inline void env_order_apply(int& tm, int& tn, int tiles_m, int tiles_n, int sm, int sn) {
   if (sm > 1) tm = tm * sm % tiles_m;
   if (sn > 1) tn = tn * sn % tiles_n;
+}
+
+__host__ __device__ inline int env_rank(const int* keys, int n, int i) {
+  const int k = keys[i];
+  int r = 0;
+  for (int j = 0; j < n; ++j) r += (keys[j] < k || (keys[j] == k && j < i)) ? 1 : 0;
+  return r;
+}
+__host__ __device__ inline int env_unit_key(const int* skr, const int* skc, int g, int c) {
+  int sum = 0;
+  for (int a = 8 * g; a < 8 * g + 8; ++a)
+    for (int b = 8 * c; b < 8 * c + 8; ++b) sum += skr[a] > skc[b] ? skr[a] : skc[b];
+  return sum;
+}
+__host__ __device__ inline int env_phase_pos(int bid, int ntiles, int nfull, int shift) {
+  const int head = (nfull >> 3) << 9;
+  int b = bid, base = 0, lg = 6;
+  if (bid >= head) {
+    b = bid - head;
+    base = head;
+    lg = 0;
+    const int sub = ntiles - head <= 256 ? 0 : ((ntiles - head) >> 3) << 3;
+    if (b >= sub) return head + sub + xcd_remap_shift(b - sub, ntiles - head - sub, shift);
+  }
+  const int x = (b + shift) & 7, o = (b - ((x - shift) & 7)) >> 3;
+  const int r = o >> lg;
+  return base + (((r << 3) + ((r & 1) ? 7 - x : x)) << lg) + (o & ((1 << lg) - 1));
+}
+__host__ __device__ inline void env_phase_coords(int p, int tiles_m, int tiles_n, const uint16_t* unitperm, int& a, int& b) {
+  const int gm = tiles_m >> 3, gn = tiles_n >> 3;
+  if (p < 64 * gm * gn) {
+    const int u = unitperm[p >> 6], q = p & 63;
+    a = 8 * (u / gn) + (q & 7);
+    b = 8 * (u % gn) + (q >> 3);
+    return;
+  }
+  p -= 64 * gm * gn;
+  const int wr = tiles_n - 8 * gn;
+  if (p < 8 * gm * wr) {
+    const int g = p / (8 * wr), q = p - g * 8 * wr;
+    a = 8 * g + (q & 7);
+    b = 8 * gn + (q >> 3);
+    return;
+  }
+  p -= 8 * gm * wr;
+  const int hb = tiles_m - 8 * gm;
+  a = 8 * gm + p % hb;
+  b = p / hb;
 }
 
 template <class T, bool ENV>
@@ -760,14 +810,21 @@
 }
 
 template <class T, Tile TILE = Tile::Reg>
-__device__ inline void gemm_dispatch_env(GemmProb<T>& p, bool minus, double* smem, const EnvClip* e, int count, int order, int mlo = 0) {
+__device__ inline void gemm_dispatch_env(GemmProb<T>& p, bool minus, double* smem, const EnvClip* e, int count, int order, int mlo = 0,
+                                         const uint32_t* pm = nullptr) {
   const TileWalk<T> w(p.M, p.N);
-  const int sm = order ? env_order_stride(w.tiles_m) : 1, sn = order ? env_order_stride(w.tiles_n) : 1;
+  const int sm = (order && !pm) ? env_order_stride(w.tiles_m) : 1, sn = (order && !pm) ? env_order_stride(w.tiles_n) : 1;
   bool ran = false;
   for (int bid = blockIdx.x; bid < w.ntiles; bid += gridDim.x) {
     int tm, tn;
-    w.coords(bid, tm, tn);
-    env_order_apply(tm, tn, w.tiles_m, w.tiles_n, sm, sn);
+    if (pm) {
+      const uint32_t t = pm[bid];
+      tm = (int)(t & 0xffffu);
+      tn = (int)(t >> 16);
+    } else {
+      w.coords(bid, tm, tn);
+      env_order_apply(tm, tn, w.tiles_m, w.tiles_n, sm, sn);
+    }
     int dk = 0;
     {
       const int m_lo = tm * TileCfg<T>::BM, n_lo = tn * TileCfg<T>::BN;
@@ -841,6 +898,72 @@
   if (!op_prologue<T, true>(nodes, op, p)) return;
   gemm_dispatch<T>(p, false, smem);
 }
+__device__ __forceinline__ const uint32_t* env_perm_slot(const GemmOp& op) {
+  if (op.order != 2) return nullptr;
+  const uint16_t* pm = op.perm + (size_t)blockIdx.y * hs_env_perm_stride(op.perm_slot);
+  return pm[0] ? (const uint32_t*)(pm + 2) : nullptr;
+}
+template <class T>
+__global__ __launch_bounds__(256) void env_perm_kernel(const NodeDesc<T>* __restrict__ nodes, GemmOp op, int edge, int gridx, int min_tiles) {
+  constexpr int MAXT = HS_ENV_PERM_MAX, MAXG = MAXT / 8;
+  __shared__ int key[2 * MAXT], skey[2 * MAXT], ukey[MAXG * MAXG];
+  __shared__ uint16_t rowperm[MAXT], colperm[MAXT], unitperm[MAXG * MAXG];
+  const int slot = op.perm_slot;
+  uint16_t* const pm = op.perm + (size_t)blockIdx.y * hs_env_perm_stride(slot);
+  GemmProb<T> p;
+  EnvClip e;
+  const bool ok = resolve_op<T, true>(nodes + blockIdx.y, op, p, &e);
+  if constexpr (sizeof(T) == 8)
+    if (ok && edge) e.row0 -= edge_shift_rows(p);
+  const int tiles_m = ok ? (p.M + TileCfg<T>::BM - 1) / TileCfg<T>::BM : 0, tiles_n = ok ? (p.N + TileCfg<T>::BN - 1) / TileCfg<T>::BN : 0;
+  if (!ok || tiles_m > slot || tiles_n > slot || slot > MAXT || tiles_m * tiles_n < min_tiles) {
+    if (threadIdx.x == 0 && blockIdx.x == 0) pm[0] = 0;
+    return;
+  }
+  const int kend = e.kbase + p.K;
+  for (int i = threadIdx.x; i < tiles_m; i += blockDim.x) {
+    const int lo = i * TileCfg<T>::BM, hi = min(lo + TileCfg<T>::BM, p.M);
+    const int v = e.fL ? hs_env_min(e.fL, e.ni, e.row0 + lo, e.row0 + hi) : e.kbase;
+    key[i] = min(max(v, e.kbase), kend);
+  }
+  for (int j = threadIdx.x; j < tiles_n; j += blockDim.x) {
+    const int lo = j * TileCfg<T>::BN, hi = min(lo + TileCfg<T>::BN, p.N);
+    const int v = e.fU ? hs_env_min(e.fU, e.ni, e.col0 + lo, e.col0 + hi) : e.kbase;
+    key[MAXT + j] = min(max(v, e.kbase), kend);
+  }
+  __syncthreads();
+  for (int i = threadIdx.x; i < tiles_m; i += blockDim.x) {
+    const int r = env_rank(key, tiles_m, i);
+    rowperm[r] = (uint16_t)i;
+    skey[r] = key[i];
+  }
+  for (int j = threadIdx.x; j < tiles_n; j += blockDim.x) {
+    const int r = env_rank(key + MAXT, tiles_n, j);
+    colperm[r] = (uint16_t)j;
+    skey[MAXT + r] = key[MAXT + j];
+  }
+  __syncthreads();
+  const int gn = tiles_n >> 3, nfull = (tiles_m >> 3) * gn, ntiles = tiles_m * tiles_n;
+  for (int u = threadIdx.x; u < nfull; u += blockDim.x) ukey[u] = env_unit_key(skey, skey + MAXT, u / gn, u % gn);
+  __syncthreads();
+  for (int u = threadIdx.x; u < nfull; u += blockDim.x) unitperm[env_rank(ukey, nfull, u)] = (uint16_t)u;
+  __syncthreads();
+  const int shift = (gridx & 7) ? (int)(((unsigned)gridx * blockIdx.y) & 7u) : 0;
+  uint32_t* const tab = (uint32_t*)(pm + 2);
+  for (int bid = blockIdx.x * blockDim.x + threadIdx.x; bid < ntiles; bid += gridDim.x * blockDim.x) {
+    int a, b;
+    env_phase_coords(env_phase_pos(bid, ntiles, nfull, shift), tiles_m, tiles_n, unitperm, a, b);
+    tab[bid] = (uint32_t)rowperm[a] | ((uint32_t)colperm[b] << 16);
+  }
+  if (blockIdx.x == 0) {
+    uint16_t* const out = pm + 2 + 2 * slot * slot;
+    for (int i = threadIdx.x; i < tiles_m; i += blockDim.x) out[i] = rowperm[i];
+    for (int j = threadIdx.x; j < tiles_n; j += blockDim.x) out[slot + j] = colperm[j];
+    for (int u = threadIdx.x; u < nfull; u += blockDim.x) out[2 * slot + u] = unitperm[u];
+    if (threadIdx.x == 0) pm[0] = 1;
+  }
+}
+
 template <class T>
 __global__ __launch_bounds__(256, 2) void gemm_op_env_kernel(const NodeDesc<T>* __restrict__ nodes, GemmOp op) {
   extern __shared__ __attribute__((aligned(16))) double smem[];
@@ -862,7 +985,7 @@
   if (!resolve_op<T, true>(nodes + blockIdx.y, op, p, &e)) return;
   const int mlo = edge_shift_rows(p);
   e.row0 -= mlo;
-  gemm_dispatch_env<T, Tile::LdsEdge>(p, true, smem, &e, 0, op.order, mlo);
+  gemm_dispatch_env<T, Tile::LdsEdge>(p, true, smem, &e, 0, op.order, mlo, env_perm_slot(op));
 }
 template <class T>
 __global__ __launch_bounds__(256, 2) void trsm_inv_env_kernel(const NodeDesc<T>* __restrict__ nodes, GemmOp op) {
@@ -975,18 +1098,51 @@
   g_benv_on.store(on ? 1 : 0);
   return prev;
 }
-static bool env_order_enabled() {
+static int env_order_setting() {
   int v = g_env_order_on.load(std::memory_order_relaxed);
   if (v < 0) {
     const char* e = getenv("HS_ENV_ORDER");
-    v = (e && e[0] == '0') ? 0 : 1;
+    v = (e && e[0] == '0') ? 0 : ((e && e[0] == '1') ? 1 : 2);
     g_env_order_on.store(v);
   }
-  return v != 0;
+  return v;
 }
 extern "C" int hsk_env_order_enable(int on) {
-  const int prev = env_order_enabled() ? 1 : 0;
-  g_env_order_on.store(on ? 1 : 0);
+  const int prev = env_order_setting();
+  g_env_order_on.store(on < 0 ? 0 : (on > 2 ? 2 : on));
+  return prev;
+}
+namespace {
+std::atomic<int> g_perm_slot_limit{HS_ENV_PERM_MAX};
+std::atomic<int> g_perm_min_tiles{-1};
+std::atomic<long long> g_perm_launches{0};
+}
+int hs_env_perm_slot(int maxm) {
+  const int need = ((maxm + 1 + 127) / 128 + 7) / 8 * 8;
+  return std::max(8, std::min(need, g_perm_slot_limit.load(std::memory_order_relaxed)));
+}
+static int hs_env_perm_min_tiles() {
+  int v = g_perm_min_tiles.load(std::memory_order_relaxed);
+  if (v < 0) {
+    const char* e = getenv("HS_ENV_ORDER_MIN_TILES");
+    v = e ? std::max(0, atoi(e)) : HS_ENV_PERM_MIN_TILES;
+    g_perm_min_tiles.store(v);
+  }
+  return v;
+}
+extern "C" int hsk_env_perm_min_tiles(int min_tiles) {
+  const int prev = hs_env_perm_min_tiles();
+  g_perm_min_tiles.store(min_tiles < 0 ? HS_ENV_PERM_MIN_TILES : min_tiles);
+  return prev;
+}
+extern "C" long long hsk_env_perm_launches(int reset) { return reset ? g_perm_launches.exchange(0) : g_perm_launches.load(); }
+bool hs_env_perm_wanted(int maxm) {
+  const long long t = (maxm + 1 + 127) / 128;
+  return t * t >= hs_env_perm_min_tiles();
+}
+extern "C" int hsk_env_perm_slot_limit(int limit) {
+  const int prev = g_perm_slot_limit.load();
+  g_perm_slot_limit.store(std::max(8, std::min(limit / 8 * 8, HS_ENV_PERM_MAX)));
   return prev;
 }
 extern "C" int hsk_env_tile_order(int tiles_m, int tiles_n, int order, int32_t* tm, int32_t* tn) {
@@ -1001,6 +1157,71 @@
     tn[bid] = n;
   }
   return 0;
+}
+extern "C" int hsk_env_phase_order(int tiles_m, int tiles_n, const int32_t* kr, const int32_t* kc, int shift, int32_t* tm, int32_t* tn, int32_t* pos) {
+  if (tiles_m <= 0 || tiles_n <= 0 || tiles_m > HS_ENV_PERM_MAX || tiles_n > HS_ENV_PERM_MAX || !kr || !kc || !tm || !tn || shift < 0 || shift > 7) return -1;
+  for (int i = 0; i < tiles_m; ++i)
+    if (kr[i] < 0 || kr[i] > (1 << 24)) return -1;
+  for (int j = 0; j < tiles_n; ++j)
+    if (kc[j] < 0 || kc[j] > (1 << 24)) return -1;
+  std::vector<uint16_t> rowperm(tiles_m), colperm(tiles_n);
+  std::vector<int> skr(tiles_m), skc(tiles_n);
+  for (int i = 0; i < tiles_m; ++i) { const int r = env_rank(kr, tiles_m, i); rowperm[r] = (uint16_t)i; skr[r] = kr[i]; }
+  for (int j = 0; j < tiles_n; ++j) { const int r = env_rank(kc, tiles_n, j); colperm[r] = (uint16_t)j; skc[r] = kc[j]; }
+  const int gn = tiles_n >> 3, nfull = (tiles_m >> 3) * gn, ntiles = tiles_m * tiles_n;
+  std::vector<int> ukey(nfull);
+  std::vector<uint16_t> unitperm(nfull + 1);
+  for (int u = 0; u < nfull; ++u) ukey[u] = env_unit_key(skr.data(), skc.data(), u / gn, u % gn);
+  for (int u = 0; u < nfull; ++u) unitperm[env_rank(ukey.data(), nfull, u)] = (uint16_t)u;
+  for (int bid = 0; bid < ntiles; ++bid) {
+    int a, b;
+    const int p = env_phase_pos(bid, ntiles, nfull, shift);
+    env_phase_coords(p, tiles_m, tiles_n, unitperm.data(), a, b);
+    if (pos) pos[bid] = p;
+    tm[bid] = rowperm[a];
+    tn[bid] = colperm[b];
+  }
+  return 0;
+}
+template <class T>
+static int env_perm_hook(int ni, int nb, const int32_t* env, const GemmOp& op_in, int edge, int slot, uint16_t* out) {
+  if (ni <= 0 || nb < 0 || ni + nb > (1 << 20) || slot < 8 || (slot & 7) || slot > HS_ENV_PERM_MAX || !out) return -1;
+  const int m = ni + nb, nblk = hs_env_nblocks(ni, nb), stride = hs_env_perm_stride(slot);
+  NodeDesc<T> d;
+  memset(&d, 0, sizeof d);
+  d.ni = ni; d.nb = nb; d.m = m;
+  d.ldl = (m + 1) / 2 * 2; d.ldu = (ni + 1) / 2 * 2; d.lds = std::max((nb + 1) / 2 * 2, 2);
+  d.LF = (T*)(uintptr_t)0x10000000; d.UR = (T*)(uintptr_t)0x20000000; d.SB = (T*)(uintptr_t)0x30000000;
+  d.ni1 = ni; d.nb1 = nb;
+  int* denv = nullptr;
+  NodeDesc<T>* dn = nullptr;
+  uint16_t* dpm = nullptr;
+  int rc = 0;
+  if (env && hipMalloc((void**)&denv, sizeof(int) * 2 * nblk) != hipSuccess) rc = -6;
+  if (!rc && hipMalloc((void**)&dn, sizeof d) != hipSuccess) rc = -6;
+  if (!rc && hipMalloc((void**)&dpm, sizeof(uint16_t) * stride) != hipSuccess) rc = -6;
+  if (!rc && env && hipMemcpy(denv, env, sizeof(int) * 2 * nblk, hipMemcpyHostToDevice) != hipSuccess) rc = -6;
+  if (!rc) {
+    d.env = denv;
+    d.finalize();
+    GemmOp op = op_in;
+    op.ainv = 0; op.env = env ? 1 : 0; op.order = 2; op.perm = dpm; op.perm_slot = slot;
+    if (hipMemcpy(dn, &d, sizeof d, hipMemcpyHostToDevice) != hipSuccess || hipMemset(dpm, 0xFF, sizeof(uint16_t) * stride) != hipSuccess) rc = -6;
+    if (!rc) {
+      hipLaunchKernelGGL(env_perm_kernel<T>, dim3(2), dim3(256), 0, nullptr, dn, op, edge, 8, 0);
+      if (hipDeviceSynchronize() != hipSuccess || hipMemcpy(out, dpm, sizeof(uint16_t) * stride, hipMemcpyDeviceToHost) != hipSuccess) rc = -6;
+    }
+  }
+  if (denv) (void)hipFree(denv);
+  if (dn) (void)hipFree(dn);
+  if (dpm) (void)hipFree(dpm);
+  return rc;
+}
+extern "C" int hsk_env_perm(int is_complex, int ni, int nb, const int32_t* env, int cmat, int bmat, int r0, int r1, int c0, int c1, int k0, int k1,
+                            int edge, int slot, uint16_t* out) {
+  if (cmat < 0 || cmat > 2 || bmat < 0 || bmat > 2 || r0 < 0 || c0 < 0 || k0 < 0) return -1;
+  GemmOp op{cmat, bmat, r0, r1, c0, c1, k0, k1};
+  return is_complex ? env_perm_hook<cplx>(ni, nb, env, op, 0, slot, out) : env_perm_hook<double>(ni, nb, env, op, edge ? 1 : 0, slot, out);
 }
 extern "C" int hsk_op_flops_mode(int on) {
   (void)hipDeviceSynchronize();
@@ -1065,17 +1286,23 @@
 
 template <class T>
 void launch_gemm_op(const NodeDesc<T>* dnodes, int nbatch, int maxM, int maxN, const GemmOp& op_in, hipStream_t s, int route, bool shifted,
-                    long long live_tiles) {
+                    long long live_tiles, uint16_t* perm, int perm_slot) {
   if (nbatch <= 0 || maxM <= 0 || maxN <= 0) return;
   GemmOp op = op_in;
   op.count = (!op.ainv && g_op_count_on.load(std::memory_order_relaxed)) ? 1 : 0;
-  op.order = (op.env && !op.ainv && env_order_enabled()) ? 1 : 0;
+  op.order = (op.env && !op.ainv) ? env_order_setting() : 0;
+  if (op.order == 2 && (!perm || perm_slot < 8 || perm_slot > HS_ENV_PERM_MAX)) op.order = 1;
   static const bool dump = getenv("HS_DEBUG_SYNC") && getenv("HS_DEBUG_SYNC")[0] == '2';
   if (dump) dump_resolved_op(dnodes, nbatch, maxM, maxN, op, s);
   if (sizeof(T) != 8 || op.ainv || op.count || !gemm_lds_enabled()) route = HS_GEMM_ROUTE_REG;
   if (op.env && route == HS_GEMM_ROUTE_LDS) route = HS_GEMM_ROUTE_EDGE;
+  if (op.order == 2 && route == HS_GEMM_ROUTE_REG) op.order = 1;
+  op.perm = op.order == 2 ? perm : nullptr;
+  op.perm_slot = op.order == 2 ? perm_slot : 0;
   if (route == HS_GEMM_ROUTE_EDGE && shifted) maxM += 1;
   int tiles = ((maxM + TileCfg<T>::BM - 1) / TileCfg<T>::BM) * ((maxN + TileCfg<T>::BN - 1) / TileCfg<T>::BN);
+  const int all_tiles = tiles;
+  if (op.order == 2 && all_tiles < hs_env_perm_min_tiles()) op.order = 1, op.perm = nullptr, op.perm_slot = 0;
   if (op.cap > 0 && tiles > op.cap) tiles = std::max(8, op.cap / 8 * 8);
   if (op.env && !(op.cap > 0)) {
     static const int walk_max = getenv("HS_ENV_WALK") ? atoi(getenv("HS_ENV_WALK")) : 4;
@@ -1093,6 +1320,11 @@
   }
   const OpKernel<T> k = pick_op_kernel<T>(op, route);
   if (k.launches) k.launches->fetch_add(1, std::memory_order_relaxed);
+  if (op.order == 2) {
+    g_perm_launches.fetch_add(1, std::memory_order_relaxed);
+    hipLaunchKernelGGL(env_perm_kernel<T>, dim3(std::max(1, std::min(32, all_tiles / 2048)), nbatch), dim3(256), 0, s, dnodes, op, 1, tiles,
+                       hs_env_perm_min_tiles());
+  }
   hipLaunchKernelGGL(k.fn, dim3(tiles, nbatch), dim3(256), k.lds_bytes, s, dnodes, op);
 }
 
@@ -1175,7 +1407,7 @@
   hipLaunchKernelGGL(gemm_probs_kernel<T>, dim3(tiles, nprob), dim3(256), lds_bytes, s, dprobs, minus);
 }
 
-template void launch_gemm_op<double>(const NodeDesc<double>*, int, int, int, const GemmOp&, hipStream_t, int, bool, long long);
-template void launch_gemm_op<cplx>(const NodeDesc<cplx>*, int, int, int, const GemmOp&, hipStream_t, int, bool, long long);
+template void launch_gemm_op<double>(const NodeDesc<double>*, int, int, int, const GemmOp&, hipStream_t, int, bool, long long, uint16_t*, int);
+template void launch_gemm_op<cplx>(const NodeDesc<cplx>*, int, int, int, const GemmOp&, hipStream_t, int, bool, long long, uint16_t*, int);
 template void launch_gemm_probs<double>(const GemmProb<double>*, int, int, int, int, hipStream_t);
 template void launch_gemm_probs<cplx>(const GemmProb<cplx>*, int, int, int, int, hipStream_t);
diff --git a/include/hs_kernels.h b/include/hs_kernels.h
--- a/include/hs_kernels.h
+++ b/include/hs_kernels.h
@@ -130,6 +130,12 @@
 int hsk_branch_envelope_enable(int on);
 int hsk_env_order_enable(int on);
 int hsk_env_tile_order(int tiles_m, int tiles_n, int order, int32_t* tm, int32_t* tn);
+int hsk_env_phase_order(int tiles_m, int tiles_n, const int32_t* kr, const int32_t* kc, int shift, int32_t* tm, int32_t* tn, int32_t* pos);
+int hsk_env_perm(int is_complex, int ni, int nb, const int32_t* env, int cmat, int bmat, int r0, int r1, int c0, int c1, int k0, int k1, int edge,
+                 int slot, uint16_t* out);
+int hsk_env_perm_slot_limit(int limit);
+int hsk_env_perm_min_tiles(int min_tiles);
+long long hsk_env_perm_launches(int reset);
 int hsk_op_flops_mode(int on);
 int hsk_op_flops(double* out);
 
```

After: 1.992 s (median of 6 runs). 6.6% less time.
